# HSarham/automatic-ar

Measured on AMD Instinct MI355X. Metric: LM iterations/sec, higher is better.
Workload: dtype f64

## Files before the change

### automatic-ar_amd/aar/__init__.py

```python
import ctypes as C
import os

import numpy as np

_HERE = os.path.dirname(os.path.abspath(__file__))
LIB_PATH = os.environ.get("AAR_LIB") or os.path.join(os.path.dirname(_HERE), "libaar.so")

AAR_OK = 0
AAR_ERR_INVALID, AAR_ERR_NO_DEVICE, AAR_ERR_HIP, AAR_ERR_UNSUPPORTED = -1, -2, -3, -4
AAR_ERR_NUMERIC, AAR_ERR_IO, AAR_ERR_COMM = -5, -6, -7
RES_F32, RES_F64 = 0, 1
COMM_ID_BYTES = 128

SYMBOLS = [
    "aar_last_error", "aar_dataset_free", "aar_dataset_full_len", "aar_synth_default", "aar_synth_generate",
    "aar_solution_read", "aar_solution_write", "aar_solution_write_yaml", "aar_detections_write",
    "aar_rodrigues_vec2mat", "aar_rodrigues_mat2vec", "aar_plan_shards", "aar_comm_make_id", "aar_comm_create",
    "aar_comm_destroy", "aar_problem_desc_from_dataset", "aar_problem_create", "aar_problem_destroy",
    "aar_problem_full_len", "aar_problem_num_vars", "aar_problem_local_obs", "aar_eval_residuals",
    "aar_eval_normal_equations", "aar_eval_damped_step", "aar_lm_default_params", "aar_lm_init", "aar_lm_step",
    "aar_lm_get_solution", "aar_lm_solve", "aar_get_stage_times", "aar_reproj_stats", "aar_device_count",
    "aar_device_synchronize", "aar_set_kernel_profiling", "aar_get_kernel_times", "aar_kernel_name",
    "aar_problem_set_huber_delta", "aar_problem_get_huber_delta", "aar_track", "aar_cam_config_read",
    "aar_undistort_points", "aar_local_group_create", "aar_local_group_destroy", "aar_comm_create_local",
    "aar_cam_configs_read", "aar_detections_read", "aar_detections_free", "aar_subseqs_read", "aar_ippe_square",
    "aar_vote_transforms", "aar_init_default_params", "aar_initializer_run", "aar_initializer_object_poses",
    "aar_comm_get_stats", "aar_lm_set_step_callback", "aar_lm_set_stop_function", "aar_problem_extract_z", "aar_problem_merge_z",
    "aar_solution_read_ex", "aar_cam_configs_read_ex", "aar_set_stage_timers", "aar_problem_pcg_iterations",
    "aar_solver_default_options", "aar_problem_create_ex", "aar_problem_get_solver_stats", "aar_problem_set_test_hook",
    "aar_problem_covariance", "aar_covariance_write_yaml",
    "aar_problem_residual_report", "aar_dataset_select_observations", "aar_residual_report_write_yaml",
    "aar_problem_constraints_validate", "aar_problem_create_constrained", "aar_problem_num_priors", "aar_problem_eval_priors",
    "aar_smooth_params_validate", "aar_track_smooth", "aar_track_smooth_system",
]
NUM_KERNELS = 18
PRIOR_CAMERA, PRIOR_MARKER = 0, 1
PRIOR_KINDS = {"camera": PRIOR_CAMERA, "marker": PRIOR_MARKER}
SOLVER_DIRECT, SOLVER_PCG, SOLVER_SPCG, SOLVER_AUTO = 0, 1, 2, 3
TEST_HOOK_SPCG_DROP = 1
ENV_SOLVER, ENV_DETERMINISTIC, ENV_PCG_ETA, ENV_PCG_MAX_IT = 1, 2, 4, 8
SOLVERS = {"direct": SOLVER_DIRECT, "pcg": SOLVER_PCG, "spcg": SOLVER_SPCG, "auto": SOLVER_AUTO}
SOLVER_NAMES = {v: k for k, v in SOLVERS.items()}


class AarError(RuntimeError):
    def __init__(self, code, msg):
        super().__init__("aar error %d: %s" % (code, msg))
        self.code = code


class CDataset(C.Structure):
    _fields_ = [
        ("num_cams", C.c_int32), ("num_markers", C.c_int32), ("num_frames", C.c_int32),
        ("root_cam", C.c_int32), ("root_marker", C.c_int32),
        ("cam_ids", C.POINTER(C.c_int32)), ("marker_ids", C.POINTER(C.c_int32)), ("frame_ids", C.POINTER(C.c_int32)),
        ("image_sizes", C.POINTER(C.c_int32)), ("cam_mats", C.POINTER(C.c_double)), ("dist_coeffs", C.POINTER(C.c_double)),
        ("marker_size", C.c_double), ("num_obs", C.c_int64),
        ("obs_frame", C.POINTER(C.c_int32)), ("obs_cam", C.POINTER(C.c_int32)), ("obs_marker", C.POINTER(C.c_int32)),
        ("obs_uv", C.POINTER(C.c_float)), ("x_full", C.POINTER(C.c_double)), ("x_truth", C.POINTER(C.c_double)),
        ("optimize_cam_poses", C.c_int32), ("optimize_marker_poses", C.c_int32),
        ("optimize_object_poses", C.c_int32), ("optimize_cam_intrinsics", C.c_int32),
    ]


class CSynthDesc(C.Structure):
    _fields_ = [
        ("num_cams", C.c_int32), ("num_markers", C.c_int32), ("num_frames", C.c_int32), ("seed", C.c_uint64),
        ("marker_size", C.c_double), ("noise_px", C.c_double), ("init_rot_sigma", C.c_double),
        ("init_trans_sigma", C.c_double), ("init_scale", C.c_double), ("cam_arc_deg", C.c_double),
        ("min_view_cos", C.c_double),
    ]


class CProblemDesc(C.Structure):
    _fields_ = [
        ("num_cams", C.c_int32), ("num_markers", C.c_int32), ("num_frames", C.c_int32),
        ("root_cam", C.c_int32), ("root_marker", C.c_int32),
        ("cam_mats", C.POINTER(C.c_double)), ("marker_size", C.c_double), ("num_obs", C.c_int64),
        ("obs_frame", C.POINTER(C.c_int32)), ("obs_cam", C.POINTER(C.c_int32)), ("obs_marker", C.POINTER(C.c_int32)),
        ("obs_uv", C.POINTER(C.c_float)),
        ("optimize_cam_poses", C.c_int32), ("optimize_marker_poses", C.c_int32), ("optimize_object_poses", C.c_int32),
        ("optimize_cam_intrinsics", C.c_int32),
        ("residual_mode", C.c_int32), ("with_huber", C.c_int32), ("device_id", C.c_int32), ("comm", C.c_void_p),
    ]


class CSolverOptions(C.Structure):
    _fields_ = [("struct_size", C.c_uint32), ("solver", C.c_int32), ("deterministic", C.c_int32), ("pcg_max_it", C.c_int32),
                ("pcg_eta", C.c_double), ("pcg_eta_loose", C.c_double), ("pcg_eta_switch", C.c_double), ("pcg_abs_tol", C.c_double)]


class CSolverStats(C.Structure):
    _fields_ = [("struct_size", C.c_uint32), ("solver", C.c_int32), ("deterministic", C.c_int32), ("last_iterations", C.c_int32),
                ("total_iterations", C.c_int64), ("solves", C.c_int64), ("fallbacks", C.c_int64), ("pcg_eta", C.c_double),
                ("pcg_max_it", C.c_int32), ("env_overrides", C.c_int32), ("same_xcd_solves", C.c_int64), ("pcg_eta_loose", C.c_double),
                ("pcg_eta_switch", C.c_double), ("pcg_abs_tol", C.c_double)]


class CCovarianceReport(C.Structure):
    _fields_ = [("struct_size", C.c_uint32), ("num_residuals", C.c_int64), ("num_vars", C.c_int64), ("sum_sq", C.c_double),
                ("sigma2", C.c_double), ("min_pivot", C.c_double), ("max_pivot", C.c_double), ("frames_written", C.c_int32)]


class COutlierRule(C.Structure):
    _fields_ = [("struct_size", C.c_uint32), ("k_median", C.c_double), ("min_px", C.c_double)]


class CResidualReport(C.Structure):
    _fields_ = [("struct_size", C.c_uint32), ("num_detections", C.c_int64), ("num_rejected", C.c_int64), ("num_nonfinite", C.c_int64),
                ("sum_sq", C.c_double), ("rmse", C.c_double), ("median", C.c_double), ("max", C.c_double), ("threshold", C.c_double),
                ("cams_emptied", C.c_int32), ("markers_emptied", C.c_int32), ("frames_emptied", C.c_int32)]


class CPosePrior(C.Structure):
    _fields_ = [("kind", C.c_int32), ("index", C.c_int32), ("x6", C.c_double * 6), ("info", C.c_double * 36)]


class CConstraints(C.Structure):
    _fields_ = [("struct_size", C.c_uint32), ("n_fixed_cams", C.c_int32), ("fixed_cams", C.POINTER(C.c_int32)),
                ("n_fixed_markers", C.c_int32), ("fixed_markers", C.POINTER(C.c_int32)),
                ("n_priors", C.c_int32), ("priors", C.POINTER(CPosePrior))]


class Constraints:

    def __init__(self, fixed_cams=None, fixed_markers=None, priors=None):
        self._fc = np.ascontiguousarray(list(fixed_cams or []), dtype=np.int32)
        self._fm = np.ascontiguousarray(list(fixed_markers or []), dtype=np.int32)
        pr = list(priors or [])
        self._pr = (CPosePrior * max(len(pr), 1))()
        for i, (kind, index, x6, info) in enumerate(pr):
            q = self._pr[i]
            q.kind = PRIOR_KINDS[kind] if isinstance(kind, str) else int(kind)
            q.index = int(index)
            x6 = np.asarray(x6, dtype=np.float64).reshape(6)
            info = np.asarray(info, dtype=np.float64).reshape(36)
            for k in range(6):
                q.x6[k] = float(x6[k])
            for k in range(36):
                q.info[k] = float(info[k])
        c = CConstraints()
        c.struct_size = C.sizeof(CConstraints)
        c.n_fixed_cams = len(self._fc)
        c.fixed_cams = self._fc.ctypes.data_as(C.POINTER(C.c_int32)) if len(self._fc) else None
        c.n_fixed_markers = len(self._fm)
        c.fixed_markers = self._fm.ctypes.data_as(C.POINTER(C.c_int32)) if len(self._fm) else None
        c.n_priors = len(pr)
        c.priors = C.cast(self._pr, C.POINTER(CPosePrior)) if pr else None
        self.c = c
        self.n_priors = len(pr)

    def empty(self):
        return self.c.n_fixed_cams == 0 and self.c.n_fixed_markers == 0 and self.c.n_priors == 0


def constraints_validate(ds, fixed_cams=None, fixed_markers=None, priors=None, optimize=None, struct_size=None):
    cds = ds.as_c()
    d = CProblemDesc()
    lib().aar_problem_desc_from_dataset(C.byref(cds), C.byref(d))
    if optimize is not None:
        d.optimize_cam_poses, d.optimize_marker_poses, d.optimize_object_poses = [int(b) for b in optimize]
    k = Constraints(fixed_cams, fixed_markers, priors)
    if struct_size is not None:
        k.c.struct_size = int(struct_size)
    _check(lib().aar_problem_constraints_validate(C.byref(d), C.byref(k.c)))


class CLmParams(C.Structure):
    _fields_ = [
        ("max_iters", C.c_int32), ("min_error", C.c_double), ("min_step_error_diff", C.c_double),
        ("min_average_step_error_diff", C.c_double), ("tau", C.c_double), ("verbose", C.c_int32),
    ]


class CSmoothParams(C.Structure):
    _fields_ = [("struct_size", C.c_uint32), ("sigma_rot", C.c_double), ("sigma_trans", C.c_double),
                ("frame_time", C.POINTER(C.c_double)), ("rel_motion", C.POINTER(C.c_double))]


# ... 765 lines not shown
        x = np.array(self._x(x_full), dtype=np.float64)
        it = np.zeros(self.ds.num_frames, dtype=np.int32)
        err = np.zeros(self.ds.num_frames)
        _check(lib().aar_track(self.handle, _dptr(x), C.byref(params) if params is not None else None,
                               it.ctypes.data_as(C.POINTER(C.c_int32)), _dptr(err)))
        return x, it, err

    def track_smooth(self, x_full, sigma_rot, sigma_trans, frame_time=None, rel_motion=None, params=None):
        x = np.array(self._x(x_full), dtype=np.float64)
        F = self.ds.num_frames
        sp = SmoothParams(sigma_rot, sigma_trans, frame_time, rel_motion)
        sp.check_lengths(F)
        fe, pe = np.zeros(max(F, 1)), np.zeros(max(F - 1, 1))
        rep = CSmoothReport()
        rep.struct_size = C.sizeof(CSmoothReport)
        _check(lib().aar_track_smooth(self.handle, _dptr(x), C.byref(params) if params is not None else None, C.byref(sp.c),
                                      _dptr(fe), _dptr(pe), C.byref(rep)))
        report = {k: getattr(rep, k) for k, _ in CSmoothReport._fields_ if k != "struct_size"}
        return x, report, fe[:F], pe[:max(F - 1, 0)]

    def track_smooth_system(self, x_full, sigma_rot, sigma_trans, mu, frame_time=None, rel_motion=None):
        x = self._x(x_full)
        F = self.ds.num_frames
        sp = SmoothParams(sigma_rot, sigma_trans, frame_time, rel_motion)
        sp.check_lengths(F)
        diag, off = np.zeros((max(F, 1), 6, 6)), np.zeros((max(F - 1, 1), 6, 6))
        rhs, delta, cost = np.zeros(6 * max(F, 1)), np.zeros(6 * max(F, 1)), np.zeros(2)
        _check(lib().aar_track_smooth_system(self.handle, _dptr(x), C.byref(sp.c), float(mu), _dptr(diag), _dptr(off), _dptr(rhs),
                                             _dptr(delta), _dptr(cost)))
        return diag[:F], off[:max(F - 1, 0)], rhs[:6 * F], delta[:6 * F], (cost[0], cost[1])

    def set_step_callback(self, fn, want_z=True):
        if fn is None:
            self._step_cb = None
            _check(lib().aar_lm_set_step_callback(self.handle, C.cast(None, STEP_CB), None, 0))
            return
        def tramp(ctx, zp, n):
            fn(np.ctypeslib.as_array(zp, shape=(n,)).copy() if zp else None)
        self._step_cb = STEP_CB(tramp)
        _check(lib().aar_lm_set_step_callback(self.handle, self._step_cb, None, int(want_z)))

    def set_stop_function(self, fn):
        if fn is None:
            self._stop_fn = None
            _check(lib().aar_lm_set_stop_function(self.handle, C.cast(None, STOP_FN), None))
            return
        def tramp(ctx, zp, n):
            return 1 if fn(np.ctypeslib.as_array(zp, shape=(n,)).copy()) else 0
        self._stop_fn = STOP_FN(tramp)
        _check(lib().aar_lm_set_stop_function(self.handle, self._stop_fn, None))

    def extract_z(self, x_full):
        x = self._x(x_full)
        z = np.zeros(self.num_vars)
        _check(lib().aar_problem_extract_z(self.handle, _dptr(x), _dptr(z)))
        return z

    def set_huber_delta(self, delta):
        _check(lib().aar_problem_set_huber_delta(self.handle, float(delta)))

    def get_huber_delta(self):
        return float(lib().aar_problem_get_huber_delta(self.handle))

    def set_kernel_profiling(self, on):
        _check(lib().aar_set_kernel_profiling(self.handle, int(on)))

    def kernel_times(self):
        sec = np.zeros(NUM_KERNELS)
        cnt = np.zeros(NUM_KERNELS, dtype=np.int64)
        _check(lib().aar_get_kernel_times(self.handle, _dptr(sec), cnt.ctypes.data_as(C.POINTER(C.c_int64))))
        return {lib().aar_kernel_name(i).decode(): (float(sec[i]), int(cnt[i])) for i in range(NUM_KERNELS)}

    def pcg_iterations(self):
        out = (C.c_int32 * 2)()
        _check(lib().aar_problem_pcg_iterations(self.handle, out))
        return int(out[0]), int(out[1])

    def solver_stats(self):
        st = CSolverStats()
        st.struct_size = C.sizeof(CSolverStats)
        _check(lib().aar_problem_get_solver_stats(self.handle, C.byref(st)))
        return dict(solver=SOLVER_NAMES[st.solver], deterministic=bool(st.deterministic), last_iterations=st.last_iterations,
                    total_iterations=st.total_iterations, solves=st.solves, fallbacks=st.fallbacks, pcg_eta=st.pcg_eta, pcg_max_it=st.pcg_max_it,
                    same_xcd_solves=st.same_xcd_solves, pcg_eta_loose=st.pcg_eta_loose, pcg_eta_switch=st.pcg_eta_switch, pcg_abs_tol=st.pcg_abs_tol, env_overrides=st.env_overrides)

    def set_test_hook(self, hook, value):
        _check(lib().aar_problem_set_test_hook(self.handle, int(hook), int(value)))

    def set_stage_timers(self, on):
        _check(lib().aar_set_stage_timers(self.handle, int(on)))

    def stage_times(self):
        t = CStageTimes()
        _check(lib().aar_get_stage_times(self.handle, C.byref(t)))
        return {n: getattr(t, n) for n, _ in CStageTimes._fields_}
```

### automatic-ar_amd/csrc/ba_capi.hip

```cpp
#include <hip/hip_runtime.h>
#include <dlfcn.h>
#include <execinfo.h>
#include <fcntl.h>
#include <unistd.h>
#include <signal.h>

#include <algorithm>
#include <array>
#include <atomic>
#include <chrono>
#include <cmath>
#include <cstring>
#include <map>
#include <numeric>
#include <condition_variable>
#include <mutex>
#include <vector>

#include "../host/internal.h"
#include "geom.hpp"
#include "hostcopy.h"
#include "kernels.h"

using namespace aar;
// ... 112 lines not shown
    if (i < n_pad) {
        if (j > i) return;
        double *a = S + (size_t)i * n_pad + j, *b = packed + (size_t)i * (i + 1) / 2 + j;
        if (dir == 0) *b = *a; else *a = *b;
    } else if (j < extra) {
        double *a = S + (size_t)n_pad * n_pad + j, *b = packed + tri + j;
        if (dir == 0) *b = *a; else *a = *b;
    }
}
}

#define NCCL_TRY(expr)                                                                                          \
    do {                                                                                                        \
        int _r = (expr);                                                                                        \
        if (_r != 0)                                                                                            \
            return set_error(AAR_ERR_COMM, "%s failed: %s", #expr, g_nccl.GetErrorString ? g_nccl.GetErrorString(_r) : "?"); \
    } while (0)

struct aar_problem {
    DeviceProblem P;
    PoseLayout L;
    int f_begin = 0, f_end = 0;
    int64_t o_begin = 0, N_global = 0;
    aar_comm *comm = nullptr;
    int device = 0;
    hipStream_t stream = nullptr;
    std::vector<void *> allocs;
    double *h_scal = nullptr;
    int32_t h_flags[4] = {0, 0, 0, 0};
    unsigned long long seq = 0;
    double *d_frames_all = nullptr;
    double *d_diag = nullptr;
    double *d_pack = nullptr;
    double *d_status = nullptr;
    PinnedBuf h_z;
    double *h_gather = nullptr; size_t h_gather_n = 0;
    hipEvent_t up_ev = nullptr;
    bool mu_seed_valid = false;
    double mu_seed = 0;
    std::vector<int32_t> h_fslot_start, h_fslot_ent;
    std::vector<int32_t> h_ent_fixed;
    std::vector<aar_pose_prior> priors;
    aar_lm_params prm;
    int cur = 0;
    double mu = -1, v = 2, currErr = 0, prevErr = 0;
    double rel_drop = -1;
    bool lm_ready = false;
    bool with_huber = false;
    float hubber_delta = 2.5f;
    aar_lm_step_callback step_cb = nullptr;
    void *step_ctx = nullptr;
    bool step_want_z = false;
    aar_lm_stop_function stop_fn = nullptr;
    void *stop_ctx = nullptr;
    std::vector<double> cb_x, cb_z;
    float huber_of_blocks = -1.f;
    bool blocks_valid = false;
    double vinv_mu = -1;
    double schur_mu = -1;
    int panels_blk = -1;
    double panels_mu = -1;
    bool s_reduced = false;
    bool trial_reduced = false;
    bool fused_comm = true;
    bool spec_chol = true;
    int solver = AAR_SOLVER_DIRECT;
    int env_overrides = 0;
    bool force_direct = false;
    int spcg_skip = 0, spcg_backoff = 0;
    int last_cg_its = -1;
    int near_cap_tries = 0;
    int64_t spcg_fallbacks = 0;
    double *h_pcg = nullptr;
    unsigned long long pcg_seq = 0;
    int spec_chol_blk = -1;
    double spec_chol_mu = -1;
    bool spec_chol_by_cg = false;
    double spec_chol_eta = 0;
    hipStream_t stream2 = nullptr;
    hipEvent_t ev_fork = nullptr, ev_join = nullptr;
    bool overlap = false;
    bool merge_passes = true;
    int64_t trial_points = 0, launches = 0;
    aar_stage_times times;
    bool stage_timers = false;
    hipEvent_t ev[2] = {nullptr, nullptr};
    bool profiling = false;
    std::vector<hipEvent_t> ev_pool;
    std::vector<int> ev_kid;
    size_t ev_used = 0;
    double k_seconds[KID_COUNT] = {0};
    int64_t k_launches[KID_COUNT] = {0};
    double *cov_ws = nullptr;
    int32_t *cov_iws = nullptr;
    RRWork rr;
    bool rr_ready = false;
};

namespace {

template <class T>
int dev_alloc(aar_problem *pb, T **ptr, size_t count) {
    void *p = nullptr;
    size_t bytes = std::max<size_t>(count, 1) * sizeof(T);
    HIP_TRY(hipMalloc(&p, bytes));
    HIP_TRY(hipMemsetAsync(p, 0, bytes, pb->stream));
    pb->allocs.push_back(p);
    *ptr = static_cast<T *>(p);
    return AAR_OK;
}

int copy_h2d(aar_problem *pb, void *dst, const void *src, size_t bytes) {
    const char *what = "";
    const int e = h2d(dst, src, bytes, pb->stream, &what);
    return e ? set_error(AAR_ERR_HIP, "%s failed: %s", what, hipGetErrorString((hipError_t)e)) : AAR_OK;
}
int copy_d2h(aar_problem *pb, void *dst, const void *src, size_t bytes) {
    const char *what = "";
    const int e = d2h(dst, src, bytes, pb->stream, &what);
    return e ? set_error(AAR_ERR_HIP, "%s failed: %s", what, hipGetErrorString((hipError_t)e)) : AAR_OK;
}

template <class T>
int dev_upload(aar_problem *pb, T **ptr, const std::vector<T> &h) {
    int rc = dev_alloc(pb, ptr, h.size());
    if (rc) return rc;
    return h.empty() ? AAR_OK : copy_h2d(pb, *ptr, h.data(), h.size() * sizeof(T));
}

int ensure_device(int device_id) {
    int n = 0;
    hipError_t e = hipGetDeviceCount(&n);
    if (e != hipSuccess || n <= 0)
        return set_error(AAR_ERR_NO_DEVICE, "no HIP device available (%s); this library has no CPU path",
                         e == hipSuccess ? "device count 0" : hipGetErrorString(e));
    if (device_id < 0 || device_id >= n) return set_error(AAR_ERR_INVALID, "device_id %d out of range (%d devices)", device_id, n);
    HIP_TRY(hipSetDevice(device_id));
    return AAR_OK;
}

void pack_z(const aar_problem *pb, const double *x_full, double *z) {
    const PoseLayout &L = pb->L;
    const int A = pb->P.A, F = pb->P.F;
    memset(z, 0, (size_t)6 * (A + F) * sizeof(double));
    for (int c = 0; c < L.C; c++)
        if (c != L.rc) memcpy(&z[6 * (size_t)c], x_full + L.full_cam0() + 6LL * L.cam_slot(c), 6 * sizeof(double));
    for (int m = 0; m < L.M; m++)
        if (m != L.rm) memcpy(&z[6 * (size_t)(L.C + m)], x_full + L.full_mk0() + 6LL * L.mk_slot(m), 6 * sizeof(double));
    if (F) memcpy(&z[6 * (size_t)A], x_full + L.full_fr0() + 6LL * pb->f_begin, (size_t)6 * F * sizeof(double));
    if (L.oi)
        for (int c = 0; c < L.C; c++) memcpy(&z[6 * (size_t)(L.C + L.M + c)], x_full + L.full_intr0() + 9LL * c, 4 * sizeof(double));
}

int upload_z(aar_problem *pb, const double *x_full, int which) {
    if (pb->up_ev) HIP_TRY(hipEventSynchronize(pb->up_ev));
    const size_t cnt = (size_t)6 * (pb->P.A + pb->P.F);
    if (pb->h_z.reserve(cnt)) return set_error(AAR_ERR_HIP, "hipHostMalloc(pose staging) failed");
    pack_z(pb, x_full, pb->h_z.data());
    if (!pb->up_ev && hipEventCreateWithFlags(&pb->up_ev, hipEventDisableTiming) != hipSuccess) { pb->up_ev = nullptr; (void)hipGetLastError(); }
    if (cnt) HIP_TRY(hipMemcpyAsync(pb->P.z[which], pb->h_z.data(), cnt * sizeof(double), hipMemcpyHostToDevice, pb->stream));
    if (pb->up_ev) HIP_TRY(hipEventRecord(pb->up_ev, pb->stream));
    else HIP_TRY(hipStreamSynchronize(pb->stream));
    return AAR_OK;
}

int allreduce(aar_problem *pb, double *buf, size_t count, int op) {
// ... 292 lines not shown
        pb->spec_chol_blk = -1;
    }
    if (P.use_pcg) {
        if (pb->vinv_mu != mu) {
            launch_frame_inv(P, cur, mu, pb->stream);
            pb->vinv_mu = mu;
            pb->launches += 1;
        }
        if (!pb->comm) {
            StageTimer t(pb, &pb->times.chol);
            launch_pcg(P, cur, mu, pb->stream);
            pb->launches += 1;
        } else {
            { StageTimer t(pb, &pb->times.chol); launch_pcgd_setup(P, cur, mu, pb->stream); }
            { StageTimer t(pb, &pb->times.allreduce); int rc = allreduce(pb, P.pcgd_setup, (size_t)P.A * 28 + ((P.pcg_fused && !P.deterministic && P.pcg_coarse) ? 144 : 0), NCCL_SUM); if (rc) return rc; }
            pb->launches += 1;
            for (int k = 0;; k++) {
                const bool last = k >= P.pcg_max_it + 1;
                const bool poll = last || (k % 4) == 3;
                if (poll) pb->pcg_seq++;
                { StageTimer t(pb, &pb->times.chol); launch_pcgd_iter(P, cur, mu, k, last, poll ? pb->pcg_seq : 0ull, pb->stream); }
                pb->launches += 1;
                if (poll) {
                    int rc = check_async("pcg launch");
                    if (rc) return rc;
                    volatile unsigned long long *sq = reinterpret_cast<volatile unsigned long long *>(pb->h_pcg) + 3;
                    const auto t0 = std::chrono::steady_clock::now();
                    unsigned spins = 0;
                    int poll_rc = AAR_OK;
                    while (*sq != pb->pcg_seq) {
                        if ((++spins & 0x3fff) == 0) {
                            if (hipStreamQuery(pb->stream) == hipSuccess && *sq != pb->pcg_seq) {
                                poll_rc = set_error(AAR_ERR_HIP, "device did not publish the PCG progress record: %s", hipGetErrorString(hipGetLastError()));
                                break;
                            }
                            if (std::chrono::duration<double>(std::chrono::steady_clock::now() - t0).count() > 120.0) {
                                poll_rc = set_error(AAR_ERR_HIP, "timed out waiting for the PCG progress record");
                                break;
                            }
                        }
                        __builtin_ia32_pause();
                    }
                    std::atomic_thread_fence(std::memory_order_acquire);
                    if (poll_rc) return poll_rc;
                    if (pb->h_pcg[0] != 0.0 || last) break;
                }
                { StageTimer t(pb, &pb->times.allreduce); int rc = allreduce(pb, pcgd_y_of_launch(P, k), (size_t)6 * P.A, NCCL_SUM); if (rc) return rc; }
            }
        }
        chol_done = true;
    }
    if (!P.use_pcg && pb->schur_mu != mu) {
        StageTimer t(pb, &pb->times.schur);
        if (pb->s_reduced) {
            int rc = zero_block_set(pb, cur);
            if (rc) return rc;
            launch_passB(P, cur, pb->stream);
            launch_prior(P, cur, true, pb->stream);
            pb->launches += P.n_prior ? 2 : 1;
            pb->s_reduced = false;
        } else if (pb->schur_mu >= 0) {
            launch_schur(P, cur, -1.0, pb->stream, 0, 0, nullptr, panels_ok(pb, cur, pb->schur_mu));
            panels_now(pb, cur, pb->schur_mu);
            pb->launches += 1;
        }
        if (pb->vinv_mu != mu) {
            launch_frame_inv(P, cur, mu, pb->stream);
            pb->vinv_mu = mu;
            pb->launches += 1;
        }
        launch_schur(P, cur, 1.0, pb->stream, 0, 0, nullptr, panels_ok(pb, cur, mu));
        panels_now(pb, cur, mu);
        pb->launches += 1;
    }
    pb->schur_mu = -1;
    if (pb->comm && !pb->s_reduced && !P.use_pcg) {
        StageTimer t(pb, &pb->times.allreduce);
        int rc = allreduce_system(pb, cur, 0);
        if (rc) return rc;
    }
    pb->s_reduced = false;
    pb->trial_reduced = false;
    bool backsub_rode = false;
    if (P.use_spcg && !pb->force_direct && pb->spcg_skip > 0) pb->spcg_skip--;
    if (!chol_done) {
        StageTimer t(pb, &pb->times.chol);
        if (by_cg) backsub_rode = launch_spcg(P, cur, mu, pb->stream, pb->stage_timers ? -1 : tr);
        else backsub_rode = launch_chol(P, cur, mu, pb->stream, pb->stage_timers ? -1 : tr);
    }
    if (!backsub_rode) {
        StageTimer t(pb, &pb->times.backsub);
        launch_backsub(P, cur, tr, pb->stream);
    }
    pb->launches += 2 + 3 * P.nT;
    pb->blocks_valid = false;
    if (evaluate_trial) {
        int rc = eval_blocks(pb, tr, mu * 0.33, cur, false, true);
        if (rc) return rc;
        pb->trial_points++;
    } else {
        HIP_TRY(hipMemsetAsync(P.err_part, 0, sizeof(double) * (size_t)std::max(n_err_terms(P), 1), pb->stream));
    }
    int rc = AAR_OK;
    bool rode = false;
    if (P.use_pcg) {
        if ((rc = launch_scalars(pb, n_err_terms(P)))) return rc;
    } else if (evaluate_trial && !pb->comm) {
        StageTimer t(pb, &pb->times.schur);
        rode = launch_schur(P, tr, 1.0, pb->stream, pb->seq + 1, n_err_terms(P), nullptr, panels_ok(pb, tr, mu * 0.33));
        panels_now(pb, tr, mu * 0.33);
        pb->launches += 1;
        if (rode) pb->seq++;
        else if ((rc = launch_scalars(pb, n_err_terms(P)))) return rc;
    } else if (evaluate_trial && pb->fused_comm) {
        {
            StageTimer t(pb, &pb->times.schur);
            rode = launch_schur(P, tr, 1.0, pb->stream, 0, n_err_terms(P), P.blk[tr].tail, panels_ok(pb, tr, mu * 0.33));
            panels_now(pb, tr, mu * 0.33);
            pb->launches += 1;
            if (!rode) { launch_reduce_scalars(P, n_err_terms(P), false, 0ull, pb->stream, P.blk[tr].tail); pb->launches += 1; }
        }
        pb->seq++;
        {
            StageTimer t(pb, &pb->times.allreduce);
            if ((rc = allreduce_system(pb, tr, 4, pb->seq))) return rc;
        }
        pb->trial_reduced = true;
        if (pb->spec_chol && !pb->stage_timers && !pb->profiling) {
            StageTimer t(pb, &pb->times.chol);
            const bool spec_cg = P.use_spcg && pb->spcg_skip == 0 && !cg_near_cap;
            if (spec_cg) launch_spcg(P, tr, mu * 0.33, pb->stream);
            else (void)launch_chol(P, tr, mu * 0.33, pb->stream);
            pb->spec_chol_by_cg = spec_cg;
            pb->spec_chol_blk = tr;
            pb->spec_chol_mu = mu * 0.33;
            pb->spec_chol_eta = P.pcg_eta_now;
            pb->launches += 3 * P.nT;
        }
    } else {
        if ((rc = launch_scalars(pb, n_err_terms(P)))) return rc;
        if (evaluate_trial) {
            StageTimer t(pb, &pb->times.schur);
            launch_schur(P, tr, 1.0, pb->stream, 0, 0, nullptr, panels_ok(pb, tr, mu * 0.33));
            panels_now(pb, tr, mu * 0.33);
            pb->launches += 1;
        }
    }
    if ((rc = check_async("kernel launch"))) return rc;
    if ((rc = wait_result(pb))) return rc;
    if (by_cg && pb->h_scal[7] >= 0.0) pb->last_cg_its = (int)pb->h_scal[7];
    if (by_cg && (pb->h_flags[0] & (8 | 4))) pb->last_cg_its = std::min(P.spcg_max_it, SPCG_MAX_IT);
    if (cg_near_cap && P.use_spcg && !pb->force_direct && pb->spcg_skip == 0 && ++pb->near_cap_tries >= 8) { pb->last_cg_its = -1; pb->near_cap_tries = 0; }
    if (pb->h_flags[0]) {
        (void)hipMemsetAsync(P.flags, 0, 4 * sizeof(int32_t), pb->stream);
        if (by_cg && (pb->h_flags[0] & (8 | 4))) {
            if (pb->h_flags[0] & 4) spcg_ws_reset(P, pb->stream);
            pb->spcg_fallbacks++;
            pb->spcg_backoff = pb->spcg_backoff ? std::min(2 * pb->spcg_backoff, 1024) : 8;
            pb->spcg_skip = pb->spcg_backoff;
            return TRY_CG_FAILED;
        }
        set_error(AAR_ERR_NUMERIC, "device flags %d at mu=%g (1: a frame block is not positive definite, 2: non-positive pivot of the reduced system, 4: back-substitution chain timed out)", pb->h_flags[0], mu);
        return ((pb->h_flags[0] & 2) && !(pb->h_flags[0] & 4)) ? TRY_NOT_POSITIVE_DEFINITE : AAR_ERR_NUMERIC;
    }
    return AAR_OK;
}

int rebuild_current(aar_problem *pb) {
    pb->mu_seed_valid = false;
    int rc = zero_block_set(pb, pb->cur);
    if (rc) return rc;
    if ((rc = zero_block_set(pb, 1 - pb->cur))) return rc;
    const float huber_now = pb->P.huber;
    if (pb->with_huber && pb->huber_of_blocks > 0.f) pb->P.huber = pb->huber_of_blocks;
    rc = eval_blocks(pb, pb->cur, -1.0, -1);
    pb->P.huber = huber_now;
    if (rc) return rc;
    pb->blocks_valid = true;
    pb->vinv_mu = -1;
    pb->schur_mu = -1;
    pb->s_reduced = pb->trial_reduced = false;
    return AAR_OK;
}

int damped_try_fb(aar_problem *pb, double mu, bool evaluate_trial) {
    int rc = damped_try(pb, mu, evaluate_trial);
    if (rc != TRY_CG_FAILED) return rc;
    if (evaluate_trial) pb->trial_points--;
    pb->trial_reduced = false;
    if ((rc = rebuild_current(pb))) return rc;
    pb->force_direct = true;
    rc = damped_try(pb, mu, evaluate_trial);
// ... 274 lines not shown
    return problem_create(d, opts, &k, out);
}

int32_t aar_problem_num_priors(const aar_problem *pb) { return pb ? pb->P.n_prior : 0; }

static int abort_bt_fd = 2;
static void abort_backtrace(int sig) {
    void *bt[64];
    { char msg[64]; const int k = aar::g_last_kernel_id; int n = 0; const char *t = "last kernel id "; while (t[n]) { msg[n] = t[n]; n++; } if (k < 0) msg[n++] = '-'; else { if (k >= 10) msg[n++] = '0' + k / 10; msg[n++] = '0' + k % 10; } msg[n++] = '\n'; (void)!write(abort_bt_fd, msg, n); }
    const int n = backtrace(bt, 64);
    backtrace_symbols_fd(bt, n, abort_bt_fd);
    signal(sig, SIG_DFL);
    raise(sig);
}

int aar_problem_create_ex(const aar_problem_desc *d, const aar_solver_options *opts, aar_problem **out) { return problem_create(d, opts, nullptr, out); }

static int problem_create(const aar_problem_desc *d, const aar_solver_options *opts, const aar_problem_constraints *cons, aar_problem **out) {
    { static bool once = false; if (!once && getenv("AAR_ABORT_BACKTRACE")) { once = true; const int fd = open(getenv("AAR_ABORT_BACKTRACE"), O_WRONLY | O_CREAT | O_APPEND, 0644); if (fd >= 0) abort_bt_fd = fd; signal(SIGABRT, abort_backtrace); } }
    if (!d || !out) return set_error(AAR_ERR_INVALID, "aar_problem_create: null argument");
    aar_solver_options so;
    aar_solver_default_options(&so);
    if (opts) {
        if (opts->struct_size < 2 * sizeof(uint32_t)) return set_error(AAR_ERR_INVALID, "aar_solver_options.struct_size is not set (use aar_solver_default_options)");
        memcpy(&so, opts, std::min<size_t>(opts->struct_size, sizeof so));
        so.struct_size = (uint32_t)sizeof so;
    }
    int env_over = 0;
    if (const char *e = getenv("AAR_SOLVER")) {
        if (so.solver == AAR_SOLVER_AUTO) {
            int v = -1;
            if (!strcmp(e, "direct")) v = AAR_SOLVER_DIRECT;
            else if (!strcmp(e, "pcg")) v = AAR_SOLVER_PCG;
            else if (!strcmp(e, "spcg")) v = AAR_SOLVER_SPCG;
            if (v >= 0) { so.solver = v; env_over |= AAR_ENV_SOLVER; }
        }
    }
    if (const char *e = getenv("AAR_DETERMINISTIC")) if (!so.deterministic && atoi(e) != 0) { so.deterministic = 1; env_over |= AAR_ENV_DETERMINISTIC; }
    if (const char *e = getenv("AAR_PCG_ETA")) if (so.pcg_eta == 0 && atof(e) > 0) { so.pcg_eta = atof(e); env_over |= AAR_ENV_PCG_ETA; }
    if (const char *e = getenv("AAR_PCG_MAX_IT")) if (so.pcg_max_it == 0 && atoi(e) > 0) { so.pcg_max_it = atoi(e); env_over |= AAR_ENV_PCG_MAX_IT; }
    if (so.solver < AAR_SOLVER_DIRECT || so.solver > AAR_SOLVER_AUTO) return set_error(AAR_ERR_INVALID, "aar_solver_options.solver %d is not one of AAR_SOLVER_*", so.solver);
    if (so.pcg_eta < 0 || so.pcg_max_it < 0 || so.pcg_eta_loose < 0 || so.pcg_eta_switch < 0 || so.pcg_abs_tol < 0) return set_error(AAR_ERR_INVALID, "aar_solver_options: negative pcg_eta / pcg_eta_loose / pcg_eta_switch / pcg_abs_tol / pcg_max_it");
    const int C = d->num_cams, M = d->num_markers, Fg = d->num_frames;
    const int64_t Ng = d->num_obs;
    if (C < 1 || M < 1 || Fg < 0 || Ng < 0) return set_error(AAR_ERR_INVALID, "aar_problem_create: bad sizes");
    if (d->root_cam < 0 || d->root_cam >= C || d->root_marker < 0 || d->root_marker >= M)
        return set_error(AAR_ERR_INVALID, "aar_problem_create: root index out of range");
    if (!d->cam_mats || (Ng > 0 && (!d->obs_frame || !d->obs_cam || !d->obs_marker || !d->obs_uv)))
        return set_error(AAR_ERR_INVALID, "aar_problem_create: null array");
    if (Ng >= (1LL << 31) || (int64_t)C + M >= 32768) return set_error(AAR_ERR_UNSUPPORTED, "problem too large for 32-bit indexing");
    std::vector<int64_t> per_frame(Fg, 0);
    int64_t global_slots = 0;
    {
        std::vector<int32_t> seen_c(C, -1), seen_m(M, -1);
        for (int64_t o = 0; o < Ng; o++) {
            const int f = d->obs_frame[o], c = d->obs_cam[o], m = d->obs_marker[o];
            if (f < 0 || f >= Fg || c < 0 || c >= C || m < 0 || m >= M) return set_error(AAR_ERR_INVALID, "observation %lld has an index out of range", (long long)o);
            if (o > 0 && f < d->obs_frame[o - 1]) return set_error(AAR_ERR_INVALID, "observations must be ordered by frame (reference residual order)");
            per_frame[f]++;
            if (seen_c[c] != f) { seen_c[c] = f; global_slots += d->optimize_cam_intrinsics ? 2 : 1; }
            if (seen_m[m] != f) { seen_m[m] = f; global_slots += 1; }
        }
    }
    int rc = ensure_device(d->device_id);
    if (rc) return rc;

    aar_problem *pb = new aar_problem();
    pb->device = d->device_id;
    pb->comm = d->comm;
    aar_lm_default_params(&pb->prm);
    memset(&pb->times, 0, sizeof pb->times);
    const char *tenv = getenv("AAR_STAGE_TIMERS");
    pb->stage_timers = tenv && tenv[0] == '1';
    auto fail = [&](int code) { aar_problem_destroy(pb); return code; };
    if (hipStreamCreateWithFlags(&pb->stream, hipStreamNonBlocking) != hipSuccess) return fail(set_error(AAR_ERR_HIP, "hipStreamCreate failed"));
    (void)hipEventCreate(&pb->ev[0]);
    (void)hipEventCreate(&pb->ev[1]);
    if (hipStreamCreateWithFlags(&pb->stream2, hipStreamNonBlocking) != hipSuccess ||
        hipEventCreateWithFlags(&pb->ev_fork, hipEventDisableTiming) != hipSuccess ||
        hipEventCreateWithFlags(&pb->ev_join, hipEventDisableTiming) != hipSuccess)
        return fail(set_error(AAR_ERR_HIP, "second stream / events could not be created"));
    { const char *e = getenv("AAR_OVERLAP"); pb->overlap = (e && e[0] == '1'); }
    { const char *e = getenv("AAR_MERGE_PASSES"); if (e) pb->merge_passes = (e[0] != '0'); }
    { const char *e = getenv("AAR_FUSED_COMM"); if (e) pb->fused_comm = (e[0] != '0'); }
    { const char *e = getenv("AAR_SPEC_CHOL"); if (e) pb->spec_chol = (e[0] != '0'); }

    PoseLayout &L = pb->L;
    L.C = C; L.M = M; L.F = Fg; L.rc = d->root_cam; L.rm = d->root_marker;
    L.oc = d->optimize_cam_poses != 0; L.om = d->optimize_marker_poses != 0; L.of = d->optimize_object_poses != 0;
    L.oi = d->optimize_cam_intrinsics != 0;
    pb->N_global = Ng;

    const int world = pb->comm ? pb->comm->world : 1, rank = pb->comm ? pb->comm->rank : 0;
    pb->P.pcg_rank0 = rank == 0 ? 1 : 0;
    std::vector<int32_t> begin(world + 1, 0);
    if ((rc = aar_plan_shards(Fg, per_frame.data(), world, begin.data()))) return fail(rc);
    pb->f_begin = begin[rank];
    pb->f_end = begin[rank + 1];
    int64_t ob = 0;
    for (int f = 0; f < pb->f_begin; f++) ob += per_frame[f];
    int64_t N = 0;
    for (int f = pb->f_begin; f < pb->f_end; f++) N += per_frame[f];
    pb->o_begin = ob;

    DeviceProblem &P = pb->P;
    P.intr = L.oi ? 1 : 0;
    P.C = C; P.M = M; P.A = C + M + (L.oi ? C : 0); P.F = pb->f_end - pb->f_begin; P.N = N;
    P.n = 6 * P.A;
    P.nT = (P.n + CHOL_NB - 1) / CHOL_NB;
    P.n_pad = P.nT * CHOL_NB;
    P.spcg_root_c = (L.oc && C > 1) ? L.rc : -1;
    P.spcg_root_m = (L.om && M > 1) ? C + L.rm : -1;
    P.spcg_n_free = (L.oc ? C - 1 : 0) + (L.om ? M - 1 : 0) + (L.oi ? C : 0);
    P.res_f32 = d->residual_mode == AAR_RES_F64 ? 0 : 1;
    pb->with_huber = d->with_huber != 0;
    P.huber = pb->with_huber ? pb->hubber_delta : -1.f;
    P.half_size = (double)((float)d->marker_size / 2.f);
    P.frames_fixed = L.of ? 0 : 1;
    const int A = P.A, F = P.F;
    std::vector<int32_t> held(C + M, 0);
    bool held_extra = false;
    if (cons) {
        for (int i = 0; i < cons->n_fixed_cams; i++) { const int c = cons->fixed_cams[i]; if (c != L.rc && L.oc) { held[c] = 1; held_extra = true; } }
        for (int i = 0; i < cons->n_fixed_markers; i++) { const int m = cons->fixed_markers[i]; if (m != L.rm && L.om) { held[C + m] = 1; held_extra = true; } }
    }

    int local_rc = AAR_OK;
    std::vector<int32_t> frame_obs_start(F + 1, 0), fslot_start(F + 1, 0), fslot_ent;
    std::vector<ObsIdx> a_idx(N);
    std::vector<float> a_uv((size_t)8 * N);
    if (N) memcpy(a_uv.data(), d->obs_uv + 8 * ob, sizeof(float) * 8 * N);
    {
        int64_t o = 0;
        std::vector<int32_t> slot_of(A, -1);
        for (int f = 0; f < F; f++) {
            frame_obs_start[f] = (int32_t)o;
            const int64_t cnt = per_frame[pb->f_begin + f];
            std::vector<int32_t> ents;
            for (int64_t k = 0; k < cnt; k++) {
                const int64_t g = ob + o + k;
                ents.push_back(d->obs_cam[g]);
                ents.push_back(C + d->obs_marker[g]);
                if (L.oi) ents.push_back(C + M + d->obs_cam[g]);
            }
            std::sort(ents.begin(), ents.end());
            ents.erase(std::unique(ents.begin(), ents.end()), ents.end());
            if (ents.size() >= (1u << SLOT_C_BITS) && !local_rc) local_rc = set_error(AAR_ERR_UNSUPPORTED, "frame %d touches %zu entities (limit %d)", f, ents.size(), (1 << SLOT_C_BITS) - 1);
            for (size_t s = 0; s < ents.size(); s++) slot_of[ents[s]] = (int32_t)s;
            for (int64_t k = 0; k < cnt; k++) {
                const int64_t g = ob + o + k;
                ObsIdx id;
                id.frame = f; id.cam = d->obs_cam[g]; id.marker = C + d->obs_marker[g];
                id.slots = pack_slots(slot_of[id.cam], slot_of[id.marker], L.oi ? slot_of[C + M + id.cam] : 0);
                a_idx[o + k] = id;
            }
            fslot_start[f] = (int32_t)fslot_ent.size();
            fslot_ent.insert(fslot_ent.end(), ents.begin(), ents.end());
            P.max_kf = std::max<int>(P.max_kf, (int)ents.size());
            o += cnt;
        }
        frame_obs_start[F] = (int32_t)o;
        fslot_start[F] = (int32_t)fslot_ent.size();
    }
    P.total_slots = (int)fslot_ent.size();
    std::vector<int32_t> frame_stride(F, 1);
    for (int f = 0; f < F; f++) {
// ... 1330 lines not shown
    if (frame_err && F && (rc = copy_d2h(pb, frame_err, w.Ef[cur], (size_t)F * sizeof(double)))) return rc;
    if (pair_err && F > 1 && (rc = copy_d2h(pb, pair_err, w.Pe[cur], (size_t)(F - 1) * sizeof(double)))) return rc;
    if ((rc = check_async("smoothing kernels"))) return rc;
    PoseLayout keep = pb->L;
    pb->L.oc = false; pb->L.om = false; pb->L.of = true;
    rc = download_z(pb, pb->cur, x_full);
    pb->L = keep;
    if (rc) return rc;
    if (report) {
        aar_smooth_report r;
        memset(&r, 0, sizeof r);
        r.struct_size = report->struct_size;
        r.iterations = iters; r.stop_code = mustExit; r.rejected_tries = rejected;
        r.initial_cost = initial; r.final_cost = currErr; r.final_data_cost = currData; r.final_prior_cost = currPrior;
        r.final_mu = mu;
        r.seconds = std::chrono::duration<double>(std::chrono::steady_clock::now() - t0).count();
        memcpy(report, &r, std::min<size_t>(report->struct_size, sizeof r));
    }
    return AAR_OK;
}

int aar_set_kernel_profiling(aar_problem *pb, int on) {
    if (!pb) return set_error(AAR_ERR_INVALID, "aar_set_kernel_profiling: null argument");
    HIP_TRY(hipSetDevice(pb->device));
    HIP_TRY(hipStreamSynchronize(pb->stream));
    pb->ev_kid.clear();
    pb->ev_used = 0;
    pb->profiling = on != 0;
    if (on) {
        memset(pb->k_seconds, 0, sizeof pb->k_seconds);
        memset(pb->k_launches, 0, sizeof pb->k_launches);
        pb->P.hook.pre = prof_pre;
        pb->P.hook.post = prof_post;
        pb->P.hook.ctx = pb;
    } else {
        pb->P.hook = LaunchHook();
    }
    return AAR_OK;
}

int aar_get_kernel_times(aar_problem *pb, double seconds[AAR_NUM_KERNELS], int64_t launches[AAR_NUM_KERNELS]) {
    if (!pb || !seconds || !launches) return set_error(AAR_ERR_INVALID, "aar_get_kernel_times: null argument");
    static_assert(AAR_NUM_KERNELS == KID_COUNT, "kernel id table out of sync with include/aar.h");
    static_assert(ENT_STRIDE == ENT_STRIDE_H, "entity row stride");
    HIP_TRY(hipSetDevice(pb->device));
    HIP_TRY(hipStreamSynchronize(pb->stream));
    prof_harvest(pb);
    for (int i = 0; i < KID_COUNT; i++) { seconds[i] = pb->k_seconds[i]; launches[i] = pb->k_launches[i]; }
    return AAR_OK;
}

const char *aar_kernel_name(int kid) {
    static const char *names[KID_COUNT] = {"k_unpack", "k_residual", "k_passA", "k_passB", "k_maxdiag", "k_frame_inv", "k_schur",
                                           "k_ldl_diag", "k_ldl_trsm", "k_ldl_update", "k_ldl_backsolve", "k_backsub",
                                           "k_reduce_scalars", "k_ldl_panel", "k_pcg", "k_spcg", "k_spcg_pre", "k_prior"};
    return (kid >= 0 && kid < KID_COUNT) ? names[kid] : "?";
}

int aar_problem_pcg_iterations(aar_problem *pb, int32_t out[2]) {
    if (!pb || !out) return set_error(AAR_ERR_INVALID, "aar_problem_pcg_iterations: null argument");
    out[0] = out[1] = 0;
    if (!pb->P.use_pcg && !pb->P.use_spcg) return AAR_OK;
    HIP_TRY(hipSetDevice(pb->device));
    { int rc = copy_d2h(pb, out, pb->P.use_pcg ? pb->P.pcg_counter + 2 : pb->P.spcg_iters, 2 * sizeof(int32_t)); if (rc) return rc; }
    if (out[0] > SPCG_MAX_IT && pb->P.use_spcg) out[0] = SPCG_MAX_IT;
    return AAR_OK;
}

int aar_problem_get_solver_stats(aar_problem *pb, aar_solver_stats *out) {
    if (!pb || !out) return set_error(AAR_ERR_INVALID, "aar_problem_get_solver_stats: null argument");
    const size_t cap = out->struct_size;
    if (cap < 4 * sizeof(int32_t) || cap > 4096) return set_error(AAR_ERR_INVALID, "aar_solver_stats.struct_size is not set (sizeof(aar_solver_stats) of the caller)");
    aar_solver_stats st;
    memset(&st, 0, sizeof st);
    st.solver = pb->solver;
    st.deterministic = pb->P.deterministic;
    st.pcg_eta = pb->P.pcg_eta;
    st.pcg_max_it = pb->P.use_spcg ? pb->P.spcg_max_it : pb->P.pcg_max_it;
    st.pcg_eta_loose = pb->P.pcg_eta_loose;
    st.pcg_eta_switch = pb->P.pcg_eta_switch;
    st.pcg_abs_tol = pb->P.pcg_abs_tol;
    st.env_overrides = pb->env_overrides;
    st.fallbacks = pb->spcg_fallbacks;
    if (pb->P.use_pcg || pb->P.use_spcg) {
        int32_t c[8] = {0, 0, 0, 0, 0, 0, 0, 0};
        HIP_TRY(hipSetDevice(pb->device));
        int rc = copy_d2h(pb, c, pb->P.use_spcg ? pb->P.spcg_iters : pb->P.pcg_counter + 2, (pb->P.use_spcg ? 8 : 3) * sizeof(int32_t));
        if (rc) return rc;
        st.last_iterations = std::min(c[0], pb->P.use_spcg ? SPCG_MAX_IT : c[0]);
        st.total_iterations = c[1];
        st.solves = c[2];
        st.same_xcd_solves = c[4];
    }
    st.struct_size = (uint32_t)std::min(cap, sizeof st);
    memcpy(out, &st, std::min(cap, sizeof st));
    return AAR_OK;
}

int aar_problem_set_test_hook(aar_problem *pb, int32_t hook, int32_t value) {
    if (!pb) return set_error(AAR_ERR_INVALID, "aar_problem_set_test_hook: null argument");
    if (hook == AAR_TEST_HOOK_SPCG_DROP) { pb->P.spcg_test_drop = value; return AAR_OK; }
    return set_error(AAR_ERR_INVALID, "aar_problem_set_test_hook: unknown hook %d", hook);
}

int aar_set_stage_timers(aar_problem *pb, int on) {
    if (!pb) return set_error(AAR_ERR_INVALID, "aar_set_stage_timers: null argument");
    HIP_TRY(hipSetDevice(pb->device));
    HIP_TRY(hipStreamSynchronize(pb->stream));
    pb->stage_timers = on != 0;
    memset(&pb->times, 0, sizeof pb->times);
    return AAR_OK;
}

int aar_get_stage_times(aar_problem *pb, aar_stage_times *t) {
    if (!pb || !t) return set_error(AAR_ERR_INVALID, "aar_get_stage_times: null argument");
    *t = pb->times;
    return AAR_OK;
}

}
```

### automatic-ar_amd/csrc/backsub.hpp

```cpp
#pragma once
#include "geom.hpp"
#include "kernels.h"

namespace aar {

__device__ __forceinline__ void hop_publish(int32_t *flag, int value, bool leader) {
    asm volatile("s_waitcnt vmcnt(0)" ::: "memory");
    if (leader) __hip_atomic_store(flag, value, __ATOMIC_RELAXED, __HIP_MEMORY_SCOPE_AGENT);
}
__device__ __forceinline__ bool hop_wait(const int32_t *flag, int value) {
    long spins = 0;
    while (__hip_atomic_load(flag, __ATOMIC_RELAXED, __HIP_MEMORY_SCOPE_AGENT) != value) {
        __builtin_amdgcn_s_sleep(1);
        if (++spins > (1L << 24)) return false;
    }
    asm volatile("" ::: "memory");
    return true;
}

struct BacksubArgs {
    const int32_t *fslot_start, *fslot_ent;
    const double *W, *Vinv, *gf, *g0, *delta_s, *zc;
    const float *Wf;
    double *zt;
    int A, F, n_frame_blocks;
    double *lin_part, *ent_out;
    int k_ent0;
};

__device__ __forceinline__ void backsub_body(const BacksubArgs &b, int blk, double *red, const int32_t *flag, int epoch, int32_t *err_flags) {
    const int tid = threadIdx.x, lane = tid & 63, wave = __builtin_amdgcn_readfirstlane(tid >> 6), nwaves = blockDim.x >> 6;
    auto dl = [&](int i) -> double {
        return flag ? __hip_atomic_load(b.delta_s + i, __ATOMIC_RELAXED, __HIP_MEMORY_SCOPE_AGENT) : b.delta_s[i];
    };
    auto wait = [&]() {
        if (!flag) return;
        if (tid == 0 && !hop_wait(flag, epoch)) atomicOr(err_flags, 4);
        __syncthreads();
    };
    if (blk == b.n_frame_blocks) {
        wait();
        double d2 = 0.0, dg = 0.0;
        for (int i = tid; i < 6 * b.A; i += blockDim.x) {
            const double d = dl(i);
            b.zt[i] = b.zc[i] + d;
            d2 += d * d;
            dg += d * b.g0[i];
        }
#pragma unroll
        for (int off = 32; off > 0; off >>= 1) { d2 += __shfl_xor(d2, off); dg += __shfl_xor(dg, off); }
        if (lane == 0) { red[wave] = d2; red[16 + wave] = dg; }
        __syncthreads();
        if (tid == 0) {
            double s2 = 0.0, sg = 0.0;
            for (int w = 0; w < nwaves; w++) { s2 += red[w]; sg += red[16 + w]; }
            b.lin_part[2 * (size_t)b.F] = s2;
            b.lin_part[2 * (size_t)b.F + 1] = sg;
        }
        __threadfence_block();
        __syncthreads();
        for (int e = tid; e < b.A; e += blockDim.x) {
            if (e >= b.k_ent0) make_k_row(b.zt + 6 * (size_t)e, b.ent_out + (size_t)e * ENT_STRIDE);
            else make_ent_row(b.zt + 6 * (size_t)e, b.ent_out + (size_t)e * ENT_STRIDE);
        }
        return;
    }
    const int f = blk * nwaves + wave;
    const bool live = f < b.F;
    const int s0 = live ? b.fslot_start[f] : 0, s1 = live ? b.fslot_start[f + 1] : 0;
    const int sl = s0 + lane;
    const bool has = sl < s1;
    int a0 = 0;
    double2 w0[18];
    if (has) {
        a0 = b.fslot_ent[sl];
        if (b.Wf) {
            const float4 *wf = reinterpret_cast<const float4 *>(b.Wf + (size_t)s0 * 36) + lane;
            const int kf = s1 - s0;
#pragma unroll
            for (int q = 0; q < 9; q++) {
                const float4 v = wf[(size_t)q * kf];
                w0[2 * q] = make_double2(v.x, v.y); w0[2 * q + 1] = make_double2(v.z, v.w);
            }
        } else {
            const double2 *wb = reinterpret_cast<const double2 *>(b.W + (size_t)sl * 36);
#pragma unroll
            for (int q = 0; q < 18; q++) w0[q] = wb[q];
        }
    }
    double g[6], vrow[6], zc6 = 0.0;
#pragma unroll
    for (int i = 0; i < 6; i++) { g[i] = live ? b.gf[(size_t)f * 6 + i] : 0.0; vrow[i] = (live && lane < 6) ? b.Vinv[(size_t)f * 36 + lane * 6 + i] : 0.0; }
    if (live && lane < 6) zc6 = b.zc[(size_t)6 * (b.A + f) + lane];
    wait();
    if (!live) return;
    double c[6] = {0, 0, 0, 0, 0, 0};
    if (has) {
        double da[6];
#pragma unroll
        for (int i = 0; i < 6; i++) da[i] = dl(6 * a0 + i);
#pragma unroll
        for (int i = 0; i < 6; i++) {
            c[0] += w0[3 * i].x * da[i]; c[1] += w0[3 * i].y * da[i]; c[2] += w0[3 * i + 1].x * da[i];
            c[3] += w0[3 * i + 1].y * da[i]; c[4] += w0[3 * i + 2].x * da[i]; c[5] += w0[3 * i + 2].y * da[i];
        }
    }
    for (int s = s0 + lane + 64; s < s1; s += 64) {
        const int a = b.fslot_ent[s];
        double2 wt[18];
        if (b.Wf) {
            const float4 *wf = reinterpret_cast<const float4 *>(b.Wf + (size_t)s0 * 36) + (s - s0);
            const int kf = s1 - s0;
#pragma unroll
            for (int q = 0; q < 9; q++) {
                const float4 v = wf[(size_t)q * kf];
                wt[2 * q] = make_double2(v.x, v.y); wt[2 * q + 1] = make_double2(v.z, v.w);
            }
        } else {
            const double2 *wb = reinterpret_cast<const double2 *>(b.W + (size_t)s * 36);
#pragma unroll
            for (int q = 0; q < 18; q++) wt[q] = wb[q];
        }
        double da[6];
#pragma unroll
        for (int i = 0; i < 6; i++) da[i] = dl(6 * a + i);
#pragma unroll
        for (int i = 0; i < 6; i++) {
            const double2 x0 = wt[3 * i], x1 = wt[3 * i + 1], x2 = wt[3 * i + 2];
            c[0] += x0.x * da[i]; c[1] += x0.y * da[i]; c[2] += x1.x * da[i];
            c[3] += x1.y * da[i]; c[4] += x2.x * da[i]; c[5] += x2.y * da[i];
        }
    }
#pragma unroll
    for (int off = 32; off > 0; off >>= 1)
#pragma unroll
        for (int i = 0; i < 6; i++) c[i] += __shfl_xor(c[i], off);
    double d = 0.0;
    if (lane < 6) {
#pragma unroll
        for (int k = 0; k < 6; k++) d += vrow[k] * (g[k] - c[k]);
        b.zt[(size_t)6 * (b.A + f) + lane] = zc6 + d;
    }
    {
        const double zn = (lane < 6) ? zc6 + d : 0.0;
        double zv[6];
#pragma unroll
        for (int i = 0; i < 6; i++) zv[i] = __shfl(zn, i);
        if (lane == 0) make_ent_row(zv, b.ent_out + (size_t)(b.A + f) * ENT_STRIDE);
    }
    double d2 = (lane < 6) ? d * d : 0.0;
    double dgv = 0.0;
#pragma unroll
    for (int i = 0; i < 6; i++) dgv += (lane == i) ? d * g[i] : 0.0;
#pragma unroll
    for (int off = 4; off > 0; off >>= 1) { d2 += __shfl_xor(d2, off); dgv += __shfl_xor(dgv, off); }
    if (lane == 0) { b.lin_part[2 * (size_t)f] = d2; b.lin_part[2 * (size_t)f + 1] = dgv; }
}

BacksubArgs backsub_args(const DeviceProblem &P, int cur, int trial, int waves_per_block);

}
```

### automatic-ar_amd/csrc/eval_kernels.hip

```cpp
#include <algorithm>
#include <vector>
#include "geom.hpp"
#include "kernels.h"
#include "hostcopy.h"
#include "wave.hpp"
#include "track_eval.hpp"

namespace aar {

volatile int g_last_kernel_id = -1;

template <int NV, int CH = 32, class Sink>
__device__ __forceinline__ void wave_sum_lds(const double (&vals)[NV], double *__restrict__ sc, int lane, Sink sink) {
    constexpr int L = 64 / CH;
    constexpr int SPREAD = 32 / CH > 0 ? 32 / CH : 1;
#pragma unroll
    for (int base = 0; base < NV; base += CH) {
        const int cnt = (NV - base) < CH ? (NV - base) : CH;
#pragma unroll
        for (int i = 0; i < CH; i++)
            if (i < cnt) sc[i * 64 + lane] = vals[base + i];
        __builtin_amdgcn_fence(__ATOMIC_RELEASE, "wavefront");
        __builtin_amdgcn_wave_barrier();
        const int vi = lane / L, part = lane % L;
        double s = 0;
        if (vi < cnt) {
            const double *row = sc + lane * CH;
#pragma unroll 8
            for (int k = 0; k < CH; k++) s += row[(k + lane / SPREAD) & (CH - 1)];
        }
#pragma unroll
        for (int off = 1; off < L; off <<= 1) s += __shfl_xor(s, off);
        if (part == 0 && vi < cnt) sink(base + vi, s);
        __builtin_amdgcn_wave_barrier();
        __builtin_amdgcn_fence(__ATOMIC_ACQUIRE, "wavefront");
    }
}

__global__ void k_unpack(const double *__restrict__ z, double *__restrict__ ent, int n_ent, int k0, int k1, double *__restrict__ zero_p, int64_t zero_n,
                         double *__restrict__ zero_q, int64_t zero_qn) {
    const int64_t gid = (int64_t)blockIdx.x * blockDim.x + threadIdx.x;
    for (int64_t i = gid; i < zero_n; i += (int64_t)gridDim.x * blockDim.x) zero_p[i] = 0.0;
    for (int64_t i = gid; i < zero_qn; i += (int64_t)gridDim.x * blockDim.x) zero_q[i] = 0.0;
    if (gid >= n_ent) return;
    if (gid >= k0 && gid < k1) make_k_row(z + 6 * gid, ent + gid * ENT_STRIDE);
    else make_ent_row(z + 6 * gid, ent + gid * ENT_STRIDE);
}

__global__ void __launch_bounds__(256) k_residual(const ObsIdx *__restrict__ idx, const float *__restrict__ uv,
                                                  const double *__restrict__ ent, const double *__restrict__ Kmat, int kstride,
                                                  int64_t N, int A, double h, int res_f32, float huber, double *__restrict__ r_out,
                                                  double *__restrict__ err_part) {
    const int64_t o = (int64_t)blockIdx.x * blockDim.x + threadIdx.x;
    double ss = 0;
    if (o < N) {
        const ObsIdx id = idx[o];
        const float4 uv0 = reinterpret_cast<const float4 *>(uv)[2 * o];
        const float4 uv1 = reinterpret_cast<const float4 *>(uv)[2 * o + 1];
        const float ou[8] = {uv0.x, uv0.y, uv0.z, uv0.w, uv1.x, uv1.y, uv1.z, uv1.w};
        EntRT ec, em, ef;
        load_ent_rt(ent, id.cam, ec);
        load_ent_rt(ent, id.marker, em);
        load_ent_rt(ent, A + id.frame, ef);
        double K[9];
#pragma unroll
        for (int i = 0; i < 9; i++) K[i] = Kmat[kstride * id.cam + i];
#pragma unroll
        for (int k = 0; k < 4; k++) {
            CornerGeom g;
            project_corner(ec, em, ef, K, h, k, g);
            double rx, ry;
            corner_residual(ou[2 * k], ou[2 * k + 1], g.u, g.v, res_f32, huber, rx, ry);
            ss += rx * rx + ry * ry;
            if (r_out) {
                r_out[8 * o + 2 * k] = rx;
                r_out[8 * o + 2 * k + 1] = ry;
            }
        }
    }
    __shared__ double wsum[4];
#pragma unroll
    for (int off = 32; off > 0; off >>= 1) ss += __shfl_xor(ss, off);
    if ((threadIdx.x & 63) == 0) wsum[threadIdx.x >> 6] = ss;
    __syncthreads();
    if (threadIdx.x == 0) err_part[blockIdx.x] = wsum[0] + wsum[1] + wsum[2] + wsum[3];
}

__device__ __forceinline__ void load_ent_lds(const double *row, Ent &e) {
#pragma unroll
    for (int i = 0; i < 9; i++) e.R[i] = row[i];
#pragma unroll
    for (int i = 0; i < 3; i++) e.t[i] = row[9 + i];
#pragma unroll
    for (int i = 0; i < 9; i++) e.Jl[i] = row[12 + i];
}

struct PassAArgs {
    const ObsIdx *idx; const float *uv; const double *ent; const double *Kmat;
    int kstride;
    const int32_t *frame_obs_start, *fslot_start, *fslot_ent, *frame_stride;
    unsigned long long *stamps;
    int k_ent0;
    int A, F, C, res_f32, max_kf, frames_fixed;
    float huber;
    double h, mu_pred;
    double *V, *gf, *W, *Vinv, *hf, *err_part;
    float *Wf;
    double *zero0; int64_t zero0_n; double *zero1; int64_t zero1_n; double *zero2; int64_t zero2_n;
    int32_t *flags;
    double *Wd, *Yd; const int32_t *slot_dense; int Ad;
};

constexpr int ENT_LDS = 25;
constexpr int WLS = 37;
__host__ __device__ constexpr size_t passA_w_doubles(int max_kf) { return ((size_t)max_kf * WLS + 1) & ~(size_t)1; }
__host__ __device__ constexpr int passA_sum_chunk(int block) { return block >= 128 ? 8 : 32; }

template <int BLOCK>
__device__ __forceinline__ void passA_epilogue(const PassAArgs &a, const double *Wl, const double *acc, double *scratch, const int f, const int s0, const int kf) {
    const int tid = threadIdx.x;
// ... 119 lines not shown
    }
    constexpr int LPO = 4 / CPL;
    for (int t = tid; t < nobs * LPO; t += BLOCK) {
        const int it = t / LPO, part = t - it * LPO;
        const int o = o0 + (int)(((int64_t)it * stride) % nobs);
        const ObsIdx id = a.idx[o];
        const int sc = id.slots & ((1 << SLOT_C_BITS) - 1), sm = (id.slots >> SLOT_C_BITS) & ((1 << SLOT_M_BITS) - 1);
        const int sk = (id.slots >> (SLOT_C_BITS + SLOT_M_BITS)) & ((1 << SLOT_M_BITS) - 1);
        Ent ec, em;
        load_ent_lds(entl + (size_t)sc * ENT_LDS, ec);
        load_ent_lds(entl + (size_t)sm * ENT_LDS, em);
        double K[9];
#pragma unroll
        for (int i = 0; i < 9; i++) K[i] = a.Kmat[a.kstride * id.cam + i];
        double Wc[36], Wm[36], Wk[INTR ? 24 : 1];
#pragma unroll
        for (int i = 0; i < 36; i++) { Wc[i] = 0.0; Wm[i] = 0.0; }
        if (INTR) {
#pragma unroll
            for (int i = 0; i < 24; i++) Wk[i] = 0.0;
        }
#pragma unroll
        for (int kk = 0; kk < CPL; kk++) {
            const int k = part * CPL + kk;
            const float2 ouv = reinterpret_cast<const float2 *>(a.uv)[4 * (int64_t)o + k];
            CornerGeom g;
            project_corner(ec, em, ef, K, a.h, k, g);
            double r[2];
            corner_residual(ouv.x, ouv.y, g.u, g.v, a.res_f32, a.huber, r[0], r[1]);
            double Gc[2][6], Gm[2][6], Gf[2][6];
            corner_jacobian<true, true, true>(ec, em, ef, K, g, Gc, Gm, Gf);
            if (INTR) {
                double Gk[2][4];
                corner_jacobian_intr(g, Gk);
#pragma unroll
                for (int rr = 0; rr < 2; rr++)
#pragma unroll
                    for (int i = 0; i < 4; i++)
#pragma unroll
                        for (int j = 0; j < 6; j++) Wk[i * 6 + j] += Gk[rr][i] * Gf[rr][j];
            }
#pragma unroll
            for (int rr = 0; rr < 2; rr++) {
                vals[27] += r[rr] * r[rr];
#pragma unroll
                for (int i = 0; i < 6; i++) {
                    vals[21 + i] += Gf[rr][i] * r[rr];
#pragma unroll
                    for (int j = 0; j <= i; j++) vals[i * (i + 1) / 2 + j] += Gf[rr][i] * Gf[rr][j];
#pragma unroll
                    for (int j = 0; j < 6; j++) {
                        Wc[i * 6 + j] += Gc[rr][i] * Gf[rr][j];
                        Wm[i * 6 + j] += Gm[rr][i] * Gf[rr][j];
                    }
                }
            }
        }
        double *wc = Wl + sc * WLS;
        double *wm = Wl + sm * WLS;
#pragma unroll
        for (int i = 0; i < 36; i++) atomicAdd(wc + i, Wc[i]);
#pragma unroll
        for (int i = 0; i < 36; i++) atomicAdd(wm + i, Wm[i]);
        if (INTR) {
            double *wk = Wl + sk * WLS;
#pragma unroll
            for (int i = 0; i < 24; i++) atomicAdd(wk + i, Wk[i]);
        }
    }
    wave_sum_lds<28, CH>(vals, scratch + wave * (CH * 64), lane, [&](int i, double s) { atomicAdd(acc + i, s); });
    __syncthreads();
    passA_epilogue<BLOCK>(a, Wl, acc, scratch, f, s0, kf);
}

constexpr int HLS = 21, HLS_INTR = 25;
__host__ __device__ constexpr size_t passA_h_doubles(int max_kf, int hls = HLS) { return ((size_t)max_kf * hls + 1) & ~(size_t)1; }

#ifdef AAR_PASSA_STAMPS
#define PA_STAMP(n) do { if (a.stamps && f < 512 && tid == 0) a.stamps[f * 16 + (n)] = __builtin_readcyclecounter(); } while (0)
#else
#define PA_STAMP(n) do { } while (0)
#endif

template <int BLOCK, int CPL, bool INTR = false>
__device__ __forceinline__ void passA_wrench_body(const PassAArgs &a, double *lds, const int f, const int n_blocks_a) {
    constexpr int SL = INTR ? HLS_INTR : HLS;
    double *Hl = lds;
    double *acc = lds + passA_h_doubles(a.max_kf, SL);
    double *hacc = acc + 32;
    double *frow = acc + 64;
    double *Yl = frow + 24;
    double *vil = Yl + 36;
    const int tid = threadIdx.x, lane = tid & 63, wave = tid >> 6;
    const int o0 = a.frame_obs_start[f], nobs = a.frame_obs_start[f + 1] - o0;
    const int s0 = a.fslot_start[f], kf = a.fslot_start[f + 1] - s0;
    PA_STAMP(0);
    Ent ef;
    load_ent(a.ent, a.A + __builtin_amdgcn_readfirstlane(f), ef);
    constexpr int LPO = 4 / CPL;
    const int stride = a.frame_stride[f];
    const int part = tid % LPO;
    int pos = 0, step = 0;
    if (nobs > 0) {
        pos = (int)(((unsigned long long)(tid / LPO) * (unsigned)stride) % (unsigned)nobs);
        step = (int)(((unsigned long long)(BLOCK / LPO) * (unsigned)stride) % (unsigned)nobs);
    }
    int t = tid;
    bool have = t < nobs * LPO;
    ObsIdx id = {0, 0, 0, 0};
    float2 ouv[CPL];
    EntRT ec, em;
    double K[9];
    auto fetch_obs = [&]() {
        const int o = o0 + pos;
        id = a.idx[o];
#pragma unroll
        for (int kk = 0; kk < CPL; kk++) ouv[kk] = reinterpret_cast<const float2 *>(a.uv)[4 * (int64_t)o + part * CPL + kk];
    };
    auto fetch_rows = [&]() {
        load_ent_rt(a.ent, id.cam, ec);
        load_ent_rt(a.ent, id.marker, em);
#pragma unroll
        for (int i = 0; i < 9; i++) K[i] = a.Kmat[a.kstride * id.cam + i];
    };
    if (have) fetch_obs();
    const int e_slot = tid < kf ? a.fslot_ent[s0 + tid] : -1;
    double2 frv = make_double2(0.0, 0.0);
    if (tid < ENT_STRIDE / 2) frv = reinterpret_cast<const double2 *>(a.ent + (size_t)(a.A + f) * ENT_STRIDE)[tid];
    for (int i = tid; i < kf * SL; i += BLOCK) Hl[i] = 0.0;
    for (int i = tid; i < 64; i += BLOCK) acc[i] = 0.0;
    if (have) fetch_rows();
    {
        const int64_t gid = (int64_t)f * BLOCK + tid, gstride = (int64_t)n_blocks_a * BLOCK;
        for (int64_t i = gid; i < a.zero0_n; i += gstride) a.zero0[i] = 0.0;
        for (int64_t i = gid; i < a.zero1_n; i += gstride) a.zero1[i] = 0.0;
        for (int64_t i = gid; i < a.zero2_n; i += gstride) a.zero2[i] = 0.0;
    }
    __syncthreads();
    PA_STAMP(1);

    double vals[7];
#pragma unroll
    for (int i = 0; i < 7; i++) vals[i] = 0.0;
    while (have) {
        const int sc = id.slots & ((1 << SLOT_C_BITS) - 1), sm = (id.slots >> SLOT_C_BITS) & ((1 << SLOT_M_BITS) - 1);
        const int sk = (id.slots >> (SLOT_C_BITS + SLOT_M_BITS)) & ((1 << SLOT_M_BITS) - 1);
        double H[21], Mk[INTR ? 24 : 1];
#pragma unroll
        for (int i = 0; i < 21; i++) H[i] = 0.0;
        if (INTR) {
#pragma unroll
            for (int i = 0; i < 24; i++) Mk[i] = 0.0;
        }
#pragma unroll (INTR && CPL == 4 ? 2 : CPL)
        for (int kk = 0; kk < CPL; kk++) {
            CornerGeom g;
            project_corner(ec, em, ef, K, a.h, part * CPL + kk, g);
            double r[2], w[2][6];
            corner_residual(ouv[kk].x, ouv[kk].y, g.u, g.v, a.res_f32, a.huber, r[0], r[1]);
            corner_wrench(ec, K, g, w);
            if (INTR) {
                double Gk[2][4];
                corner_jacobian_intr(g, Gk);
#pragma unroll
                for (int rr = 0; rr < 2; rr++)
#pragma unroll
                    for (int i = 0; i < 4; i++)
#pragma unroll
                        for (int j = 0; j < 6; j++) Mk[i * 6 + j] += Gk[rr][i] * w[rr][j];
            }
#pragma unroll
            for (int rr = 0; rr < 2; rr++) {
                vals[6] += r[rr] * r[rr];
#pragma unroll
                for (int i = 0; i < 6; i++) {
                    vals[i] += w[rr][i] * r[rr];
#pragma unroll
                    for (int j = 0; j <= i; j++) H[i * (i + 1) / 2 + j] += w[rr][i] * w[rr][j];
                }
            }
        }
        t += BLOCK;
        have = t < nobs * LPO;
        if (have) {
            pos += step;
            if (pos >= nobs) pos -= nobs;
            fetch_obs();
        }
        double *hc = Hl + sc * SL, *hm = Hl + sm * SL;
#pragma unroll
        for (int i = 0; i < 21; i++) atomicAdd(hc + i, H[i]);
#pragma unroll
        for (int i = 0; i < 21; i++) atomicAdd(hm + i, H[i]);
        if (INTR) {
            double *hk = Hl + sk * SL;
#pragma unroll
            for (int i = 0; i < 24; i++) atomicAdd(hk + i, Mk[i]);
        }
        if (have) fetch_rows();
    }
    PA_STAMP(2);
    double2 rv[7];
    if (e_slot >= 0) {
        const double2 *rowp = reinterpret_cast<const double2 *>(a.ent + (size_t)e_slot * ENT_STRIDE);
#pragma unroll
        for (int i = 0; i < 7; i++) rv[i] = rowp[4 + i];
        if (e_slot < a.C) atomicAdd(hacc + 30, 1.0);
    }
    for (int ts = tid + BLOCK; ts < kf; ts += BLOCK)
        if (a.fslot_ent[s0 + ts] < a.C) atomicAdd(hacc + 30, 1.0);
    if (tid < ENT_STRIDE / 2) { frow[2 * tid] = frv.x; frow[2 * tid + 1] = frv.y; }
#pragma unroll
    for (int i = 0; i < 7; i++) {
        const double sv = wave_sum_dpp(vals[i]);
        if (lane == 0) atomicAdd(hacc + 21 + i, sv);
    }
    PA_STAMP(3);
    __syncthreads();
    PA_STAMP(4);
    if (tid < 21) {
        const int nc = (int)hacc[30];
        double sv = 0.0;
        for (int ts = 0; ts < nc; ts++) sv += Hl[ts * SL + tid];
        hacc[tid] = sv;
    }
    __syncthreads();
    PA_STAMP(5);
    if (wave == BLOCK / 64 - 1) {
        const double *jl = frow + 12;
        if (lane < 36) {
            const int k = lane / 6, j = lane - 6 * k;
            Yl[lane] = j < 3 ? hacc[sym6(k, 0)] * jl[j] + hacc[sym6(k, 1)] * jl[3 + j] + hacc[sym6(k, 2)] * jl[6 + j] : hacc[sym6(k, j)];
        }
        __builtin_amdgcn_fence(__ATOMIC_RELEASE, "wavefront");
        __builtin_amdgcn_wave_barrier();
        __builtin_amdgcn_fence(__ATOMIC_ACQUIRE, "wavefront");
        if (lane < 28) {
            double out;
            if (lane < 21) {
                int i = 0;
                while ((i + 1) * (i + 2) / 2 <= lane) i++;
                const int j = lane - i * (i + 1) / 2;
                out = i < 3 ? jl[i] * Yl[j] + jl[3 + i] * Yl[6 + j] + jl[6 + i] * Yl[12 + j] : Yl[i * 6 + j];
            } else if (lane < 27) {
                const int i = lane - 21;
                out = i < 3 ? jl[i] * hacc[21] + jl[3 + i] * hacc[22] + jl[6 + i] * hacc[23] : hacc[21 + i];
            } else out = hacc[27];
            acc[lane] = out;
        }
        __builtin_amdgcn_fence(__ATOMIC_RELEASE, "wavefront");
        __builtin_amdgcn_wave_barrier();
        __builtin_amdgcn_fence(__ATOMIC_ACQUIRE, "wavefront");
        if (a.mu_pred >= 0.0 && lane == 63) {
            double out[36];
            if (a.frames_fixed) {
#pragma unroll
                for (int i = 0; i < 36; i++) out[i] = 0.0;
            } else {
                double m[6][6];
#pragma unroll
                for (int i = 0; i < 6; i++)
#pragma unroll
                    for (int j = 0; j < 6; j++) m[i][j] = acc[sym6(i, j)] + (i == j ? a.mu_pred : 0.0);
                if (!spd6_inverse(m, out)) atomicOr(a.flags, 1);
            }
            const bool dense_ = a.Yd != nullptr;
#pragma unroll
            for (int i = 0; i < 6; i++) {
                double hv = 0.0;
#pragma unroll
                for (int j = 0; j < 6; j++) {
                    a.Vinv[(size_t)f * 36 + i * 6 + j] = out[i * 6 + j];
                    hv += out[i * 6 + j] * acc[21 + j];
                    if (dense_) vil[i * 6 + j] = out[i * 6 + j];
                }
                a.hf[(size_t)f * 6 + i] = hv;
            }
        }
    }
    PA_STAMP(6);
    for (int ts = tid; ts < kf; ts += BLOCK) {
        int e = e_slot;
        if (ts != tid) {
            e = a.fslot_ent[s0 + ts];
            const double2 *rowp = reinterpret_cast<const double2 *>(a.ent + (size_t)e * ENT_STRIDE);
#pragma unroll
            for (int i = 0; i < 7; i++) rv[i] = rowp[4 + i];
        }
        if (INTR && e >= a.k_ent0) {
            const double *mk = Hl + ts * SL;
            double wv[36];
#pragma unroll
            for (int i = 0; i < 4; i++) {
                double m6[6];
#pragma unroll
                for (int j = 0; j < 6; j++) m6[j] = mk[i * 6 + j];
#pragma unroll
                for (int j = 0; j < 3; j++) wv[6 * i + j] = m6[0] * ef.Jl[j] + m6[1] * ef.Jl[3 + j] + m6[2] * ef.Jl[6 + j];
                wv[6 * i + 3] = m6[3]; wv[6 * i + 4] = m6[4]; wv[6 * i + 5] = m6[5];
            }
#pragma unroll
            for (int q = 24; q < 36; q++) wv[q] = 0.0;
            if (a.W) {
                double2 *wp = reinterpret_cast<double2 *>(a.W + (size_t)(s0 + ts) * 36);
#pragma unroll
                for (int q = 0; q < 18; q++) wp[q] = make_double2(wv[2 * q], wv[2 * q + 1]);
            }
            if (a.Wf) {
                float4 *wf = reinterpret_cast<float4 *>(a.Wf + (size_t)s0 * 36) + ts;
#pragma unroll
                for (int q = 0; q < 9; q++) wf[(size_t)q * kf] = make_float4((float)wv[4 * q], (float)wv[4 * q + 1], (float)wv[4 * q + 2], (float)wv[4 * q + 3]);
            }
            continue;
        }
        const bool cam = e < a.C;
        const double tt[3] = {cam ? rv[0].y - ef.t[0] : rv[0].y, cam ? rv[1].x - ef.t[1] : rv[1].x, cam ? rv[1].y - ef.t[2] : rv[1].y};
        const double Jl[9] = {rv[2].x, rv[2].y, rv[3].x, rv[3].y, rv[4].x, rv[4].y, rv[5].x, rv[5].y, rv[6].x};
        double H[21], X[6][6];
        const double *slot = Hl + ts * SL;
#pragma unroll
        for (int i = 0; i < 21; i++) H[i] = slot[i];
#pragma unroll
        for (int l = 0; l < 6; l++) {
            double zt[3], zb[3], x[3];
#pragma unroll
            for (int i = 0; i < 3; i++) {
                zt[i] = cam ? H[sym6(i, l)] : ef.R[i] * H[sym6(0, l)] + ef.R[3 + i] * H[sym6(1, l)] + ef.R[6 + i] * H[sym6(2, l)];
                zb[i] = cam ? H[sym6(3 + i, l)] : ef.R[i] * H[sym6(3, l)] + ef.R[3 + i] * H[sym6(4, l)] + ef.R[6 + i] * H[sym6(5, l)];
            }
            cross3(tt, zb, x);
            const double v[3] = {zt[0] - x[0], zt[1] - x[1], zt[2] - x[2]};
#pragma unroll
            for (int i = 0; i < 3; i++) {
                const double wt = Jl[i] * v[0] + Jl[3 + i] * v[1] + Jl[6 + i] * v[2];
                X[i][l] = cam ? -wt : wt;
                X[3 + i][l] = cam ? -zb[i] : zb[i];
            }
        }
        double2 *wp = reinterpret_cast<double2 *>(a.W + (size_t)(s0 + ts) * 36);
        float4 *wf = a.Wf ? reinterpret_cast<float4 *>(a.Wf + (size_t)s0 * 36) + ts : nullptr;
#pragma unroll
        for (int i2 = 0; i2 < 3; i2++) {
            float w12[12];
#pragma unroll
            for (int ii = 0; ii < 2; ii++) {
                const int i = 2 * i2 + ii;
                double wr[3];
#pragma unroll
                for (int j = 0; j < 3; j++) wr[j] = X[i][0] * ef.Jl[j] + X[i][1] * ef.Jl[3 + j] + X[i][2] * ef.Jl[6 + j];
                if (a.W) {
                    wp[3 * i] = make_double2(wr[0], wr[1]);
                    wp[3 * i + 1] = make_double2(wr[2], X[i][3]);
                    wp[3 * i + 2] = make_double2(X[i][4], X[i][5]);
                }
                w12[6 * ii] = (float)wr[0]; w12[6 * ii + 1] = (float)wr[1]; w12[6 * ii + 2] = (float)wr[2];
                w12[6 * ii + 3] = (float)X[i][3]; w12[6 * ii + 4] = (float)X[i][4]; w12[6 * ii + 5] = (float)X[i][5];
            }
            if (wf) {
#pragma unroll
                for (int q = 0; q < 3; q++) wf[(size_t)(3 * i2 + q) * kf] = make_float4(w12[4 * q], w12[4 * q + 1], w12[4 * q + 2], w12[4 * q + 3]);
            }
        }
    }
    PA_STAMP(7);
    __syncthreads();
    PA_STAMP(8);
    for (int q = tid; q < 36; q += BLOCK) a.V[(size_t)f * 36 + q] = acc[sym6(q / 6, q % 6)];
    for (int q = tid; q < 6; q += BLOCK) a.gf[(size_t)f * 6 + q] = acc[21 + q];
    if (tid == 0) a.err_part[f] = acc[27];
    const bool dense = a.Yd != nullptr && a.mu_pred >= 0.0;
    PA_STAMP(9);
    if (dense) {
        __syncthreads();
        double vi[36];
#pragma unroll
        for (int q = 0; q < 36; q++) vi[q] = vil[q];
        const size_t fbase = (size_t)f * a.Ad * 36;
        for (int ts = tid; ts < kf; ts += BLOCK) {
            const double2 *wp = reinterpret_cast<const double2 *>(a.W + (size_t)(s0 + ts) * 36);
            const size_t o = fbase + (size_t)a.slot_dense[s0 + ts] * 36;
#pragma unroll
            for (int i = 0; i < 6; i++) {
                const double2 w0 = wp[3 * i], w1 = wp[3 * i + 1], w2 = wp[3 * i + 2];
                const double w[6] = {w0.x, w0.y, w1.x, w1.y, w2.x, w2.y};
                double y[6] = {0, 0, 0, 0, 0, 0};
#pragma unroll
                for (int k = 0; k < 6; k++)
#pragma unroll
                    for (int j = 0; j < 6; j++) y[j] = fma(w[k], vi[k * 6 + j], y[j]);
                double2 *yp = reinterpret_cast<double2 *>(a.Yd + o + i * 6), *wd = reinterpret_cast<double2 *>(a.Wd + o + i * 6);
                yp[0] = make_double2(y[0], y[1]); yp[1] = make_double2(y[2], y[3]); yp[2] = make_double2(y[4], y[5]);
                wd[0] = w0; wd[1] = w1; wd[2] = w2;
            }
        }
        if (tid < 6) a.Wd[fbase + tid] = acc[21 + tid];
    }
}

struct PassBArgs {
    const ObsIdx *idx; const float *uv; const double *ent; const double *Kmat; const int32_t *chunk_start;
    int kstride, k_ent0;
    int n_chunks, A, res_f32, n_pad;
    float huber;
    double h;
    double *U0, *g0;
    double *part; int part_stride;
};

template <bool DET = false, bool LEAN = false>
__device__ __forceinline__ void passB_body(const PassBArgs &b, double *scratch, const int first_chunk) {
    const ObsIdx *__restrict__ idx = b.idx;
    const float *__restrict__ uv = b.uv;
    const double *__restrict__ ent = b.ent, *__restrict__ Kmat = b.Kmat;
    const int32_t *__restrict__ chunk_start = b.chunk_start;
    const int n_chunks = b.n_chunks, A = b.A, res_f32 = b.res_f32, n_pad = b.n_pad;
    const float huber = b.huber;
    const double h = b.h;
    double *__restrict__ U0 = b.U0, *__restrict__ g0 = b.g0;
    const int lane = threadIdx.x & 63, wave = __builtin_amdgcn_readfirstlane(threadIdx.x >> 6);
    const int chunk = first_chunk + wave;
    if (chunk >= n_chunks) return;
    const int o0 = chunk_start[chunk], o1 = chunk_start[chunk + 1];
    double vals[90];
#pragma unroll
    for (int i = 0; i < 90; i++) vals[i] = 0.0;
    const ObsIdx head = idx[o0];
    Ent ec, em;
    load_ent(ent, head.cam, ec);
    load_ent(ent, head.marker, em);
    double K[9];
#pragma unroll
    for (int i = 0; i < 9; i++) K[i] = Kmat[b.kstride * head.cam + i];
    for (int o = o0 + lane; o < o1; o += 64) {
        const ObsIdx id = idx[o];
        const float4 uv0 = reinterpret_cast<const float4 *>(uv)[2 * (int64_t)o];
        const float4 uv1 = reinterpret_cast<const float4 *>(uv)[2 * (int64_t)o + 1];
        const float ou[8] = {uv0.x, uv0.y, uv0.z, uv0.w, uv1.x, uv1.y, uv1.z, uv1.w};
        Ent ef;
        load_ent(ent, A + id.frame, ef);
#pragma unroll LEAN ? 1 : 4
        for (int k = 0; k < 4; k++) {
            CornerGeom g;
            project_corner(ec, em, ef, K, h, k, g);
            double r[2];
            float ox, oy;
            if (LEAN) { const float2 t = reinterpret_cast<const float2 *>(uv)[4 * (int64_t)o + k]; ox = t.x; oy = t.y; }
            else { ox = ou[2 * k]; oy = ou[2 * k + 1]; }
            corner_residual(ox, oy, g.u, g.v, res_f32, huber, r[0], r[1]);
            double Gc[2][6], Gm[2][6], Gf[2][6];
            corner_jacobian<true, true, false>(ec, em, ef, K, g, Gc, Gm, Gf);
#pragma unroll
            for (int rr = 0; rr < 2; rr++) {
#pragma unroll
                for (int i = 0; i < 6; i++) {
                    vals[78 + i] += Gc[rr][i] * r[rr];
                    vals[84 + i] += Gm[rr][i] * r[rr];
#pragma unroll
                    for (int j = 0; j <= i; j++) {
                        vals[i * (i + 1) / 2 + j] += Gc[rr][i] * Gc[rr][j];
                        vals[21 + i * (i + 1) / 2 + j] += Gm[rr][i] * Gm[rr][j];
                    }
#pragma unroll
                    for (int j = 0; j < 6; j++) vals[42 + i * 6 + j] += Gc[rr][i] * Gm[rr][j];
                }
            }
        }
    }
    const int rc = 6 * head.cam, rm = 6 * head.marker;
    wave_sum_lds<90>(vals, scratch + wave * 2048, lane, [&](int v, double s) {
        if (DET) { b.part[(size_t)chunk * b.part_stride + v] = s; return; }
        if (v < 42) {
            const int base = v < 21 ? rc : rm, p = v < 21 ? v : v - 21;
            int i = 0;
            while ((i + 1) * (i + 2) / 2 <= p) i++;
            const int j = p - i * (i + 1) / 2;
            atomicAdd(U0 + (size_t)(base + i) * n_pad + base + j, s);
        } else if (v < 78) {
            const int i = (v - 42) / 6, j = (v - 42) % 6;
            atomicAdd(U0 + (size_t)(rm + j) * n_pad + rc + i, s);
        } else if (v < 84) {
            atomicAdd(g0 + rc + (v - 78), s);
        } else {
            atomicAdd(g0 + rm + (v - 84), s);
        }
    });
}

template <bool DET = false>
__device__ __forceinline__ void passB_wrench_body(const PassBArgs &b, double *scratch, const int first_chunk) {
    __shared__ double pb_red[4][128];
    const ObsIdx *__restrict__ idx = b.idx;
    const float *__restrict__ uv = b.uv;
    const double *__restrict__ ent = b.ent, *__restrict__ Kmat = b.Kmat;
    const int32_t *__restrict__ chunk_start = b.chunk_start;
    const int n_chunks = b.n_chunks, A = b.A, res_f32 = b.res_f32, n_pad = b.n_pad;
    const float huber = b.huber;
    const double h = b.h;
    double *__restrict__ U0 = b.U0, *__restrict__ g0 = b.g0;
    const int lane = threadIdx.x & 63, wave = __builtin_amdgcn_readfirstlane(threadIdx.x >> 6);
    const int chunk = first_chunk + wave;
    if (chunk >= n_chunks) return;
    const int o0 = chunk_start[chunk], o1 = chunk_start[chunk + 1];
    double vals[90];
#pragma unroll
    for (int i = 0; i < 90; i++) vals[i] = 0.0;
    const ObsIdx head = idx[o0];
    Ent ec, em;
    load_ent(ent, head.cam, ec);
    load_ent(ent, head.marker, em);
    double K[9];
#pragma unroll
    for (int i = 0; i < 9; i++) K[i] = Kmat[b.kstride * head.cam + i];
    for (int o = o0 + lane; o < o1; o += 64) {
        const ObsIdx id = idx[o];
        const float4 uv0 = reinterpret_cast<const float4 *>(uv)[2 * (int64_t)o];
        const float4 uv1 = reinterpret_cast<const float4 *>(uv)[2 * (int64_t)o + 1];
        const float ou[8] = {uv0.x, uv0.y, uv0.z, uv0.w, uv1.x, uv1.y, uv1.z, uv1.w};
        EntRT ef;
        load_ent_rt(ent, A + id.frame, ef);
        double H[21], bw[6];
#pragma unroll
        for (int i = 0; i < 21; i++) H[i] = 0.0;
#pragma unroll
        for (int i = 0; i < 6; i++) bw[i] = 0.0;
#pragma unroll
        for (int k = 0; k < 4; k++) {
            CornerGeom g;
            project_corner(ec, em, ef, K, h, k, g);
            double r[2];
            corner_residual(ou[2 * k], ou[2 * k + 1], g.u, g.v, res_f32, huber, r[0], r[1]);
#pragma unroll
            for (int rr = 0; rr < 2; rr++) {
                double w[6];
#pragma unroll
                for (int j = 0; j < 3; j++) w[3 + j] = (K[3 * rr + j] - (rr ? g.v : g.u) * K[6 + j]) * g.iw;
                cross3(g.pc, &w[3], &w[0]);
#pragma unroll
                for (int i = 0; i < 6; i++) {
                    bw[i] += w[i] * r[rr];
#pragma unroll
                    for (int j = 0; j <= i; j++) H[i * (i + 1) / 2 + j] += w[i] * w[j];
                }
            }
        }
        double Q[3][3], E[3][3], e3[3];
        {
            const double d[3] = {ec.t[0] - ef.t[0], ec.t[1] - ef.t[1], ec.t[2] - ef.t[2]};
#pragma unroll
            for (int i = 0; i < 3; i++) {
#pragma unroll
                for (int j = 0; j < 3; j++) Q[i][j] = ef.R[i] * ec.R[j] + ef.R[3 + i] * ec.R[3 + j] + ef.R[6 + i] * ec.R[6 + j];
                e3[i] = ef.R[i] * d[0] + ef.R[3 + i] * d[1] + ef.R[6 + i] * d[2] - em.t[i];
            }
#pragma unroll
            for (int j = 0; j < 3; j++) {
                const double qc[3] = {Q[0][j], Q[1][j], Q[2][j]};
                double x[3];
                cross3(e3, qc, x);
                E[0][j] = x[0]; E[1][j] = x[1]; E[2][j] = x[2];
            }
        }
#pragma unroll
        for (int i = 0; i < 21; i++) vals[i] += H[i];
#pragma unroll
        for (int i = 0; i < 6; i++) vals[78 + i] += bw[i];
#pragma unroll
        for (int i = 0; i < 3; i++) {
            vals[84 + i] += Q[i][0] * bw[0] + Q[i][1] * bw[1] + Q[i][2] * bw[2] + E[i][0] * bw[3] + E[i][1] * bw[4] + E[i][2] * bw[5];
            vals[87 + i] += Q[i][0] * bw[3] + Q[i][1] * bw[4] + Q[i][2] * bw[5];
// ... 171 lines not shown
            atomicAdd(U0 + (size_t)(rk + i) * n_pad + rm + j, s);
        } else {
            atomicAdd(g0 + rk + (v - 58), s);
        }
    });
}

__global__ void __launch_bounds__(256) k_passB_intr(const PassBArgs b) {
    __shared__ double scratch[4 * 2048];
    passB_intr_body(b, scratch, (int)blockIdx.x * 4);
}
__global__ void __launch_bounds__(256) k_passB_intr_det(const PassBArgs b) {
    __shared__ double scratch[4 * 2048];
    passB_intr_body<true>(b, scratch, (int)blockIdx.x * 4);
}

struct PassBReduceArgs {
    const int32_t *start, *chunk, *kind, *ea, *eb;
    const double *part;
    int stride, n_items, n_pad, intr, k_ent0;
    double *U0, *g0;
};
__device__ __forceinline__ void unpack_lower(int p, int &i, int &j) {
    i = 0;
    while ((i + 1) * (i + 2) / 2 <= p) i++;
    j = p - i * (i + 1) / 2;
}
__global__ void __launch_bounds__(256) k_passB_reduce(const PassBReduceArgs r) {
    const int item = (int)blockIdx.x * 4 + (int)(threadIdx.x >> 6), lane = threadIdx.x & 63;
    if (item >= r.n_items) return;
    const int c0 = r.start[item], c1 = r.start[item + 1], kind = r.kind[item];
    const int ea = r.ea[item], eb = r.eb[item];
    const int nv = kind == 0 ? (r.intr ? 65 : 27) : (kind == 1 ? 27 : (r.intr ? 60 : 36));
    for (int v = lane; v < nv; v += 64) {
        int src, i, j;
        double *dst;
        if (kind == 0) {
            const int rc = 6 * ea, rk = 6 * (r.k_ent0 + ea);
            if (v < 21) { src = v; unpack_lower(v, i, j); dst = r.U0 + (size_t)(rc + i) * r.n_pad + rc + j; }
            else if (v < 27) { src = 78 + (v - 21); dst = r.g0 + rc + (v - 21); }
            else if (v < 37) { src = 90 + (v - 27); unpack_lower(v - 27, i, j); dst = r.U0 + (size_t)(rk + i) * r.n_pad + rk + j; }
            else if (v < 61) { src = 90 + 10 + (v - 37); i = (v - 37) / 6; j = (v - 37) % 6; dst = r.U0 + (size_t)(rk + i) * r.n_pad + rc + j; }
            else { src = 90 + 58 + (v - 61); dst = r.g0 + rk + (v - 61); }
        } else if (kind == 1) {
            const int rm = 6 * ea;
            if (v < 21) { src = 21 + v; unpack_lower(v, i, j); dst = r.U0 + (size_t)(rm + i) * r.n_pad + rm + j; }
            else { src = 84 + (v - 21); dst = r.g0 + rm + (v - 21); }
        } else {
            const int rc = 6 * ea, rm = 6 * eb, rk = 6 * (r.k_ent0 + ea);
            if (v < 36) { src = 42 + v; i = v / 6; j = v % 6; dst = r.U0 + (size_t)(rm + j) * r.n_pad + rc + i; }
            else { src = 90 + 34 + (v - 36); i = (v - 36) / 6; j = (v - 36) % 6; dst = r.U0 + (size_t)(rk + i) * r.n_pad + rm + j; }
        }
        double s = 0.0;
        int k = c0;
        for (; k + 8 <= c1; k += 8) {
            double t[8];
#pragma unroll
            for (int u = 0; u < 8; u++) t[u] = r.part[(size_t)r.chunk[k + u] * r.stride + src];
#pragma unroll
            for (int u = 0; u < 8; u++) s += t[u];
        }
        for (; k < c1; k++) s += r.part[(size_t)r.chunk[k] * r.stride + src];
        *dst = s;
    }
}

template <int BLOCK, int CPL, bool WR>
__global__ void __launch_bounds__(BLOCK) k_passA_intr(const PassAArgs a) {
    extern __shared__ double lds[];
    if (WR) passA_wrench_body<BLOCK, CPL, true>(a, lds, (int)blockIdx.x, (int)gridDim.x);
    else passA_body<BLOCK, CPL, true>(a, lds, (int)blockIdx.x, (int)gridDim.x);
}

template <int BLOCK, int CPL, bool WR, bool WRB = WR>
__global__ void __launch_bounds__(BLOCK) k_passAB(const PassAArgs a, const PassBArgs b) {
    extern __shared__ double lds[];
    if ((int)blockIdx.x < a.F) {
        if (WR) passA_wrench_body<BLOCK, CPL>(a, lds, (int)blockIdx.x, a.F);
        else passA_body<BLOCK, CPL>(a, lds, (int)blockIdx.x, a.F);
    } else if (WRB) passB_wrench_body(b, lds, ((int)blockIdx.x - a.F) * (BLOCK / 64));
    else passB_body(b, lds, ((int)blockIdx.x - a.F) * (BLOCK / 64));
}
template <int BLOCK, int CPL>
__global__ void __launch_bounds__(BLOCK, 2) k_passAB_o2(const PassAArgs a, const PassBArgs b) {
    extern __shared__ double lds[];
    if ((int)blockIdx.x < a.F) passA_wrench_body<BLOCK, CPL>(a, lds, (int)blockIdx.x, a.F);
    else passB_body<false, true>(b, lds, ((int)blockIdx.x - a.F) * (BLOCK / 64));
}
template <int BLOCK, int CPL, bool WR>
__global__ void __launch_bounds__(BLOCK) k_passAB_intr(const PassAArgs a, const PassBArgs b, int nb) {
    extern __shared__ double lds[];
    const int blk = (int)blockIdx.x;
    if (blk < a.F) {
        if (WR) passA_wrench_body<BLOCK, CPL, true>(a, lds, blk, a.F);
        else passA_body<BLOCK, CPL, true>(a, lds, blk, a.F);
    }
    else if (blk < a.F + nb) passB_body(b, lds, (blk - a.F) * (BLOCK / 64));
    else passB_intr_body(b, lds, (blk - a.F - nb) * (BLOCK / 64));
}

__global__ void __launch_bounds__(256) k_maxdiag(const double *__restrict__ U0, int n_pad, int A,
                                                 const int32_t *__restrict__ ent_fixed, const double *__restrict__ V,
                                                 int F, int frames_fixed, double *__restrict__ out) {
    double m = -1.7976931348623157e308;
    for (int i = threadIdx.x; i < 6 * A; i += blockDim.x)
        if (!ent_fixed[i / 6]) m = fmax(m, U0[(size_t)i * n_pad + i]);
    if (!frames_fixed)
        for (int i0 = threadIdx.x; i0 < 6 * F; i0 += 8 * (int)blockDim.x) {
            double v[8];
#pragma unroll
            for (int u = 0; u < 8; u++) {
                const int i = i0 + u * (int)blockDim.x;
                v[u] = i < 6 * F ? V[(size_t)(i / 6) * 36 + (i % 6) * 7] : m;
            }
#pragma unroll
            for (int u = 0; u < 8; u++) m = fmax(m, v[u]);
        }
    __shared__ double wm[4];
#pragma unroll
    for (int off = 32; off > 0; off >>= 1) m = fmax(m, __shfl_xor(m, off));
    if ((threadIdx.x & 63) == 0) wm[threadIdx.x >> 6] = m;
    __syncthreads();
    if (threadIdx.x == 0) out[0] = fmax(fmax(wm[0], wm[1]), fmax(wm[2], wm[3]));
}

void launch_unpack(const DeviceProblem &P, int which, hipStream_t st, int zero_blk) {
    const int n_ent = P.A + P.F;
    double *zp = nullptr, *zq = nullptr;
    int64_t zn = 0, zqn = 0;
    int blocks = (n_ent + 255) / 256;
    if (zero_blk >= 0) {
        zp = P.blk[zero_blk].S; zn = (int64_t)P.n_pad * P.n_pad + 2 * (int64_t)P.n_pad;
        zq = P.lin_part; zqn = 2 * (int64_t)(P.F + 1);
        blocks = (int)std::max<int64_t>(blocks, std::min<int64_t>(512, (zn + 2047) / 2048));
    }
    { HookScope _h(P, KID_UNPACK); hipLaunchKernelGGL(k_unpack, dim3(blocks), dim3(256), 0, st, P.z[which], P.ent[which], n_ent,
                                                      P.C + P.M, P.intr ? P.C + P.M + P.C : P.C + P.M, zp, zn, zq, zqn); }
}

void launch_residual(const DeviceProblem &P, int which, double *r_out, hipStream_t st) {
    const int blocks = (int)((P.N + 255) / 256);
    if (blocks == 0) return;
    const KTable kt = k_table(P, which);
    { HookScope _h(P, KID_RESIDUAL); hipLaunchKernelGGL(k_residual, dim3(blocks), dim3(256), 0, st, P.a_idx, P.a_uv, P.ent[which], kt.base, kt.stride, P.N, P.A,
                       P.half_size, P.res_f32, P.huber, r_out, P.err_part); }
}

int residual_blocks(const DeviceProblem &P) { return (int)((P.N + 255) / 256); }

size_t passA_wrench_lds_bytes(int max_kf, bool intr) { return (passA_h_doubles(max_kf, intr ? HLS_INTR : HLS) + 64 + 24 + 72) * sizeof(double); }

size_t passA_lds_bytes(int max_kf, int block) {
    return (passA_w_doubles(max_kf) + 64 + (size_t)(max_kf + 1) * ENT_LDS + (block / 64) * passA_sum_chunk(block) * 64) * sizeof(double);
}

static PassAArgs passA_args(const DeviceProblem &P, int which, double mu_pred, int zero_blk) {
    PassAArgs a;
    a.idx = P.a_idx; a.uv = P.a_uv; a.ent = P.ent[which];
    { const KTable kt = k_table(P, which); a.Kmat = kt.base; a.kstride = kt.stride; }
    a.frame_obs_start = P.frame_obs_start; a.fslot_start = P.fslot_start; a.fslot_ent = P.fslot_ent; a.frame_stride = P.frame_stride;
    a.stamps = nullptr; a.k_ent0 = P.intr ? P.C + P.M : P.A;
#ifdef AAR_PASSA_STAMPS
    {
        static unsigned long long *st = nullptr;
        if (!st && getenv("AAR_STAMPS_A")) {
            (void)hipMalloc(&st, 512 * 16 * 8); (void)hipMemset(st, 0, 512 * 16 * 8);
            static unsigned long long *keep = st;
            atexit([] { std::vector<unsigned long long> h(512 * 16); (void)d2h(h.data(), keep, 512 * 16 * 8, nullptr);
                        FILE *fp = fopen(getenv("AAR_STAMPS_A"), "w"); for (int i = 0; i < 512; i++) { for (int j = 0; j < 16; j++) fprintf(fp, "%llu ", h[i * 16 + j]); fprintf(fp, "\n"); } fclose(fp); });
        }
        a.stamps = st;
    }
#endif
    a.A = P.A; a.F = P.F; a.C = P.C; a.res_f32 = P.res_f32; a.max_kf = P.max_kf; a.frames_fixed = P.frames_fixed;
    a.huber = P.huber;
    a.h = P.half_size; a.mu_pred = mu_pred;
    const DeviceProblem::Blocks &b = P.blk[which];
    a.V = b.V; a.gf = b.gf; a.W = b.W; a.Wf = b.Wf; a.Vinv = b.Vinv; a.hf = b.hf; a.err_part = P.err_part;
    if (b.Wf && !P.want_w64) a.W = nullptr;
    a.zero0 = a.zero1 = a.zero2 = nullptr; a.zero0_n = a.zero1_n = a.zero2_n = 0;
    if (zero_blk >= 0) {
        const DeviceProblem::Blocks &zb = P.blk[zero_blk];
        a.zero0 = zb.S; a.zero0_n = (int64_t)P.n_pad * P.n_pad;
        a.zero1 = zb.rhs; a.zero1_n = P.n_pad;
        a.zero2 = zb.g0; a.zero2_n = P.n_pad;
    }
    a.flags = P.flags;
    a.Wd = a.Yd = nullptr; a.slot_dense = nullptr; a.Ad = 0;
    if (P.n_smwork > 0 && P.dense_from_passA) { a.Wd = P.Wd; a.Yd = P.Yd; a.slot_dense = P.slot_dense; a.Ad = P.Ad; }
    return a;
}

static PassBArgs passB_args(const DeviceProblem &P, int which) {
    PassBArgs b;
    b.idx = P.b_idx; b.uv = P.b_uv; b.ent = P.ent[which]; b.chunk_start = P.chunk_start;
    { const KTable kt = k_table(P, which); b.Kmat = kt.base; b.kstride = kt.stride; }
    b.k_ent0 = P.C + P.M;
    b.n_chunks = P.n_chunks; b.A = P.A; b.res_f32 = P.res_f32; b.n_pad = P.n_pad; b.huber = P.huber; b.h = P.half_size;
    b.U0 = P.blk[which].S; b.g0 = P.blk[which].g0;
    b.part = P.pb_part; b.part_stride = P.pb_stride;
    return b;
}

template <int B, int CPL>
static void launch_passA_t(const DeviceProblem &P, const PassAArgs &a, const PassBArgs *pbargs, hipStream_t st) {
    size_t lds = P.tune.passA_wrench ? passA_wrench_lds_bytes(P.max_kf, P.intr != 0) : passA_lds_bytes(P.max_kf, B);
    if (pbargs) lds = std::max(lds, (size_t)(B / 64) * 2048 * sizeof(double));
    HookScope _h(P, KID_PASSA);
    const int nb = (P.n_chunks + B / 64 - 1) / (B / 64);
    if (P.intr && pbargs) {
        if (P.tune.passA_wrench) launch_lds(k_passAB_intr<B, CPL, true>, dim3(P.F + 2 * nb), dim3(B), lds, st, a, *pbargs, nb);
        else launch_lds(k_passAB_intr<B, CPL, false>, dim3(P.F + 2 * nb), dim3(B), lds, st, a, *pbargs, nb);
    } else if (P.intr) {
        if (P.tune.passA_wrench) launch_lds(k_passA_intr<B, CPL, true>, dim3(P.F), dim3(B), lds, st, a);
        else launch_lds(k_passA_intr<B, CPL, false>, dim3(P.F), dim3(B), lds, st, a);
    } else if (pbargs && P.tune.passA_wrench && !P.tune.passB_wrench_merged &&
               (P.tune.passAB_occ2 >= 0 ? P.tune.passAB_occ2 != 0 : P.F + nb > P.n_cus * 4 / (B / 64))) {
        launch_lds(k_passAB_o2<B, CPL>, dim3(P.F + nb), dim3(B), lds, st, a, *pbargs);
    } else if (pbargs && P.tune.passA_wrench && !P.tune.passB_wrench_merged) {
        launch_lds(k_passAB<B, CPL, true, false>, dim3(P.F + nb), dim3(B), lds, st, a, *pbargs);
    } else if (pbargs && P.tune.passA_wrench) {
        launch_lds(k_passAB<B, CPL, true>, dim3(P.F + nb), dim3(B), lds, st, a, *pbargs);
    } else if (pbargs) {
        launch_lds(k_passAB<B, CPL, false>, dim3(P.F + nb), dim3(B), lds, st, a, *pbargs);
    } else if (P.tune.passA_wrench) {
        launch_lds(k_passA<B, CPL, true>, dim3(P.F), dim3(B), lds, st, a);
    } else {
        launch_lds(k_passA<B, CPL, false>, dim3(P.F), dim3(B), lds, st, a);
    }
}

static void launch_passA_any(const DeviceProblem &P, const PassAArgs &a, const PassBArgs *pbargs, hipStream_t st) {
    const double avg = (double)P.N / (double)P.F;
    if (P.deterministic && avg > 96) return launch_passA_t<64, 4>(P, a, pbargs, st);
    const int var = P.tune.passA_variant;
    if (var == 641) return launch_passA_t<64, 1>(P, a, pbargs, st);
    if (var == 642) return launch_passA_t<64, 2>(P, a, pbargs, st);
    if (var == 644) return launch_passA_t<64, 4>(P, a, pbargs, st);
    if (var == 1281) return launch_passA_t<128, 1>(P, a, pbargs, st);
    if (var == 1282) return launch_passA_t<128, 2>(P, a, pbargs, st);
    if (var == 1284) return launch_passA_t<128, 4>(P, a, pbargs, st);
    if (var == 2564) return launch_passA_t<256, 4>(P, a, pbargs, st);
    if (avg <= 14) launch_passA_t<64, 1>(P, a, pbargs, st);
    else if (avg <= 30) launch_passA_t<64, 2>(P, a, pbargs, st);
    else if (avg <= 96) launch_passA_t<64, 4>(P, a, pbargs, st);
    else launch_passA_t<128, 4>(P, a, pbargs, st);
}

void launch_passA(const DeviceProblem &P, int which, double mu_pred, int zero_blk, hipStream_t st) {
    if (P.F == 0) return;
    launch_passA_any(P, passA_args(P, which, mu_pred, zero_blk), nullptr, st);
}

void launch_passB(const DeviceProblem &P, int which, hipStream_t st) {
    if (P.n_chunks == 0) return;
    if (P.deterministic) {
        HookScope _h(P, KID_PASSB);
        const PassBArgs b = passB_args(P, which);
        if (P.tune.passA_wrench) hipLaunchKernelGGL(k_passB_det<true>, dim3((P.n_chunks + 3) / 4), dim3(256), 0, st, b);
        else hipLaunchKernelGGL(k_passB_det<false>, dim3((P.n_chunks + 3) / 4), dim3(256), 0, st, b);
        if (P.intr) hipLaunchKernelGGL(k_passB_intr_det, dim3((P.n_chunks + 3) / 4), dim3(256), 0, st, b);
        PassBReduceArgs r;
        r.start = P.pbr_start; r.chunk = P.pbr_chunk; r.kind = P.pbr_kind; r.ea = P.pbr_a; r.eb = P.pbr_b; r.part = P.pb_part;
        r.stride = P.pb_stride; r.n_items = P.n_pbr; r.n_pad = P.n_pad; r.intr = P.intr; r.k_ent0 = P.C + P.M; r.U0 = b.U0; r.g0 = b.g0;
        hipLaunchKernelGGL(k_passB_reduce, dim3((P.n_pbr + 3) / 4), dim3(256), 0, st, r);
        return;
    }
    {
        HookScope _h(P, KID_PASSB);
        if (P.tune.passB_lean == 1) hipLaunchKernelGGL(k_passB_lean2, dim3((P.n_chunks + 3) / 4), dim3(256), 0, st, passB_args(P, which));
        else if (P.tune.passB_lean == 2) hipLaunchKernelGGL(k_passB_lean1, dim3((P.n_chunks + 3) / 4), dim3(256), 0, st, passB_args(P, which));
        else if (P.tune.passA_wrench) hipLaunchKernelGGL(k_passB<true>, dim3((P.n_chunks + 3) / 4), dim3(256), 0, st, passB_args(P, which));
        else hipLaunchKernelGGL(k_passB<false>, dim3((P.n_chunks + 3) / 4), dim3(256), 0, st, passB_args(P, which));
    }
    if (P.intr) { HookScope _h(P, KID_PASSB); hipLaunchKernelGGL(k_passB_intr, dim3((P.n_chunks + 3) / 4), dim3(256), 0, st, passB_args(P, which)); }
}

bool launch_passAB(const DeviceProblem &P, int which, double mu_pred, int zero_blk, hipStream_t st) {
    if (P.F == 0 || P.n_chunks == 0 || P.deterministic) return false;
    const int64_t waves = (int64_t)P.F * ((double)P.N / (double)P.F <= 96 ? 1 : 4) + (P.intr ? 2 : 1) * (int64_t)P.n_chunks;
    if (waves > 4096) return false;
    const PassBArgs b = passB_args(P, which);
    launch_passA_any(P, passA_args(P, which, mu_pred, zero_blk), &b, st);
    return true;
}

void launch_maxdiag(const DeviceProblem &P, int which, hipStream_t st) {
    { HookScope _h(P, KID_MAXDIAG); hipLaunchKernelGGL(k_maxdiag, dim3(1), dim3(256), 0, st, P.blk[which].S, P.n_pad, P.A, P.ent_fixed, P.blk[which].V, P.F,
                       P.frames_fixed, P.scal + 4); }
}

}

namespace aar {


__global__ void __launch_bounds__(256) k_track(const TrackArgs a) {
    const int lane = threadIdx.x & 63, f = blockIdx.x * 4 + __builtin_amdgcn_readfirstlane(threadIdx.x >> 6);
    if (f >= a.F) return;
    double z[6];
#pragma unroll
    for (int i = 0; i < 6; i++) z[i] = a.z[6 * (size_t)(a.A + f) + i];
    const double rows = 8.0 * (double)(a.frame_obs_start[f + 1] - a.frame_obs_start[f]);
    double V[21], g[6];
    double currErr = track_eval<true>(a, f, z, lane, V, g), prevErr = currErr;
    double mu = -1.0, v = 2.0;
    int mustExit = 0, iters = 0;
    for (int it = 0; it < a.max_iters && !mustExit && rows > 0; it++) {
        if (it > 0) (void)track_eval<true>(a, f, z, lane, V, g);
        if (mu < 0) {
            double mx = V[0];
#pragma unroll
            for (int i = 1; i < 6; i++) mx = fmax(mx, V[i * (i + 1) / 2 + i]);
            mu = mx * a.tau;
        }
        double gain = 0.0;
        int ntries = 0;
        bool accepted = false;
        do {
            double m[6][6], inv[36], d[6], zt[6];
#pragma unroll
            for (int i = 0; i < 6; i++)
#pragma unroll
                for (int j = 0; j < 6; j++) m[i][j] = V[sym6(i, j)] + (i == j ? mu : 0.0);
            (void)spd6_inverse(m, inv);
            double d2 = 0.0, dg = 0.0;
#pragma unroll
            for (int i = 0; i < 6; i++) {
                double s = 0.0;
#pragma unroll
                for (int j = 0; j < 6; j++) s += inv[i * 6 + j] * g[j];
// ... 47 lines not shown
```

### automatic-ar_amd/csrc/kernels.h

```cpp
#pragma once
#include <hip/hip_runtime.h>
#include <stdint.h>
#include <utility>

namespace aar {

constexpr int CHOL_NB = 96;
constexpr int PASSB_CHUNK = 1024;
constexpr int SPCG_MAX_IT = 128, SPCG_BUFS = SPCG_MAX_IT + 2, SPCG_MAX_NT = 14;
inline int spcg_default_cap(int nT) { return nT <= 4 ? 64 : SPCG_MAX_IT; }
constexpr int PCG_NY = 16;
constexpr int PCG_NYV = 2;
constexpr int PCG_HOP_WORDS = (2 * PCG_NY + 1) * 16;
constexpr double PCG_W32_MIN_ETA = 1e-4;
constexpr double SPCG_ABS_TOL_DEFAULT = 2e-5, PCG_ABS_TOL_DEFAULT = 5e-5;
constexpr double SPCG_ETA_DEFAULT = 3e-4, SPCG_ETA_LOOSE_DEFAULT = 0.0, PCG_ETA_DEFAULT = 5e-3, PCG_ETA_LOOSE_DEFAULT = 0.0;
inline int spcg_stride(int n_pad) { return 8 * (n_pad / 6); }


#ifndef SPCG_PRE
#define SPCG_PRE 0
#endif

enum KernelId { KID_UNPACK = 0, KID_RESIDUAL, KID_PASSA, KID_PASSB, KID_MAXDIAG, KID_FRAME_INV, KID_SCHUR, KID_LDL_DIAG,
// ... 16 lines not shown
    int64_t N = 0;
    int n = 0, n_pad = 0, nT = 0;
    int total_slots = 0, max_kf = 0;
    int n_chunks = 0, n_swork = 0;
    int res_f32 = 1;
    float huber = -1.f;
    double half_size = 0;
    double *K = nullptr;
    ObsIdx *a_idx = nullptr;
    float *a_uv = nullptr;
    int32_t *frame_obs_start = nullptr;
    int32_t *frame_stride = nullptr;
    int32_t *fslot_start = nullptr;
    int32_t *fslot_ent = nullptr;
    ObsIdx *b_idx = nullptr;
    float *b_uv = nullptr;
    int32_t *chunk_start = nullptr;
    int32_t *ent_fixed = nullptr;
    int frames_fixed = 0;
    int32_t *sw_ent = nullptr, *sw_begin = nullptr, *sw_end = nullptr;
    int4 *pair_rec = nullptr;
    int n_smwork = 0;
    int32_t *sm_ga = nullptr, *sm_gb = nullptr, *sm_fb = nullptr, *sm_fe = nullptr, *sm_frames = nullptr;
    int Ad = 0;
    int32_t *slot_dense = nullptr;
    int32_t *slot_frame = nullptr;
    int32_t *dense_ent = nullptr;
    double *Wd = nullptr, *Yd = nullptr;
    int dense_from_passA = 1;
    int deterministic = 0;
    double *pb_part = nullptr;
    int pb_stride = 0, n_pbr = 0;
    int32_t *pbr_start = nullptr, *pbr_chunk = nullptr, *pbr_kind = nullptr, *pbr_a = nullptr, *pbr_b = nullptr;
    double *sp_part = nullptr;
    int64_t *sp_off = nullptr;
    int32_t *se_start = nullptr, *se_items = nullptr;
    int use_pcg = 0, pcg_grid = 0, pcg_max_it = 200;
    double pcg_eta = 0.1;
    double pcg_eta_loose = 0.0, pcg_eta_switch = 0.01, pcg_eta_now = 0.1;
    double pcg_abs_tol = SPCG_ABS_TOL_DEFAULT;
    int pcg_n_items = 0;
    int32_t *pcg_it_ent = nullptr, *pcg_it_begin = nullptr, *pcg_it_end = nullptr, *pcg_ent_item_start = nullptr;
    double *pcg_ws = nullptr;
    int32_t *pcg_counter = nullptr;
    mutable int pcg_parity = 0;
    int n_cus = 256;
    mutable int want_w64 = 0;
    int pcg_fused = 1;
    int pcg_rank0 = 1;
    int pcg_resident = 1;
    int pcg_e_every = 1;
    mutable int pcg_e_age = 0;
    int pcg_coarse = 1, pcg_coarse_from = 8;
    int32_t *up_start = nullptr, *up_ent = nullptr;
    double *pcg_yg = nullptr;
    int32_t *pcg_hop = nullptr;
    int use_spcg = 0, spcg_max_it = 64;
    int spcg_spread = 8;
    int spcg_coarse = 1;
    int spcg_coarse_from = 12;
    mutable int spcg_coarse_on = 0;
    double *spcg_pre = nullptr;
    mutable int spcg_pre_epoch = 0;
    int spcg_root_c = -1, spcg_root_m = -1, spcg_n_free = 0;
    int spcg_test_drop = -1;
    double *spcg_ws = nullptr;
    int32_t *spcg_iters = nullptr;
    mutable int spcg_parity = 0;
    int32_t *spcg_done = nullptr;
    mutable int spcg_epoch = 0;
    double *pcgd_setup = nullptr, *pcgd_minv = nullptr, *pcgd_state = nullptr, *pcgd_y = nullptr, *pcgd_host = nullptr;
    struct Tuning {
        int fused_panel = 3;
        int bs_rides = 1;
        int backsub_rides = 0;
        int lookahead = 1;
        int passA_variant = 0;
        int passAB_occ2 = -1;
        int spcg_backsub_rides = 0;
        int passA_wrench = 1;
        int passB_wrench_merged = 0;
        int passB_lean = 0;
        int pack_system = -1;
        int init_headstart = 1;
    } tune;
    double *z[2] = {nullptr, nullptr};
    double *ent[2] = {nullptr, nullptr};
    struct Blocks {
        double *V = nullptr, *gf = nullptr;
        double *W = nullptr;
        float *Wf = nullptr;
        double *Vinv = nullptr, *hf = nullptr;
        double *S = nullptr;
        double *rhs = nullptr;
        double *g0 = nullptr;
        double *tail = nullptr;
    } blk[2];
    double *Dfac = nullptr;
    double *Linv16 = nullptr;
    double *Lp = nullptr;
    double *zf = nullptr;
    double *delta_s = nullptr;
    int32_t *bs_flags = nullptr;
    mutable int bs_epoch = 0;
    double *err_part = nullptr;
    double *lin_part = nullptr;
    double *scal = nullptr;
    double *host_result = nullptr;
    int32_t *flags = nullptr;
    double *r_out = nullptr;
    int n_prior = 0, prior_rank0 = 1;
    int32_t *prior_ent = nullptr;
    double *prior_dat = nullptr;
    double *prior_out = nullptr;
    LaunchHook hook;
};

void raise_dynamic_lds(const void *kernel, size_t bytes);
template <typename... Params, typename... Args>
inline void launch_lds(void (*kernel)(Params...), dim3 grid, dim3 block, size_t lds, hipStream_t st, Args &&...args) {
    raise_dynamic_lds(reinterpret_cast<const void *>(kernel), lds);
    hipLaunchKernelGGL(kernel, grid, block, lds, st, std::forward<Args>(args)...);
}

struct KTable { const double *base; int stride; };
constexpr int ENT_STRIDE_H = 24;
inline KTable k_table(const DeviceProblem &P, int which) {
    if (P.intr) return KTable{P.ent[which] + (size_t)(P.C + P.M) * ENT_STRIDE_H, ENT_STRIDE_H};
    return KTable{P.K, 9};
}
constexpr int SLOT_C_BITS = 10, SLOT_M_BITS = 11;
inline int pack_slots(int sc, int sm, int sk) { return sc | (sm << SLOT_C_BITS) | (sk << (SLOT_C_BITS + SLOT_M_BITS)); }

extern volatile int g_last_kernel_id;
struct HookScope {
    const DeviceProblem &P;
    int kid;
    HookScope(const DeviceProblem &p, int k) : P(p), kid(k) { g_last_kernel_id = k; if (P.hook.pre) P.hook.pre(P.hook.ctx, kid); }
    ~HookScope() { if (P.hook.post) P.hook.post(P.hook.ctx, kid); }
};

void launch_unpack(const DeviceProblem &P, int which, hipStream_t st, int zero_blk = -1);
void launch_residual(const DeviceProblem &P, int which, double *r_out, hipStream_t st);
void launch_passA(const DeviceProblem &P, int which, double mu_pred, int zero_blk, hipStream_t st);
void launch_passB(const DeviceProblem &P, int which, hipStream_t st);
bool launch_passAB(const DeviceProblem &P, int which, double mu_pred, int zero_blk, hipStream_t st);
size_t passA_lds_bytes(int max_kf, int block);
size_t passA_wrench_lds_bytes(int max_kf, bool intr);
void launch_maxdiag(const DeviceProblem &P, int which, hipStream_t st);
void launch_frame_inv(const DeviceProblem &P, int which, double mu, hipStream_t st, const double *mu_dev = nullptr, double mu_scale = 0.0);
bool launch_schur(const DeviceProblem &P, int which, double sign, hipStream_t st, unsigned long long ride_seq = 0, int ride_n_err = 0,
                  double *ride_scal = nullptr, bool panels_ready = false);
bool launch_chol(const DeviceProblem &P, int which, double mu, hipStream_t st, int trial = -1);
void launch_backsub(const DeviceProblem &P, int cur, int trial, hipStream_t st);
void launch_pcg(const DeviceProblem &P, int which, double mu, hipStream_t st);
size_t pcg_lds_bytes(int A, bool coarse = false);
int pcg_max_grid(int A, bool coarse, int cus);
bool launch_spcg(const DeviceProblem &P, int which, double mu, hipStream_t st, int trial = -1);
int spcg_resident_per_cu(int nT, bool coarse);
inline bool spcg_coarse_now(const DeviceProblem &P) { return P.spcg_coarse && (P.spcg_root_c >= 0 || P.spcg_root_m >= 0); }
bool spcg_fits(int nT);
size_t spcg_ws_doubles(int n_pad);
size_t spcg_pre_doubles(int n_pad);
void spcg_ws_reset(const DeviceProblem &P, hipStream_t st);
void launch_pcgd_setup(const DeviceProblem &P, int which, double mu, hipStream_t st);
void launch_pcgd_iter(const DeviceProblem &P, int which, double mu, int k, bool last, unsigned long long publish_seq, hipStream_t st);
double *pcgd_y_of_launch(const DeviceProblem &P, int k);
void launch_reduce_scalars(const DeviceProblem &P, int n_err, bool fold_shared, unsigned long long publish_seq, hipStream_t st,
                           double *scal_out = nullptr, int maxdiag_blk = -1);
void launch_publish(const DeviceProblem &P, unsigned long long publish_seq, hipStream_t st, const double *src = nullptr, bool flags_reduced = false);
int residual_blocks(const DeviceProblem &P);
constexpr int PRIOR_DAT = 42;
void launch_prior(const DeviceProblem &P, int which, bool add, hipStream_t st);
inline int n_err_terms(const DeviceProblem &P) { return P.F + ((P.n_prior > 0 && P.prior_rank0) ? 1 : 0); }
void launch_track(const DeviceProblem &P, int which, int max_iters, double min_error, double min_step, double min_avg, double tau,
                  int32_t *iters_out, double *err_out, hipStream_t st);

constexpr int SMOOTH_TAIL = 256;
struct SmoothWork {
    double *z[2] = {nullptr, nullptr};
    double *delta = nullptr;
    double *Dg = nullptr, *Of = nullptr;
    double *rhs = nullptr;
    double *Dw = nullptr, *Uw = nullptr, *bw = nullptr, *Dinv = nullptr, *Ls = nullptr;
    double *Ef[2] = {nullptr, nullptr}, *Pe[2] = {nullptr, nullptr};
    double *lin = nullptr;
    double *lam = nullptr;
    double *rel_buf = nullptr;
    const double *rel = nullptr;
    double *res = nullptr;
    int32_t *flag = nullptr;
};
size_t smooth_work_doubles(int F);
void smooth_work_carve(SmoothWork &w, double *base, int F);
void launch_smooth_eval(const DeviceProblem &P, int which, const SmoothWork &w, int cur, bool with_j, hipStream_t st);
int launch_smooth_solve(const SmoothWork &w, int F, double mu, hipStream_t st);

void launch_cov_stage(const double *S, int n_pad, double *S2, int n2, const int32_t *rowmask, hipStream_t st);
void launch_cov_inverse(const double *S2, const double *Dfac, const double *Lp, int n_pad, int n2, int nT2, int fused_m, double *Lc, double *Dinv,
                        double *X, double *Sinv, hipStream_t st);
void launch_cov_diag_blocks(const double *Sinv, int n_pad, int A, double *out, hipStream_t st);
void launch_cov_frames(const DeviceProblem &P, int which, const double *Sinv, const int32_t *rowmask, double *out, hipStream_t st);

constexpr int RR_DIGIT_BITS = 11, RR_BINS = 1 << RR_DIGIT_BITS, RR_PASSES = 6;
struct RRSel {
    unsigned long long prefix, rank;
    double t;
    int pshift, done, single, pad;
};
struct RRWork {
    double *err = nullptr, *ss = nullptr, *fstat = nullptr, *rstat = nullptr, *esum = nullptr, *emax = nullptr, *hd = nullptr;
    uint8_t *keep = nullptr;
    int32_t *perm = nullptr, *run_start = nullptr, *cam_run_start = nullptr, *mk_run_start = nullptr, *mk_runs = nullptr;
    unsigned long long *rmax = nullptr;
    uint32_t *hist = nullptr;
    RRSel *sel = nullptr;
    int R = 0;
};
constexpr int RR_HIST_WORDS = RR_BINS + 3;
void launch_rr_errors(const DeviceProblem &P, int which, const RRWork &w, unsigned long long rank, hipStream_t st);
void launch_rr_select_pass(const DeviceProblem &P, const RRWork &w, hipStream_t st);
void launch_rr_to_double(const RRWork &w, hipStream_t st);
void launch_rr_pick(const RRWork &w, bool reduced, hipStream_t st);
void launch_rr_stats(const DeviceProblem &P, const RRWork &w, int has_rule, double k_median, double min_px, hipStream_t st);

__device__ __forceinline__ double encode_flags(int f) {
    return (double)(f & 1) + 4096.0 * (double)((f >> 1) & 1) + 16777216.0 * (double)((f >> 2) & 1) + 68719476736.0 * (double)((f >> 3) & 1);
}
__device__ __forceinline__ int decode_flags(double v) {
    const long long q = (long long)v;
    return ((q % 4096) ? 1 : 0) | (((q / 4096) % 4096) ? 2 : 0) | (((q / 16777216) % 4096) ? 4 : 0) | ((q / 68719476736LL) ? 8 : 0);
}

__device__ __forceinline__ void publish_host(const double *__restrict__ scal, const int32_t *__restrict__ flags,
                                             double *__restrict__ host, unsigned long long seq, int flags_reduced = 0) {
// ... 10 lines not shown
```

### automatic-ar_amd/csrc/solve_kernels.hip

```cpp
#include <type_traits>
#include "geom.hpp"
#include "kernels.h"
#include "backsub.hpp"

namespace aar {

typedef double dg_acc_t __attribute__((ext_vector_type(4)));

__global__ void __launch_bounds__(256) k_frame_inv(const double *__restrict__ V, const double *__restrict__ gf, int F,
                                                   double mu, int frames_fixed, double *__restrict__ Vinv,
                                                   double *__restrict__ hf, int32_t *__restrict__ flags,
                                                   const double *__restrict__ mu_dev = nullptr, double mu_scale = 0.0) {
    const int f = blockIdx.x * blockDim.x + threadIdx.x;
    if (f >= F) return;
    if (mu_dev) mu = mu_scale * mu_dev[0];
    double out[36];
    if (frames_fixed) {
#pragma unroll
        for (int i = 0; i < 36; i++) out[i] = 0.0;
    } else {
        double a[6][6];
#pragma unroll
        for (int i = 0; i < 6; i++)
#pragma unroll
            for (int j = 0; j < 6; j++) a[i][j] = V[(size_t)f * 36 + i * 6 + j] + (i == j ? mu : 0.0);
        if (!spd6_inverse(a, out)) atomicOr(flags, 1);
    }
#pragma unroll
    for (int i = 0; i < 6; i++) {
        double hv = 0.0;
#pragma unroll
        for (int j = 0; j < 6; j++) {
            Vinv[(size_t)f * 36 + i * 6 + j] = out[i * 6 + j];
            hv += out[i * 6 + j] * gf[(size_t)f * 6 + j];
        }
        hf[(size_t)f * 6 + i] = hv;
    }
}

__global__ void k_publish(const double *__restrict__ scal, const int32_t *__restrict__ flags, double *__restrict__ host,
                          unsigned long long seq, int flags_reduced) {
    if (threadIdx.x == 0) publish_host(scal, flags, host, seq, flags_reduced);
}


struct ReduceArgs {
    const double *err_part; int n_err; const double *lin_part; int F; int fold_shared;
    double *scal; const int32_t *flags; double *host; unsigned long long publish_seq;
    const double *md_U, *md_V; const int32_t *md_fixed; int md_n_pad, md_A, md_frames_fixed;
    const int32_t *cg_iters;
};

__device__ __forceinline__ void reduce_scalars_body(const ReduceArgs &r) {
    __shared__ double red[3][256];
    const int tid = threadIdx.x < 256 ? threadIdx.x : 255;
    const bool act = threadIdx.x < 256;
    double e = 0.0, d2 = 0.0, dg = 0.0;
    if (act) {
    for (int i0 = tid; i0 < r.n_err; i0 += 8 * 256) {
        double v[8];
#pragma unroll
        for (int u = 0; u < 8; u++) v[u] = (i0 + 256 * u < r.n_err) ? r.err_part[i0 + 256 * u] : 0.0;
#pragma unroll
        for (int u = 0; u < 8; u++) e += v[u];
    }
    for (int i0 = tid; i0 < r.F; i0 += 8 * 256) {
        double2 v[8];
#pragma unroll
        for (int u = 0; u < 8; u++) v[u] = (i0 + 256 * u < r.F) ? reinterpret_cast<const double2 *>(r.lin_part)[i0 + 256 * u] : make_double2(0.0, 0.0);
#pragma unroll
        for (int u = 0; u < 8; u++) { d2 += v[u].x; dg += v[u].y; }
    }
    red[0][tid] = e; red[1][tid] = d2; red[2][tid] = dg;
    }
    __syncthreads();
    for (int off = 128; off > 0; off >>= 1) {
        if (act && tid < off) {
            red[0][tid] += red[0][tid + off];
            red[1][tid] += red[1][tid + off];
            red[2][tid] += red[2][tid + off];
        }
        __syncthreads();
    }
    const double sum_e = red[0][0], sum_d2 = red[1][0], sum_dg = red[2][0];
    if (r.md_U) {
        double m = -1.7976931348623157e308;
        if (act) {
            for (int i = tid; i < 6 * r.md_A; i += 256)
                if (!r.md_fixed[i / 6]) m = fmax(m, r.md_U[(size_t)i * r.md_n_pad + i]);
            if (!r.md_frames_fixed)
                for (int i0 = tid; i0 < 6 * r.F; i0 += 8 * 256) {
                    double v[8];
#pragma unroll
                    for (int u = 0; u < 8; u++) { const int i = i0 + u * 256; v[u] = i < 6 * r.F ? r.md_V[(size_t)(i / 6) * 36 + (i % 6) * 7] : m; }
#pragma unroll
                    for (int u = 0; u < 8; u++) m = fmax(m, v[u]);
                }
        }
        __syncthreads();
        if (act) red[1][tid] = m;
        __syncthreads();
        for (int off = 128; off > 0; off >>= 1) {
            if (act && tid < off) red[1][tid] = fmax(red[1][tid], red[1][tid + off]);
            __syncthreads();
        }
    }
    if (act && tid == 0) {
        if (r.md_U) r.scal[4] = red[1][0];
        r.scal[0] = sum_e; r.scal[1] = sum_d2;
        r.scal[2] = sum_dg + (r.fold_shared ? r.lin_part[2 * (size_t)r.F + 1] : 0.0);
        r.scal[3] = encode_flags(r.flags[0] | r.flags[1] | r.flags[2] | r.flags[3]);
        r.scal[5] = r.lin_part[2 * (size_t)r.F]; r.scal[6] = r.lin_part[2 * (size_t)r.F + 1];
        r.scal[7] = r.cg_iters ? (double)r.cg_iters[0] : -1.0;
        if (r.publish_seq) publish_host(r.scal, r.flags, r.host, r.publish_seq);
    }
}

__global__ void __launch_bounds__(256) k_reduce_scalars(const ReduceArgs r) { reduce_scalars_body(r); }

template <int PRE, int NW = 4>
__global__ void __launch_bounds__(64 * NW) k_schur(const int32_t *__restrict__ sw_ent, const int32_t *__restrict__ sw_begin,
                                               const int32_t *__restrict__ sw_end, const int4 *__restrict__ pair_rec,
                                               const int32_t *__restrict__ fslot_ent, const double *__restrict__ W,
                                               const double *__restrict__ Vinv, const double *__restrict__ hf, int A,
                                               int n_pad, double sign, double *__restrict__ S, double *__restrict__ rhs,
                                               int rider, const ReduceArgs red, double *__restrict__ part = nullptr,
                                               const int64_t *__restrict__ part_off = nullptr) {
    if (rider && blockIdx.x == 0) {
        reduce_scalars_body(red);
        return;
    }
    extern __shared__ __align__(16) double lds[];
    double *panel = lds;
    double *pg = lds + (size_t)A * 36;
    double *ysc = pg + 8;
    const int w = (int)blockIdx.x - rider, tid = threadIdx.x, lane = tid & 63, wave = __builtin_amdgcn_readfirstlane(tid >> 6);
    const int a = sw_ent[w], pb = sw_begin[w], pe = sw_end[w];
    for (int i = tid; i < (a + 1) * 36; i += 64 * NW) panel[i] = 0.0;
    if (tid < 8) pg[tid] = 0.0;
    __syncthreads();
    double *ys = ysc + wave * 48;
    if constexpr (PRE == 0) {
        for (int p = pb + wave; p < pe; p += NW) {
            const int4 rec = pair_rec[p];
            const int f = rec.x, sg = rec.y, s0 = rec.z, sa = sg - s0;
            const double *Wa = W + (size_t)sg * 36;
            if (lane < 36) {
                const int i = lane / 6, j = lane % 6;
                double y = 0.0;
    #pragma unroll
                for (int k = 0; k < 6; k++) y += Wa[i * 6 + k] * Vinv[(size_t)f * 36 + k * 6 + j];
                ys[lane] = y;
            } else if (lane < 42) {
                const int i = lane - 36;
                double y = 0.0;
    #pragma unroll
                for (int k = 0; k < 6; k++) y += Wa[i * 6 + k] * hf[(size_t)f * 6 + k];
                atomicAdd(pg + i, y);
            }
            __builtin_amdgcn_fence(__ATOMIC_RELEASE, "wavefront");
            __builtin_amdgcn_wave_barrier();
            double Y[36];
    #pragma unroll
            for (int i = 0; i < 18; i++) { const double2 v2 = reinterpret_cast<const double2 *>(ys)[i]; Y[2 * i] = v2.x; Y[2 * i + 1] = v2.y; }
            __builtin_amdgcn_wave_barrier();
            const int sl = lane / 6, j = lane % 6;
            if (lane < 60) {
                for (int sb = sl; sb <= sa; sb += 10) {
                    const int b = fslot_ent[s0 + sb];
                    const double2 *wr = reinterpret_cast<const double2 *>(W + (size_t)(s0 + sb) * 36 + j * 6);
                    const double2 w0 = wr[0], w1 = wr[1], w2 = wr[2];
                    double *dst = panel + b * 36 + j;
    #pragma unroll
                    for (int i = 0; i < 6; i++) {
                        const double v = Y[i * 6] * w0.x + Y[i * 6 + 1] * w0.y + Y[i * 6 + 2] * w1.x + Y[i * 6 + 3] * w1.y +
                                         Y[i * 6 + 4] * w2.x + Y[i * 6 + 5] * w2.y;
                        atomicAdd(dst + i * 6, v);
                    }
                }
            }
        }
    } else {
        const int sl = lane / 6, j = lane % 6;
        int4 rec = make_int4(0, 0, 0, 0);
        if (pb + wave < pe) rec = pair_rec[pb + wave];
        for (int p = pb + wave; p < pe; p += NW) {
            const int f = rec.x, sg = rec.y, s0 = rec.z, sa = sg - s0;
            if (p + NW < pe) rec = pair_rec[p + NW];
            const double *Wa = W + (size_t)sg * 36;
            double wa[6], vv[6];
            if (lane < 36) {
                const int i = lane / 6, jj = lane % 6;
    #pragma unroll
                for (int k = 0; k < 6; k++) { wa[k] = Wa[i * 6 + k]; vv[k] = Vinv[(size_t)f * 36 + k * 6 + jj]; }
            } else if (lane < 42) {
                const int i = lane - 36;
    #pragma unroll
                for (int k = 0; k < 6; k++) { wa[k] = Wa[i * 6 + k]; vv[k] = hf[(size_t)f * 6 + k]; }
            }
            int bm[PRE > 0 ? PRE : 1];
            double2 wr[PRE > 0 ? PRE : 1][3];
    #pragma unroll
            for (int m = 0; m < PRE; m++) {
                const int sb = sl + 10 * m;
                bm[m] = -1;
                if (lane < 60 && sb <= sa) {
                    bm[m] = fslot_ent[s0 + sb];
                    const double2 *q = reinterpret_cast<const double2 *>(W + (size_t)(s0 + sb) * 36 + j * 6);
                    wr[m][0] = q[0]; wr[m][1] = q[1]; wr[m][2] = q[2];
                }
            }
            if (lane < 42) {
                double y = 0.0;
    #pragma unroll
                for (int k = 0; k < 6; k++) y += wa[k] * vv[k];
                if (lane < 36) ys[lane] = y;
                else atomicAdd(pg + (lane - 36), y);
            }
            __builtin_amdgcn_fence(__ATOMIC_RELEASE, "wavefront");
            __builtin_amdgcn_wave_barrier();
            double Y[36];
    #pragma unroll
            for (int i = 0; i < 18; i++) { const double2 v2 = reinterpret_cast<const double2 *>(ys)[i]; Y[2 * i] = v2.x; Y[2 * i + 1] = v2.y; }
            __builtin_amdgcn_wave_barrier();
            auto accumulate = [&](int b, const double2 &w0, const double2 &w1, const double2 &w2) {
                double *dst = panel + b * 36 + j;
    #pragma unroll
                for (int i = 0; i < 6; i++) {
                    const double v = Y[i * 6] * w0.x + Y[i * 6 + 1] * w0.y + Y[i * 6 + 2] * w1.x + Y[i * 6 + 3] * w1.y +
                                     Y[i * 6 + 4] * w2.x + Y[i * 6 + 5] * w2.y;
                    atomicAdd(dst + i * 6, v);
                }
            };
    #pragma unroll
            for (int m = 0; m < PRE; m++)
                if (bm[m] >= 0) accumulate(bm[m], wr[m][0], wr[m][1], wr[m][2]);
            if (lane < 60) {
                for (int sb = sl + 10 * PRE; sb <= sa; sb += 10) {
                    const int b = fslot_ent[s0 + sb];
                    const double2 *q = reinterpret_cast<const double2 *>(W + (size_t)(s0 + sb) * 36 + j * 6);
                    accumulate(b, q[0], q[1], q[2]);
                }
            }
        }
    }
    __syncthreads();
    if (part) {
        double *rec = part + part_off[w];
        for (int idx = tid; idx < (a + 1) * 36; idx += 64 * NW) rec[idx] = panel[idx];
        if (tid < 6) rec[(a + 1) * 36 + tid] = pg[tid];
        return;
    }
    for (int idx = tid; idx < (a + 1) * 36; idx += 64 * NW) {
        const double v = panel[idx];
        if (v != 0.0) {
            const int b = idx / 36, e = idx - b * 36, i = e / 6, j = e - i * 6;
            atomicAdd(S + (size_t)(6 * a + i) * n_pad + 6 * b + j, -sign * v);
        }
    }
    if (tid < 6) atomicAdd(rhs + 6 * a + tid, -sign * pg[tid]);
}

__global__ void __launch_bounds__(256) k_schur_reduce(const int32_t *__restrict__ se_start, const int32_t *__restrict__ se_items,
                                                      const int64_t *__restrict__ part_off, const double *__restrict__ part, int n_pad,
                                                      double sign, double *__restrict__ S, double *__restrict__ rhs) {
    const int a = blockIdx.x, i0 = se_start[a], i1 = se_start[a + 1], np = (a + 1) * 36;
    for (int idx = threadIdx.x; idx < np + 6; idx += 256) {
        double s = 0.0;
        int k = i0;
        for (; k + 8 <= i1; k += 8) {
            double t[8];
#pragma unroll
            for (int u = 0; u < 8; u++) t[u] = part[part_off[se_items[k + u]] + idx];
#pragma unroll
            for (int u = 0; u < 8; u++) s += t[u];
        }
        for (; k < i1; k++) s += part[part_off[se_items[k]] + idx];
        if (idx < np) {
            const int b = idx / 36, e = idx - b * 36, i = e / 6, j = e - i * 6;
            S[(size_t)(6 * a + i) * n_pad + 6 * b + j] -= sign * s;
        } else {
            rhs[6 * a + (idx - np)] -= sign * s;
        }
    }
}

__global__ void __launch_bounds__(256) k_schur_fill(const int32_t *__restrict__ slot_frame, const int32_t *__restrict__ slot_dense,
                                                    const double *__restrict__ W, const double *__restrict__ Vinv,
                                                    const double *__restrict__ gf, int total_slots, int F, int Ad,
                                                    double *__restrict__ Wd, double *__restrict__ Yd, int rider, const ReduceArgs red) {
    if (rider && blockIdx.x == 0) {
        reduce_scalars_body(red);
        return;
    }
    const int64_t gid = (int64_t)((int)blockIdx.x - rider) * 256 + threadIdx.x;
    if (gid >= (int64_t)total_slots * 6) {
        const int64_t q = gid - (int64_t)total_slots * 6;
        if (q < (int64_t)F * 6) Wd[(q / 6) * Ad * 36 + (q % 6)] = gf[q];
        return;
    }
    const int64_t sl = gid / 6;
    const int i = (int)(gid - sl * 6);
    const int f = slot_frame[sl];
    const double2 *wp = reinterpret_cast<const double2 *>(W + sl * 36 + i * 6);
    const double2 w0 = wp[0], w1 = wp[1], w2 = wp[2];
    const double w[6] = {w0.x, w0.y, w1.x, w1.y, w2.x, w2.y};
    double y[6] = {0, 0, 0, 0, 0, 0};
#pragma unroll
    for (int k = 0; k < 6; k++) {
        const double2 *vp = reinterpret_cast<const double2 *>(Vinv + (size_t)f * 36 + k * 6);
        const double2 v0 = vp[0], v1 = vp[1], v2 = vp[2];
        y[0] = fma(w[k], v0.x, y[0]); y[1] = fma(w[k], v0.y, y[1]); y[2] = fma(w[k], v1.x, y[2]);
        y[3] = fma(w[k], v1.y, y[3]); y[4] = fma(w[k], v2.x, y[4]); y[5] = fma(w[k], v2.y, y[5]);
    }
    const size_t o = ((size_t)f * Ad + slot_dense[sl]) * 36 + i * 6;
    double2 *yp = reinterpret_cast<double2 *>(Yd + o), *wd = reinterpret_cast<double2 *>(Wd + o);
    yp[0] = make_double2(y[0], y[1]); yp[1] = make_double2(y[2], y[3]); yp[2] = make_double2(y[4], y[5]);
    wd[0] = w0; wd[1] = w1; wd[2] = w2;
}

#ifndef AAR_SM_FPS
#define AAR_SM_FPS 4
#endif
constexpr int SM_GA = 16, SM_GB = 32, SM_AR = 6 * SM_GA, SM_BR = 6 * SM_GB, SM_ROWS = SM_AR + SM_BR, SM_FPS = AAR_SM_FPS, SM_PS = 6 * SM_FPS + 2,
              SM_DEPTH = 8 / SM_FPS, SM_KT = 6 * SM_FPS / 4;
static_assert((6 * SM_FPS) % 4 == 0 && SM_DEPTH >= 1, "whole MFMA k-steps per barrier");
__global__ void __launch_bounds__(512) k_schur_mfma(const int32_t *__restrict__ w_ga, const int32_t *__restrict__ w_gb,
                                                    const int32_t *__restrict__ w_fb, const int32_t *__restrict__ w_fe,
                                                    const int32_t *__restrict__ flist, const int32_t *__restrict__ dense_ent, const double *__restrict__ Wd,
                                                    const double *__restrict__ Yd, int Ad, int n_pad, double sign,
                                                    double *__restrict__ S, double *__restrict__ rhs, int rider, const ReduceArgs red) {
    extern __shared__ __align__(16) double stage[];
    if (rider && blockIdx.x == 0) {
        reduce_scalars_body(red);
        return;
    }
    const int w = (int)blockIdx.x - rider, tid = threadIdx.x, lane = tid & 63, wave = __builtin_amdgcn_readfirstlane(tid >> 6);
    const int ga = w_ga[w], gb = w_gb[w], fb = w_fb[w], fe = w_fe[w];
    const int lr = lane >> 4, lc = lane & 15;
    constexpr int SM_PIECES = SM_ROWS * 3 * SM_FPS, SM_PPT = (SM_PIECES + 511) / 512;
    int p_lds[SM_PPT], p_off[SM_PPT];
    unsigned sideA = 0;
    auto piece_ff = [&](int u) -> int { const int q = tid + 512 * u; return q >= SM_PIECES ? -1 : q / (SM_ROWS * 3); };
#pragma unroll
    for (int u = 0; u < SM_PPT; u++) {
// ... 963 lines not shown
    double a[RPT], vl[NL];
    auto fetch_block = [&](int t) {
#pragma unroll
        for (int k = 0; k < RPT; k++) {
            const int i = gq + G * k;
            a[k] = (gq < G && i < NB) ? lcol[(size_t)(t * NB + i) * lld + j] : 0.0;
        }
    };
    fetch_block(nT - 1);
#pragma unroll
    for (int u = 0; u < NL; u++) {
        const int e = tid + 1024 * u, i = e / NB, jj = e - i * NB;
        vl[u] = (jj < i) ? dd[e] : 0.0;
    }
    double acc = 0.0;
    for (int t = nT - 1; t > s; t--) {
        if (t < nT - 1) {
            if (tid == 0 && !hop_wait(flag + t, epoch)) atomicOr(err_flags, 4);
            __syncthreads();
        }
        if (tid < NB) xs[tid] = __hip_atomic_load(x + t * NB + tid, __ATOMIC_RELAXED, __HIP_MEMORY_SCOPE_AGENT);
        __syncthreads();
#pragma unroll
        for (int k = 0; k < RPT; k++) {
            const int i = gq + G * k;
            if (i < NB) acc = fma(a[k], xs[i], acc);
        }
        if (t - 1 > s) fetch_block(t - 1);
        if (t == nT - 1) {
#pragma unroll
            for (int u = 0; u < NL; u++) {
                const int e = tid + 1024 * u, i = e / NB, jj = e - i * NB;
                Ls[i * LD + jj] = vl[u];
            }
        }
        __syncthreads();
    }
    if (gq < G) part[gq * NB + j] = acc;
    __syncthreads();
    if (tid < NB) {
        double v = zsrc[r0 + tid];
#pragma unroll
        for (int g = 0; g < G; g++) v -= part[g * NB + tid];
        w[tid] = v;
    }
    __syncthreads();
    if (wave == 0) {
        const int i0 = lane, i1 = lane + 64;
        const bool h1 = i1 < NB;
        double b0 = w[i0], b1 = h1 ? w[i1] : 0.0;
        const int i1c = h1 ? i1 : 0;
#pragma unroll
        for (int jj = NB - 1; jj > 0; jj--) {
            const double v = jj < 64 ? b0 : b1;
            const int lo = __builtin_amdgcn_readlane(__double2loint(v), jj & 63), hi = __builtin_amdgcn_readlane(__double2hiint(v), jj & 63);
            const double xj = __hiloint2double(hi, lo);
            b0 = fma(-Ls[jj * LD + i0], xj, b0);
            if (jj > 64) b1 = fma(-Ls[jj * LD + i1c], xj, b1);
        }
        __hip_atomic_store(x + r0 + i0, b0, __ATOMIC_RELAXED, __HIP_MEMORY_SCOPE_AGENT);
        if (h1) __hip_atomic_store(x + r0 + i1, b1, __ATOMIC_RELAXED, __HIP_MEMORY_SCOPE_AGENT);
        hop_publish(flag + s, epoch, lane == 0);
    }
}


void launch_frame_inv(const DeviceProblem &P, int which, double mu, hipStream_t st, const double *mu_dev, double mu_scale) {
    if (P.F == 0) return;
    const DeviceProblem::Blocks &b = P.blk[which];
    { HookScope _h(P, KID_FRAME_INV); hipLaunchKernelGGL(k_frame_inv, dim3((P.F + 255) / 256), dim3(256), 0, st, b.V, b.gf, P.F, mu, P.frames_fixed, b.Vinv, b.hf, P.flags,
                                                         mu_dev, mu_scale); }
}

static ReduceArgs reduce_args(const DeviceProblem &P, int n_err, bool fold_shared, unsigned long long publish_seq, double *scal_out = nullptr) {
    ReduceArgs r;
    r.err_part = P.err_part; r.n_err = n_err; r.lin_part = P.lin_part; r.F = P.F; r.fold_shared = fold_shared ? 1 : 0;
    r.scal = scal_out ? scal_out : P.scal; r.flags = P.flags; r.host = P.host_result; r.publish_seq = publish_seq;
    r.md_U = r.md_V = nullptr; r.md_fixed = nullptr; r.md_n_pad = r.md_A = r.md_frames_fixed = 0;
    r.cg_iters = P.use_spcg ? P.spcg_iters : nullptr;
    return r;
}

bool launch_schur(const DeviceProblem &P, int which, double sign, hipStream_t st, unsigned long long ride_seq, int ride_n_err, double *ride_scal,
                  bool panels_ready) {
    const DeviceProblem::Blocks &b = P.blk[which];
    if (P.n_smwork > 0) {
        const size_t lds = (size_t)2 * SM_ROWS * SM_PS * sizeof(double);
        const ReduceArgs red = reduce_args(P, ride_n_err, false, ride_scal ? 0ull : ride_seq, ride_scal);
        const int extra = (ride_seq || ride_scal) ? 1 : 0;
        HookScope _h(P, KID_SCHUR);
        if (!panels_ready)
            hipLaunchKernelGGL(k_schur_fill, dim3((unsigned)(((int64_t)P.total_slots * 6 + (int64_t)P.F * 6 + 255) / 256) + extra), dim3(256), 0, st, P.slot_frame, P.slot_dense,
                               b.W, b.Vinv, b.gf, P.total_slots, P.F, P.Ad, P.Wd, P.Yd, extra, red);
        const int extra_m = panels_ready ? extra : 0;
        launch_lds(k_schur_mfma, dim3(P.n_smwork + extra_m), dim3(512), lds, st, P.sm_ga, P.sm_gb, P.sm_fb, P.sm_fe, P.sm_frames, P.dense_ent, P.Wd, P.Yd, P.Ad, P.n_pad, sign,
                   b.S, b.rhs, extra_m, red);
        return extra != 0;
    }
    if (P.n_swork == 0) return false;
    if (P.deterministic) {
        const size_t lds1 = ((size_t)P.A * 36 + 8 + 48) * sizeof(double);
        HookScope _h(P, KID_SCHUR);
        launch_lds(k_schur<0, 1>, dim3(P.n_swork), dim3(64), lds1, st, P.sw_ent, P.sw_begin, P.sw_end, P.pair_rec, P.fslot_ent, b.W, b.Vinv, b.hf, P.A, P.n_pad, sign,
                   b.S, b.rhs, 0, ReduceArgs(), P.sp_part, P.sp_off);
        hipLaunchKernelGGL(k_schur_reduce, dim3(P.A), dim3(256), 0, st, P.se_start, P.se_items, P.sp_off, P.sp_part, P.n_pad, sign, b.S, b.rhs);
        return false;
    }
    const size_t lds = ((size_t)P.A * 36 + 8 + 4 * 48) * sizeof(double);
    const ReduceArgs red = reduce_args(P, ride_n_err, false, ride_scal ? 0ull : ride_seq, ride_scal);
    const int extra = (ride_seq || ride_scal) ? 1 : 0;
    HookScope _h(P, KID_SCHUR);
    launch_lds(P.max_kf > 64 ? k_schur<3> : k_schur<0>, dim3(P.n_swork + extra), dim3(256), lds, st, P.sw_ent, P.sw_begin, P.sw_end, P.pair_rec, P.fslot_ent, b.W, b.Vinv, b.hf,
               P.A, P.n_pad, sign, b.S, b.rhs, extra, red, nullptr, nullptr);
    return extra != 0;
}

BacksubArgs backsub_args(const DeviceProblem &P, int cur, int trial, int waves_per_block) {
    const DeviceProblem::Blocks &b = P.blk[cur];
    BacksubArgs a;
    a.fslot_start = P.fslot_start; a.fslot_ent = P.fslot_ent; a.W = b.W; a.Vinv = b.Vinv; a.gf = b.gf; a.g0 = b.g0;
    a.Wf = P.use_pcg ? b.Wf : nullptr;
    a.delta_s = P.delta_s; a.zc = P.z[cur]; a.zt = P.z[trial]; a.A = P.A; a.F = P.F;
    a.n_frame_blocks = (P.F + waves_per_block - 1) / waves_per_block;
    a.lin_part = P.lin_part; a.ent_out = P.ent[trial]; a.k_ent0 = P.intr ? P.C + P.M : P.A;
    return a;
}

bool launch_chol(const DeviceProblem &P, int which, double mu, hipStream_t st, int trial) {
    const DeviceProblem::Blocks &b = P.blk[which];
    const size_t lds_diag = ((size_t)NB * (NB + 2) + 2 * NB * DG_YS + (size_t)NB * (NB / 2 + 2)) * sizeof(double);
    const int fused_m = P.tune.fused_panel;
    const bool bs_rides = P.tune.bs_rides != 0;
    const bool backsub_rides = P.tune.backsub_rides != 0;
    const bool lookahead = P.tune.lookahead != 0;
    bool rode_backsub = false;
    int upd_s = -1;
    for (int s = 0; s < P.nT; s++) {
        const int m = P.nT - s - 1;
        const bool last = s == P.nT - 1;
        const bool ride = bs_rides && last && (P.nT == 2 || P.nT == 3);
        const bool ride2 = backsub_rides && last && trial >= 0 && (P.nT == 1 || ride) && !P.hook.pre;
        BacksubArgs ba = backsub_args(P, which, trial >= 0 ? trial : which, DG_THREADS / 64);
        if (ride || ride2) P.bs_epoch++;
        const int grid = 1 + (ride ? 1 : 0) + (ride2 ? ba.n_frame_blocks + 1 : 0) + (upd_s >= 0 ? ldl_update_riders(P.nT - upd_s - 1) : 0);
        { HookScope _h(P, KID_LDL_DIAG); launch_lds(k_ldl_diag, dim3(grid), dim3(DG_THREADS), lds_diag, st, b.S, P.Dfac, P.Linv16, P.n_pad, P.n, s, mu, P.ent_fixed, P.flags,
                                                 P.nT, b.rhs, b.g0, P.delta_s, P.Lp, P.zf, fused_m, P.bs_flags, P.bs_epoch, ride ? 1 : 0, ride2 ? 1 : 0, ba,
                                                 upd_s, b.S, b.rhs); }
        upd_s = -1;
        rode_backsub = ride2;
        if (m > 0 && m <= fused_m) {
            const int ns = NSB * m;
            HookScope _h(P, KID_LDL_PANEL);
            hipLaunchKernelGGL(k_ldl_panel, dim3(ns * (ns + 1) / 2 + ns), dim3(128), 0, st, b.S, b.rhs, b.g0, P.Dfac, P.Linv16, P.n_pad, P.n, s, P.nT, mu, P.ent_fixed, P.Lp, P.zf);
        } else if (m > 0) {
            { HookScope _h(P, KID_LDL_TRSM); hipLaunchKernelGGL(k_ldl_trsm, dim3(NSB * m + 1), dim3(64), 0, st, b.S, b.rhs, b.g0, P.Dfac, P.Linv16, P.n_pad, P.n, s, P.nT, mu, P.ent_fixed); }
            if (lookahead && m >= 2) upd_s = s;
            else { HookScope _h(P, KID_LDL_UPDATE); hipLaunchKernelGGL(k_ldl_update, dim3(m * (m + 1) / 2 * 9 + m), dim3(256), 0, st, b.S, b.rhs, b.g0, P.Dfac, P.n_pad, P.n, s, P.nT, mu, P.ent_fixed); }
        }
    }
    if (P.nT > 1 && !(bs_rides && P.nT <= 3)) {
        const size_t lds = ((size_t)NB * (NB + 2) + 2 * NB + 10 * NB) * sizeof(double);
        P.bs_epoch++;
        HookScope _h(P, KID_LDL_BACKSOLVE);
        launch_lds(k_ldl_backsolve, dim3(P.nT - 1), dim3(1024), lds, st, b.S, b.rhs, P.Dfac, P.delta_s, P.n_pad, P.nT, P.bs_flags, P.bs_epoch, P.flags, P.Lp, P.zf, fused_m);
    }
    return rode_backsub;
}

void launch_backsub(const DeviceProblem &P, int cur, int trial, hipStream_t st) {
    const BacksubArgs ba = backsub_args(P, cur, trial, 4);
    { HookScope _h(P, KID_BACKSUB); hipLaunchKernelGGL(k_backsub, dim3(ba.n_frame_blocks + 1), dim3(256), 0, st, ba); }
}

void launch_reduce_scalars(const DeviceProblem &P, int n_err, bool fold_shared, unsigned long long publish_seq, hipStream_t st, double *scal_out, int maxdiag_blk) {
    ReduceArgs r = reduce_args(P, n_err, fold_shared, publish_seq, scal_out);
    if (maxdiag_blk >= 0) {
        r.md_U = P.blk[maxdiag_blk].S; r.md_V = P.blk[maxdiag_blk].V; r.md_fixed = P.ent_fixed; r.md_n_pad = P.n_pad; r.md_A = P.A; r.md_frames_fixed = P.frames_fixed;
    }
    { HookScope _h(P, KID_REDUCE); hipLaunchKernelGGL(k_reduce_scalars, dim3(1), dim3(256), 0, st, r); }
}

void launch_publish(const DeviceProblem &P, unsigned long long publish_seq, hipStream_t st, const double *src, bool flags_reduced) {
    hipLaunchKernelGGL(k_publish, dim3(1), dim3(64), 0, st, src ? src : P.scal, P.flags, P.host_result, publish_seq, flags_reduced ? 1 : 0);
}

}
```

### include/aar.h

```cpp
#ifndef AAR_H
#define AAR_H
#include <stdint.h>

#ifdef __cplusplus
extern "C" {
#endif

typedef enum aar_status {
    AAR_OK = 0,
    AAR_ERR_INVALID = -1,
    AAR_ERR_NO_DEVICE = -2,
    AAR_ERR_HIP = -3,
    AAR_ERR_UNSUPPORTED = -4,
    AAR_ERR_NUMERIC = -5,
    AAR_ERR_IO = -6,
    AAR_ERR_COMM = -7
} aar_status;

const char *aar_last_error(void);

typedef struct aar_dataset {
    int32_t num_cams, num_markers, num_frames;
    int32_t root_cam, root_marker;
    int32_t *cam_ids;
// ... 75 lines not shown
    int32_t n_excluded;
    const int32_t *excluded_cams;
    int32_t device_id;
} aar_init_params;
void aar_init_default_params(aar_init_params *);
int aar_initializer_run(const aar_detections *, const aar_cam_model *cams, int32_t n_cams, const aar_init_params *,
                        aar_dataset **out);
int aar_initializer_object_poses(const aar_dataset *solution, const aar_detections *, const aar_cam_model *cams, int32_t n_cams,
                                 const aar_init_params *, aar_dataset **out);

void aar_rodrigues_vec2mat(const double w[3], double R[9]);
void aar_rodrigues_mat2vec(const double R[9], double w[3]);

int aar_plan_shards(int32_t num_frames, const int64_t *obs_per_frame, int32_t world, int32_t *begin);

typedef struct aar_comm aar_comm;
#define AAR_COMM_ID_BYTES 128
int aar_comm_make_id(char id[AAR_COMM_ID_BYTES]);
int aar_comm_create(const char id[AAR_COMM_ID_BYTES], int32_t world_size, int32_t rank, int32_t device_id,
                    aar_comm **out);
void aar_comm_destroy(aar_comm *);
typedef struct aar_comm_stats {
    int32_t world_size, rank, ranks_seen;
    int64_t allreduce_calls, allreduce_bytes, system_allreduce_bytes;
} aar_comm_stats;
int aar_comm_get_stats(const aar_comm *, aar_comm_stats *out);
typedef struct aar_local_group aar_local_group;
int aar_local_group_create(int32_t world_size, aar_local_group **out);
void aar_local_group_destroy(aar_local_group *);
int aar_comm_create_local(aar_local_group *group, int32_t rank, int32_t device_id, aar_comm **out);

typedef struct aar_problem aar_problem;

enum { AAR_RES_F32 = 0,
       AAR_RES_F64 = 1 };

typedef struct aar_problem_desc {
    int32_t num_cams, num_markers, num_frames;
    int32_t root_cam, root_marker;
    const double *cam_mats;
    double marker_size;
    int64_t num_obs;
    const int32_t *obs_frame, *obs_cam, *obs_marker;
    const float *obs_uv;
    int32_t optimize_cam_poses, optimize_marker_poses, optimize_object_poses;
    int32_t optimize_cam_intrinsics;
    int32_t residual_mode;
    int32_t with_huber;
    int32_t device_id;
    aar_comm *comm;
} aar_problem_desc;

void aar_problem_desc_from_dataset(const aar_dataset *, aar_problem_desc *);
int aar_problem_create(const aar_problem_desc *, aar_problem **out);

enum { AAR_SOLVER_DIRECT = 0, AAR_SOLVER_PCG = 1, AAR_SOLVER_SPCG = 2, AAR_SOLVER_AUTO = 3 };
typedef struct aar_solver_options {
    uint32_t struct_size;
    int32_t solver;
    int32_t deterministic;
    int32_t pcg_max_it;
    double pcg_eta;
    double pcg_eta_loose;
    double pcg_eta_switch;
    double pcg_abs_tol;
} aar_solver_options;
void aar_solver_default_options(aar_solver_options *);
int aar_problem_create_ex(const aar_problem_desc *, const aar_solver_options *, aar_problem **out);
enum { AAR_ENV_SOLVER = 1, AAR_ENV_DETERMINISTIC = 2, AAR_ENV_PCG_ETA = 4, AAR_ENV_PCG_MAX_IT = 8 };
typedef struct aar_solver_stats {
    uint32_t struct_size;
    int32_t solver;
    int32_t deterministic;
    int32_t last_iterations;
    int64_t total_iterations, solves;
    int64_t fallbacks;
    double pcg_eta;
    int32_t pcg_max_it;
    int32_t env_overrides;
    int64_t same_xcd_solves;
    double pcg_eta_loose;
    double pcg_eta_switch;
    double pcg_abs_tol;
} aar_solver_stats;
int aar_problem_get_solver_stats(aar_problem *, aar_solver_stats *out);
enum { AAR_TEST_HOOK_SPCG_DROP = 1 };
int aar_problem_set_test_hook(aar_problem *, int32_t hook, int32_t value);
void aar_problem_destroy(aar_problem *);
int64_t aar_problem_full_len(const aar_problem *);
int64_t aar_problem_num_vars(const aar_problem *);
int64_t aar_problem_local_obs(const aar_problem *);
int aar_problem_set_huber_delta(aar_problem *, float delta);
float aar_problem_get_huber_delta(const aar_problem *);

int aar_eval_residuals(aar_problem *, const double *x_full, double *r, double *sum_sq);

int aar_eval_normal_equations(aar_problem *, const double *x_full, double *JtJ, double *B, double *sum_sq);

int aar_eval_damped_step(aar_problem *, const double *x_full, double mu, double *delta);

typedef struct aar_covariance_report {
    uint32_t struct_size;
    int64_t num_residuals;
    int64_t num_vars;
    double sum_sq;
    double sigma2;
    double min_pivot, max_pivot;
    int32_t frames_written;
} aar_covariance_report;
int aar_problem_covariance(aar_problem *, const double *x_full, double *entity_cov, double *entity_diag, double *frame_cov,
                           aar_covariance_report *report);
int aar_covariance_write_yaml(const char *path, const aar_dataset *d, const double *entity_diag, const double *frame_cov, double sigma2);

typedef struct aar_outlier_rule {
    uint32_t struct_size;
    double k_median;
    double min_px;
} aar_outlier_rule;
typedef struct aar_residual_report {
    uint32_t struct_size;
    int64_t num_detections, num_rejected, num_nonfinite;
    double sum_sq, rmse;
    double median, max, threshold;
    int32_t cams_emptied, markers_emptied, frames_emptied;
} aar_residual_report;
int aar_problem_residual_report(aar_problem *, const double *x_full, const aar_outlier_rule *rule, double *det_err, uint8_t *keep,
                                double *cam_stats, double *marker_stats, double *frame_stats, aar_residual_report *report);
int aar_dataset_select_observations(const aar_dataset *d, const uint8_t *keep, aar_dataset **out);
int aar_residual_report_write_yaml(const char *path, const aar_dataset *d, const double *cam_stats, const double *marker_stats,
                                   const double *det_err, const uint8_t *keep, const aar_residual_report *report);

enum { AAR_PRIOR_CAMERA = 0, AAR_PRIOR_MARKER = 1 };
typedef struct aar_pose_prior {
    int32_t kind;
    int32_t index;
    double x6[6];
    double info[36];
} aar_pose_prior;
typedef struct aar_problem_constraints {
    uint32_t struct_size;
    int32_t n_fixed_cams;
    const int32_t *fixed_cams;
    int32_t n_fixed_markers;
    const int32_t *fixed_markers;
    int32_t n_priors;
    const aar_pose_prior *priors;
} aar_problem_constraints;
int aar_problem_constraints_validate(const aar_problem_desc *, const aar_problem_constraints *);
int aar_problem_create_constrained(const aar_problem_desc *, const aar_solver_options *options, const aar_problem_constraints *constraints,
                                   aar_problem **out);
int32_t aar_problem_num_priors(const aar_problem *);
int aar_problem_eval_priors(aar_problem *, const double *x_full, double *e_out, double *cost);

typedef struct aar_lm_params {
    int32_t max_iters;
    double min_error;
    double min_step_error_diff;
    double min_average_step_error_diff;
    double tau;
    int32_t verbose;
} aar_lm_params;
void aar_lm_default_params(aar_lm_params *);

typedef struct aar_lm_iter {
    double err, mu, gain, delta_norm;
    int32_t accepted, tries;
} aar_lm_iter;

typedef struct aar_lm_report {
// ... 66 lines not shown
```

Measured before the change: 13380.

## Fuse back-substitution into pass-A and ride pass-B on the Schur kernel

```diff
diff --git a/automatic-ar_amd/aar/__init__.py b/automatic-ar_amd/aar/__init__.py
--- a/automatic-ar_amd/aar/__init__.py
+++ b/automatic-ar_amd/aar/__init__.py
@@ -38,6 +38,7 @@
 PRIOR_KINDS = {"camera": PRIOR_CAMERA, "marker": PRIOR_MARKER}
 SOLVER_DIRECT, SOLVER_PCG, SOLVER_SPCG, SOLVER_AUTO = 0, 1, 2, 3
 TEST_HOOK_SPCG_DROP = 1
+TEST_HOOK_FUSED_CHECK = 2
 ENV_SOLVER, ENV_DETERMINISTIC, ENV_PCG_ETA, ENV_PCG_MAX_IT = 1, 2, 4, 8
 SOLVERS = {"direct": SOLVER_DIRECT, "pcg": SOLVER_PCG, "spcg": SOLVER_SPCG, "auto": SOLVER_AUTO}
 SOLVER_NAMES = {v: k for k, v in SOLVERS.items()}
@@ -94,7 +95,8 @@
     _fields_ = [("struct_size", C.c_uint32), ("solver", C.c_int32), ("deterministic", C.c_int32), ("last_iterations", C.c_int32),
                 ("total_iterations", C.c_int64), ("solves", C.c_int64), ("fallbacks", C.c_int64), ("pcg_eta", C.c_double),
                 ("pcg_max_it", C.c_int32), ("env_overrides", C.c_int32), ("same_xcd_solves", C.c_int64), ("pcg_eta_loose", C.c_double),
-                ("pcg_eta_switch", C.c_double), ("pcg_abs_tol", C.c_double)]
+                ("pcg_eta_switch", C.c_double), ("pcg_abs_tol", C.c_double), ("fused_steps", C.c_int64),
+                ("fused_check_values", C.c_int64), ("fused_check_mismatches", C.c_int64)]
 
 
 class CCovarianceReport(C.Structure):
@@ -1026,7 +1028,8 @@
         _check(lib().aar_problem_get_solver_stats(self.handle, C.byref(st)))
         return dict(solver=SOLVER_NAMES[st.solver], deterministic=bool(st.deterministic), last_iterations=st.last_iterations,
                     total_iterations=st.total_iterations, solves=st.solves, fallbacks=st.fallbacks, pcg_eta=st.pcg_eta, pcg_max_it=st.pcg_max_it,
-                    same_xcd_solves=st.same_xcd_solves, pcg_eta_loose=st.pcg_eta_loose, pcg_eta_switch=st.pcg_eta_switch, pcg_abs_tol=st.pcg_abs_tol, env_overrides=st.env_overrides)
+                    same_xcd_solves=st.same_xcd_solves, pcg_eta_loose=st.pcg_eta_loose, pcg_eta_switch=st.pcg_eta_switch, pcg_abs_tol=st.pcg_abs_tol, env_overrides=st.env_overrides,
+                    fused_steps=st.fused_steps, fused_check_values=st.fused_check_values, fused_check_mismatches=st.fused_check_mismatches)
 
     def set_test_hook(self, hook, value):
         _check(lib().aar_problem_set_test_hook(self.handle, int(hook), int(value)))
diff --git a/automatic-ar_amd/csrc/ba_capi.hip b/automatic-ar_amd/csrc/ba_capi.hip
--- a/automatic-ar_amd/csrc/ba_capi.hip
+++ b/automatic-ar_amd/csrc/ba_capi.hip
@@ -218,6 +218,11 @@
     bool overlap = false;
     bool merge_passes = true;
     int64_t trial_points = 0, launches = 0;
+    int64_t fused_steps = 0;
+    bool fused_check = false;
+    int64_t fused_check_values = 0, fused_check_mismatches = 0;
+    std::vector<double> fused_check_ref, fused_check_got;
+    bool constrained = false;
     aar_stage_times times;
     bool stage_timers = false;
     hipEvent_t ev[2] = {nullptr, nullptr};
@@ -676,19 +681,51 @@
     pb->s_reduced = false;
     pb->trial_reduced = false;
     bool backsub_rode = false;
+    const bool fused = P.tune.fused_step != 0 && evaluate_trial && !pb->comm && !P.use_pcg && !chol_done && !P.deterministic && P.tune.passA_wrench && !P.tune.passB_wrench_merged &&
+                       pb->merge_passes && !P.intr && P.n_prior == 0 && !pb->constrained && P.n_smwork == 0 && P.n_swork > 0 && P.A < 96 && P.F > 0 && P.n_chunks > 0 &&
+                       !pb->stage_timers && (int64_t)P.F * ((double)P.N / (double)P.F <= 96 ? 1 : 4) + (int64_t)P.n_chunks <= 4096;
+    const int ride_b = !fused ? 0 : (P.tune.fused_step == 2 ? 2 : (P.tune.fused_step == 3 ? 1 : (P.n_swork + 1 + (P.n_chunks + 3) / 4 > P.n_cus ? 2 : 1)));
     if (P.use_spcg && !pb->force_direct && pb->spcg_skip > 0) pb->spcg_skip--;
     if (!chol_done) {
         StageTimer t(pb, &pb->times.chol);
-        if (by_cg) backsub_rode = launch_spcg(P, cur, mu, pb->stream, pb->stage_timers ? -1 : tr);
-        else backsub_rode = launch_chol(P, cur, mu, pb->stream, pb->stage_timers ? -1 : tr);
-    }
-    if (!backsub_rode) {
+        if (by_cg) backsub_rode = launch_spcg(P, cur, mu, pb->stream, (pb->stage_timers || fused) ? -1 : tr);
+        else backsub_rode = launch_chol(P, cur, mu, pb->stream, (pb->stage_timers || fused) ? -1 : tr);
+    }
+    if (!backsub_rode && !fused) {
         StageTimer t(pb, &pb->times.backsub);
         launch_backsub(P, cur, tr, pb->stream);
     }
-    pb->launches += 2 + 3 * P.nT;
+    pb->launches += (fused ? 1 : 2) + 3 * P.nT;
     pb->blocks_valid = false;
-    if (evaluate_trial) {
+    if (fused) {
+        if (pb->panels_blk == tr) pb->panels_blk = -1;
+        const size_t chk_n[3] = {(size_t)6 * (P.A + P.F), (size_t)(P.A + P.F) * ENT_STRIDE_H, (size_t)2 * (P.F + 1)};
+        double *const chk_p[3] = {P.z[tr], P.ent[tr], P.lin_part};
+        auto chk_fetch = [&](std::vector<double> &v) -> int {
+            v.resize(chk_n[0] + chk_n[1] + chk_n[2]);
+            size_t o = 0;
+            for (int k = 0; k < 3; k++) { int rc = copy_d2h(pb, v.data() + o, chk_p[k], chk_n[k] * sizeof(double)); if (rc) return rc; o += chk_n[k]; }
+            return AAR_OK;
+        };
+        if (pb->fused_check) {
+            launch_backsub(P, cur, tr, pb->stream);
+            int rc = chk_fetch(pb->fused_check_ref);
+            if (rc) return rc;
+            for (int k = 0; k < 3; k++) HIP_TRY(hipMemsetAsync(chk_p[k], 0xFF, chk_n[k] * sizeof(double), pb->stream));
+        }
+        launch_passA_fused(P, cur, tr, mu * 0.33, pb->stream);
+        pb->launches += 1;
+        pb->fused_steps++;
+        int rc = check_async("normal-equation kernels");
+        if (rc) return rc;
+        if (pb->fused_check) {
+            if ((rc = chk_fetch(pb->fused_check_got))) return rc;
+            pb->fused_check_values += (int64_t)pb->fused_check_ref.size();
+            for (size_t i = 0; i < pb->fused_check_ref.size(); i++)
+                if (memcmp(&pb->fused_check_ref[i], &pb->fused_check_got[i], sizeof(double)) != 0) pb->fused_check_mismatches++;
+        }
+        pb->trial_points++;
+    } else if (evaluate_trial) {
         int rc = eval_blocks(pb, tr, mu * 0.33, cur, false, true);
         if (rc) return rc;
         pb->trial_points++;
@@ -701,7 +738,7 @@
         if ((rc = launch_scalars(pb, n_err_terms(P)))) return rc;
     } else if (evaluate_trial && !pb->comm) {
         StageTimer t(pb, &pb->times.schur);
-        rode = launch_schur(P, tr, 1.0, pb->stream, pb->seq + 1, n_err_terms(P), nullptr, panels_ok(pb, tr, mu * 0.33));
+        rode = launch_schur(P, tr, 1.0, pb->stream, pb->seq + 1, n_err_terms(P), nullptr, panels_ok(pb, tr, mu * 0.33), ride_b);
         panels_now(pb, tr, mu * 0.33);
         pb->launches += 1;
         if (rode) pb->seq++;
@@ -1142,6 +1179,8 @@
         return fail(set_error(AAR_ERR_HIP, "second stream / events could not be created"));
     { const char *e = getenv("AAR_OVERLAP"); pb->overlap = (e && e[0] == '1'); }
     { const char *e = getenv("AAR_MERGE_PASSES"); if (e) pb->merge_passes = (e[0] != '0'); }
+    { const char *e = getenv("AAR_FUSED_STEP"); if (e) pb->P.tune.fused_step = atoi(e); }
+    pb->constrained = cons != nullptr;
     { const char *e = getenv("AAR_FUSED_COMM"); if (e) pb->fused_comm = (e[0] != '0'); }
     { const char *e = getenv("AAR_SPEC_CHOL"); if (e) pb->spec_chol = (e[0] != '0'); }
 
@@ -2638,6 +2677,9 @@
     st.pcg_abs_tol = pb->P.pcg_abs_tol;
     st.env_overrides = pb->env_overrides;
     st.fallbacks = pb->spcg_fallbacks;
+    st.fused_steps = pb->fused_steps;
+    st.fused_check_values = pb->fused_check_values;
+    st.fused_check_mismatches = pb->fused_check_mismatches;
     if (pb->P.use_pcg || pb->P.use_spcg) {
         int32_t c[8] = {0, 0, 0, 0, 0, 0, 0, 0};
         HIP_TRY(hipSetDevice(pb->device));
@@ -2656,6 +2698,7 @@
 int aar_problem_set_test_hook(aar_problem *pb, int32_t hook, int32_t value) {
     if (!pb) return set_error(AAR_ERR_INVALID, "aar_problem_set_test_hook: null argument");
     if (hook == AAR_TEST_HOOK_SPCG_DROP) { pb->P.spcg_test_drop = value; return AAR_OK; }
+    if (hook == AAR_TEST_HOOK_FUSED_CHECK) { pb->fused_check = value != 0; return AAR_OK; }
     return set_error(AAR_ERR_INVALID, "aar_problem_set_test_hook: unknown hook %d", hook);
 }
 
diff --git a/automatic-ar_amd/csrc/backsub.hpp b/automatic-ar_amd/csrc/backsub.hpp
--- a/automatic-ar_amd/csrc/backsub.hpp
+++ b/automatic-ar_amd/csrc/backsub.hpp
@@ -28,8 +28,50 @@
     int k_ent0;
 };
 
+template <class DL, class WAIT>
+__device__ __forceinline__ void backsub_shared(const BacksubArgs &b, double *red, DL dl, WAIT wait, int vthreads = 0) {
+    const int tid = threadIdx.x, lane = tid & 63, wave = __builtin_amdgcn_readfirstlane(tid >> 6), nwaves = blockDim.x >> 6;
+    const int vt = vthreads ? vthreads : (int)blockDim.x, nv = vt >> 6;
+    wait();
+    for (int vw = wave; vw < nv; vw += nwaves) {
+        double d2 = 0.0, dg = 0.0;
+        for (int i = vw * 64 + lane; i < 6 * b.A; i += vt) {
+            const double d = dl(i);
+            b.zt[i] = b.zc[i] + d;
+            d2 += d * d;
+            dg += d * b.g0[i];
+        }
+#pragma unroll
+        for (int off = 32; off > 0; off >>= 1) { d2 += __shfl_xor(d2, off); dg += __shfl_xor(dg, off); }
+        if (lane == 0) { red[vw] = d2; red[16 + vw] = dg; }
+    }
+    __syncthreads();
+    if (tid == 0) {
+        double s2 = 0.0, sg = 0.0;
+        for (int w = 0; w < nv; w++) { s2 += red[w]; sg += red[16 + w]; }
+        b.lin_part[2 * (size_t)b.F] = s2;
+        b.lin_part[2 * (size_t)b.F + 1] = sg;
+    }
+    __threadfence_block();
+    __syncthreads();
+    for (int e = tid; e < b.A; e += blockDim.x) {
+        if (e >= b.k_ent0) make_k_row(b.zt + 6 * (size_t)e, b.ent_out + (size_t)e * ENT_STRIDE);
+        else make_ent_row(b.zt + 6 * (size_t)e, b.ent_out + (size_t)e * ENT_STRIDE);
+    }
+}
+
+__device__ __forceinline__ void backsub_shared_row(const BacksubArgs &b, int e, double *row) {
+    double z6[6];
+#pragma unroll
+    for (int i = 0; i < 6; i++) z6[i] = b.zc[6 * (size_t)e + i] + b.delta_s[6 * (size_t)e + i];
+    make_ent_row(z6, row);
+}
+
+template <class DL, class WAIT>
+__device__ __forceinline__ void backsub_frame(const BacksubArgs &b, int f, bool live, double *row_out, DL dl, WAIT wait);
+
 __device__ __forceinline__ void backsub_body(const BacksubArgs &b, int blk, double *red, const int32_t *flag, int epoch, int32_t *err_flags) {
-    const int tid = threadIdx.x, lane = tid & 63, wave = __builtin_amdgcn_readfirstlane(tid >> 6), nwaves = blockDim.x >> 6;
+    const int tid = threadIdx.x, wave = __builtin_amdgcn_readfirstlane(tid >> 6), nwaves = blockDim.x >> 6;
     auto dl = [&](int i) -> double {
         return flag ? __hip_atomic_load(b.delta_s + i, __ATOMIC_RELAXED, __HIP_MEMORY_SCOPE_AGENT) : b.delta_s[i];
     };
@@ -38,35 +80,14 @@
         if (tid == 0 && !hop_wait(flag, epoch)) atomicOr(err_flags, 4);
         __syncthreads();
     };
-    if (blk == b.n_frame_blocks) {
-        wait();
-        double d2 = 0.0, dg = 0.0;
-        for (int i = tid; i < 6 * b.A; i += blockDim.x) {
-            const double d = dl(i);
-            b.zt[i] = b.zc[i] + d;
-            d2 += d * d;
-            dg += d * b.g0[i];
-        }
-#pragma unroll
-        for (int off = 32; off > 0; off >>= 1) { d2 += __shfl_xor(d2, off); dg += __shfl_xor(dg, off); }
-        if (lane == 0) { red[wave] = d2; red[16 + wave] = dg; }
-        __syncthreads();
-        if (tid == 0) {
-            double s2 = 0.0, sg = 0.0;
-            for (int w = 0; w < nwaves; w++) { s2 += red[w]; sg += red[16 + w]; }
-            b.lin_part[2 * (size_t)b.F] = s2;
-            b.lin_part[2 * (size_t)b.F + 1] = sg;
-        }
-        __threadfence_block();
-        __syncthreads();
-        for (int e = tid; e < b.A; e += blockDim.x) {
-            if (e >= b.k_ent0) make_k_row(b.zt + 6 * (size_t)e, b.ent_out + (size_t)e * ENT_STRIDE);
-            else make_ent_row(b.zt + 6 * (size_t)e, b.ent_out + (size_t)e * ENT_STRIDE);
-        }
-        return;
-    }
+    if (blk == b.n_frame_blocks) { backsub_shared(b, red, dl, wait); return; }
     const int f = blk * nwaves + wave;
-    const bool live = f < b.F;
+    backsub_frame(b, f, f < b.F, f < b.F ? b.ent_out + (size_t)(b.A + f) * ENT_STRIDE : nullptr, dl, wait);
+}
+
+template <class DL, class WAIT>
+__device__ __forceinline__ void backsub_frame(const BacksubArgs &b, int f, bool live, double *row_out, DL dl, WAIT wait) {
+    const int lane = threadIdx.x & 63;
     const int s0 = live ? b.fslot_start[f] : 0, s1 = live ? b.fslot_start[f + 1] : 0;
     const int sl = s0 + lane;
     const bool has = sl < s1;
@@ -146,7 +167,7 @@
         double zv[6];
 #pragma unroll
         for (int i = 0; i < 6; i++) zv[i] = __shfl(zn, i);
-        if (lane == 0) make_ent_row(zv, b.ent_out + (size_t)(b.A + f) * ENT_STRIDE);
+        if (lane == 0) make_ent_row(zv, row_out);
     }
     double d2 = (lane < 6) ? d * d : 0.0;
     double dgv = 0.0;
diff --git a/automatic-ar_amd/csrc/eval_kernels.hip b/automatic-ar_amd/csrc/eval_kernels.hip
--- a/automatic-ar_amd/csrc/eval_kernels.hip
+++ b/automatic-ar_amd/csrc/eval_kernels.hip
@@ -5,37 +5,13 @@
 #include "hostcopy.h"
 #include "wave.hpp"
 #include "track_eval.hpp"
+#include "passb.hpp"
+#include "backsub.hpp"
 
 namespace aar {
 
 volatile int g_last_kernel_id = -1;
 
-template <int NV, int CH = 32, class Sink>
-__device__ __forceinline__ void wave_sum_lds(const double (&vals)[NV], double *__restrict__ sc, int lane, Sink sink) {
-    constexpr int L = 64 / CH;
-    constexpr int SPREAD = 32 / CH > 0 ? 32 / CH : 1;
-#pragma unroll
-    for (int base = 0; base < NV; base += CH) {
-        const int cnt = (NV - base) < CH ? (NV - base) : CH;
-#pragma unroll
-        for (int i = 0; i < CH; i++)
-            if (i < cnt) sc[i * 64 + lane] = vals[base + i];
-        __builtin_amdgcn_fence(__ATOMIC_RELEASE, "wavefront");
-        __builtin_amdgcn_wave_barrier();
-        const int vi = lane / L, part = lane % L;
-        double s = 0;
-        if (vi < cnt) {
-            const double *row = sc + lane * CH;
-#pragma unroll 8
-            for (int k = 0; k < CH; k++) s += row[(k + lane / SPREAD) & (CH - 1)];
-        }
-#pragma unroll
-        for (int off = 1; off < L; off <<= 1) s += __shfl_xor(s, off);
-        if (part == 0 && vi < cnt) sink(base + vi, s);
-        __builtin_amdgcn_wave_barrier();
-        __builtin_amdgcn_fence(__ATOMIC_ACQUIRE, "wavefront");
-    }
-}
 
 __global__ void k_unpack(const double *__restrict__ z, double *__restrict__ ent, int n_ent, int k0, int k1, double *__restrict__ zero_p, int64_t zero_n,
                          double *__restrict__ zero_q, int64_t zero_qn) {
@@ -321,8 +297,9 @@
 #define PA_STAMP(n) do { } while (0)
 #endif
 
-template <int BLOCK, int CPL, bool INTR = false>
-__device__ __forceinline__ void passA_wrench_body(const PassAArgs &a, double *lds, const int f, const int n_blocks_a) {
+template <int BLOCK, int CPL, bool INTR = false, bool FUSED = false>
+__device__ __forceinline__ void passA_wrench_body(const PassAArgs &a, double *lds, const int f, const int n_blocks_a, const BacksubArgs *bsp = nullptr) {
+    static_assert(!(FUSED && INTR), "the fused step has no intrinsics variant");
     constexpr int SL = INTR ? HLS_INTR : HLS;
     double *Hl = lds;
     double *acc = lds + passA_h_doubles(a.max_kf, SL);
@@ -330,12 +307,13 @@
     double *frow = acc + 64;
     double *Yl = frow + 24;
     double *vil = Yl + 36;
+    double *entl = vil + 36;
     const int tid = threadIdx.x, lane = tid & 63, wave = tid >> 6;
     const int o0 = a.frame_obs_start[f], nobs = a.frame_obs_start[f + 1] - o0;
     const int s0 = a.fslot_start[f], kf = a.fslot_start[f + 1] - s0;
     PA_STAMP(0);
     Ent ef;
-    load_ent(a.ent, a.A + __builtin_amdgcn_readfirstlane(f), ef);
+    if (!FUSED) load_ent(a.ent, a.A + __builtin_amdgcn_readfirstlane(f), ef);
     constexpr int LPO = 4 / CPL;
     const int stride = a.frame_stride[f];
     const int part = tid % LPO;
@@ -357,18 +335,38 @@
         for (int kk = 0; kk < CPL; kk++) ouv[kk] = reinterpret_cast<const float2 *>(a.uv)[4 * (int64_t)o + part * CPL + kk];
     };
     auto fetch_rows = [&]() {
-        load_ent_rt(a.ent, id.cam, ec);
-        load_ent_rt(a.ent, id.marker, em);
+        if (FUSED) {
+            const double *rc = entl + (id.slots & ((1 << SLOT_C_BITS) - 1)) * ENT_LDS, *rm = entl + ((id.slots >> SLOT_C_BITS) & ((1 << SLOT_M_BITS) - 1)) * ENT_LDS;
+#pragma unroll
+            for (int i = 0; i < 9; i++) { ec.R[i] = rc[i]; em.R[i] = rm[i]; }
+#pragma unroll
+            for (int i = 0; i < 3; i++) { ec.t[i] = rc[9 + i]; em.t[i] = rm[9 + i]; }
+        } else {
+            load_ent_rt(a.ent, id.cam, ec);
+            load_ent_rt(a.ent, id.marker, em);
+        }
 #pragma unroll
         for (int i = 0; i < 9; i++) K[i] = a.Kmat[a.kstride * id.cam + i];
     };
     if (have) fetch_obs();
     const int e_slot = tid < kf ? a.fslot_ent[s0 + tid] : -1;
     double2 frv = make_double2(0.0, 0.0);
-    if (tid < ENT_STRIDE / 2) frv = reinterpret_cast<const double2 *>(a.ent + (size_t)(a.A + f) * ENT_STRIDE)[tid];
+    if (!FUSED && tid < ENT_STRIDE / 2) frv = reinterpret_cast<const double2 *>(a.ent + (size_t)(a.A + f) * ENT_STRIDE)[tid];
+    if (FUSED) {
+        const BacksubArgs &bs = *bsp;
+        if (e_slot >= 0) backsub_shared_row(bs, e_slot, entl + tid * ENT_LDS);
+        for (int ts = tid + BLOCK; ts < kf; ts += BLOCK) backsub_shared_row(bs, a.fslot_ent[s0 + ts], entl + ts * ENT_LDS);
+        if (wave == 0) {
+            backsub_frame(bs, __builtin_amdgcn_readfirstlane(f), true, frow, [&](int i) -> double { return bs.delta_s[i]; }, [] {});
+            __builtin_amdgcn_fence(__ATOMIC_RELEASE, "wavefront");
+            __builtin_amdgcn_wave_barrier();
+            __builtin_amdgcn_fence(__ATOMIC_ACQUIRE, "wavefront");
+            if (lane < ENT_STRIDE) bs.ent_out[(size_t)(bs.A + f) * ENT_STRIDE + lane] = lane < 21 ? frow[lane] : 0.0;
+        }
+    }
     for (int i = tid; i < kf * SL; i += BLOCK) Hl[i] = 0.0;
     for (int i = tid; i < 64; i += BLOCK) acc[i] = 0.0;
-    if (have) fetch_rows();
+    if (!FUSED && have) fetch_rows();
     {
         const int64_t gid = (int64_t)f * BLOCK + tid, gstride = (int64_t)n_blocks_a * BLOCK;
         for (int64_t i = gid; i < a.zero0_n; i += gstride) a.zero0[i] = 0.0;
@@ -377,6 +375,17 @@
     }
     __syncthreads();
     PA_STAMP(1);
+    if (FUSED) {
+        auto uni = [&](int i) -> double {
+            const double v = frow[i];
+            return __hiloint2double(__builtin_amdgcn_readfirstlane(__double2hiint(v)), __builtin_amdgcn_readfirstlane(__double2loint(v)));
+        };
+#pragma unroll
+        for (int i = 0; i < 9; i++) { ef.R[i] = uni(i); ef.Jl[i] = uni(12 + i); }
+#pragma unroll
+        for (int i = 0; i < 3; i++) ef.t[i] = uni(9 + i);
+        if (have) fetch_rows();
+    }
 
     double vals[7];
 #pragma unroll
@@ -440,15 +449,24 @@
     }
     PA_STAMP(2);
     double2 rv[7];
+    auto slot_row = [&](int ts, int e) {
+        if (FUSED) {
+            const double *rowl = entl + ts * ENT_LDS + 8;
+#pragma unroll
+            for (int i = 0; i < 7; i++) rv[i] = make_double2(rowl[2 * i], rowl[2 * i + 1]);
+        } else {
+            const double2 *rowp = reinterpret_cast<const double2 *>(a.ent + (size_t)e * ENT_STRIDE);
+#pragma unroll
+            for (int i = 0; i < 7; i++) rv[i] = rowp[4 + i];
+        }
+    };
     if (e_slot >= 0) {
-        const double2 *rowp = reinterpret_cast<const double2 *>(a.ent + (size_t)e_slot * ENT_STRIDE);
-#pragma unroll
-        for (int i = 0; i < 7; i++) rv[i] = rowp[4 + i];
+        slot_row(tid, e_slot);
         if (e_slot < a.C) atomicAdd(hacc + 30, 1.0);
     }
     for (int ts = tid + BLOCK; ts < kf; ts += BLOCK)
         if (a.fslot_ent[s0 + ts] < a.C) atomicAdd(hacc + 30, 1.0);
-    if (tid < ENT_STRIDE / 2) { frow[2 * tid] = frv.x; frow[2 * tid + 1] = frv.y; }
+    if (!FUSED && tid < ENT_STRIDE / 2) { frow[2 * tid] = frv.x; frow[2 * tid + 1] = frv.y; }
 #pragma unroll
     for (int i = 0; i < 7; i++) {
         const double sv = wave_sum_dpp(vals[i]);
@@ -522,9 +540,7 @@
         int e = e_slot;
         if (ts != tid) {
             e = a.fslot_ent[s0 + ts];
-            const double2 *rowp = reinterpret_cast<const double2 *>(a.ent + (size_t)e * ENT_STRIDE);
-#pragma unroll
-            for (int i = 0; i < 7; i++) rv[i] = rowp[4 + i];
+            slot_row(ts, e);
         }
         if (INTR && e >= a.k_ent0) {
             const double *mk = Hl + ts * SL;
@@ -636,94 +652,6 @@
     }
 }
 
-struct PassBArgs {
-    const ObsIdx *idx; const float *uv; const double *ent; const double *Kmat; const int32_t *chunk_start;
-    int kstride, k_ent0;
-    int n_chunks, A, res_f32, n_pad;
-    float huber;
-    double h;
-    double *U0, *g0;
-    double *part; int part_stride;
-};
-
-template <bool DET = false, bool LEAN = false>
-__device__ __forceinline__ void passB_body(const PassBArgs &b, double *scratch, const int first_chunk) {
-    const ObsIdx *__restrict__ idx = b.idx;
-    const float *__restrict__ uv = b.uv;
-    const double *__restrict__ ent = b.ent, *__restrict__ Kmat = b.Kmat;
-    const int32_t *__restrict__ chunk_start = b.chunk_start;
-    const int n_chunks = b.n_chunks, A = b.A, res_f32 = b.res_f32, n_pad = b.n_pad;
-    const float huber = b.huber;
-    const double h = b.h;
-    double *__restrict__ U0 = b.U0, *__restrict__ g0 = b.g0;
-    const int lane = threadIdx.x & 63, wave = __builtin_amdgcn_readfirstlane(threadIdx.x >> 6);
-    const int chunk = first_chunk + wave;
-    if (chunk >= n_chunks) return;
-    const int o0 = chunk_start[chunk], o1 = chunk_start[chunk + 1];
-    double vals[90];
-#pragma unroll
-    for (int i = 0; i < 90; i++) vals[i] = 0.0;
-    const ObsIdx head = idx[o0];
-    Ent ec, em;
-    load_ent(ent, head.cam, ec);
-    load_ent(ent, head.marker, em);
-    double K[9];
-#pragma unroll
-    for (int i = 0; i < 9; i++) K[i] = Kmat[b.kstride * head.cam + i];
-    for (int o = o0 + lane; o < o1; o += 64) {
-        const ObsIdx id = idx[o];
-        const float4 uv0 = reinterpret_cast<const float4 *>(uv)[2 * (int64_t)o];
-        const float4 uv1 = reinterpret_cast<const float4 *>(uv)[2 * (int64_t)o + 1];
-        const float ou[8] = {uv0.x, uv0.y, uv0.z, uv0.w, uv1.x, uv1.y, uv1.z, uv1.w};
-        Ent ef;
-        load_ent(ent, A + id.frame, ef);
-#pragma unroll LEAN ? 1 : 4
-        for (int k = 0; k < 4; k++) {
-            CornerGeom g;
-            project_corner(ec, em, ef, K, h, k, g);
-            double r[2];
-            float ox, oy;
-            if (LEAN) { const float2 t = reinterpret_cast<const float2 *>(uv)[4 * (int64_t)o + k]; ox = t.x; oy = t.y; }
-            else { ox = ou[2 * k]; oy = ou[2 * k + 1]; }
-            corner_residual(ox, oy, g.u, g.v, res_f32, huber, r[0], r[1]);
-            double Gc[2][6], Gm[2][6], Gf[2][6];
-            corner_jacobian<true, true, false>(ec, em, ef, K, g, Gc, Gm, Gf);
-#pragma unroll
-            for (int rr = 0; rr < 2; rr++) {
-#pragma unroll
-                for (int i = 0; i < 6; i++) {
-                    vals[78 + i] += Gc[rr][i] * r[rr];
-                    vals[84 + i] += Gm[rr][i] * r[rr];
-#pragma unroll
-                    for (int j = 0; j <= i; j++) {
-                        vals[i * (i + 1) / 2 + j] += Gc[rr][i] * Gc[rr][j];
-                        vals[21 + i * (i + 1) / 2 + j] += Gm[rr][i] * Gm[rr][j];
-                    }
-#pragma unroll
-                    for (int j = 0; j < 6; j++) vals[42 + i * 6 + j] += Gc[rr][i] * Gm[rr][j];
-                }
-            }
-        }
-    }
-    const int rc = 6 * head.cam, rm = 6 * head.marker;
-    wave_sum_lds<90>(vals, scratch + wave * 2048, lane, [&](int v, double s) {
-        if (DET) { b.part[(size_t)chunk * b.part_stride + v] = s; return; }
-        if (v < 42) {
-            const int base = v < 21 ? rc : rm, p = v < 21 ? v : v - 21;
-            int i = 0;
-            while ((i + 1) * (i + 2) / 2 <= p) i++;
-            const int j = p - i * (i + 1) / 2;
-            atomicAdd(U0 + (size_t)(base + i) * n_pad + base + j, s);
-        } else if (v < 78) {
-            const int i = (v - 42) / 6, j = (v - 42) % 6;
-            atomicAdd(U0 + (size_t)(rm + j) * n_pad + rc + i, s);
-        } else if (v < 84) {
-            atomicAdd(g0 + rc + (v - 78), s);
-        } else {
-            atomicAdd(g0 + rm + (v - 84), s);
-        }
-    });
-}
 
 template <bool DET = false>
 __device__ __forceinline__ void passB_wrench_body(const PassBArgs &b, double *scratch, const int first_chunk) {
@@ -1061,6 +989,14 @@
     else passB_body(b, lds, ((int)blockIdx.x - a.F) * (BLOCK / 64));
 }
 template <int BLOCK, int CPL>
+__global__ void __launch_bounds__(BLOCK) k_passA_fused(const PassAArgs a, const BacksubArgs bs, double *g0_clear, int n_g0) {
+    extern __shared__ double lds[];
+    if ((int)blockIdx.x < a.F) { passA_wrench_body<BLOCK, CPL, false, true>(a, lds, (int)blockIdx.x, a.F, &bs); return; }
+    backsub_shared(bs, lds, [&](int i) -> double { return bs.delta_s[i]; }, [] {}, 256);
+    __syncthreads();
+    for (int i = threadIdx.x; i < n_g0; i += BLOCK) g0_clear[i] = 0.0;
+}
+template <int BLOCK, int CPL>
 __global__ void __launch_bounds__(BLOCK, 2) k_passAB_o2(const PassAArgs a, const PassBArgs b) {
     extern __shared__ double lds[];
     if ((int)blockIdx.x < a.F) passA_wrench_body<BLOCK, CPL>(a, lds, (int)blockIdx.x, a.F);
@@ -1170,7 +1106,7 @@
     return a;
 }
 
-static PassBArgs passB_args(const DeviceProblem &P, int which) {
+PassBArgs passB_args(const DeviceProblem &P, int which) {
     PassBArgs b;
     b.idx = P.b_idx; b.uv = P.b_uv; b.ent = P.ent[which]; b.chunk_start = P.chunk_start;
     { const KTable kt = k_table(P, which); b.Kmat = kt.base; b.kstride = kt.stride; }
@@ -1226,6 +1162,23 @@
     else launch_passA_t<128, 4>(P, a, pbargs, st);
 }
 
+template <int B, int CPL>
+static void launch_passA_fused_t(const DeviceProblem &P, const PassAArgs &a, const BacksubArgs &bs, double *g0c, hipStream_t st) {
+    const size_t lds = passA_wrench_lds_bytes(P.max_kf, false) + (size_t)P.max_kf * ENT_LDS * sizeof(double);
+    HookScope _h(P, KID_PASSA);
+    launch_lds(k_passA_fused<B, CPL>, dim3(P.F + 1), dim3(B), lds, st, a, bs, g0c, P.n_pad);
+}
+void launch_passA_fused(const DeviceProblem &P, int cur, int which, double mu_pred, hipStream_t st) {
+    PassAArgs a = passA_args(P, which, mu_pred, cur);
+    a.zero2 = nullptr; a.zero2_n = 0;
+    const BacksubArgs bs = backsub_args(P, cur, which, 1);
+    double *g0c = P.blk[cur].g0;
+    const double avg = (double)P.N / (double)P.F;
+    if (avg <= 14) launch_passA_fused_t<64, 1>(P, a, bs, g0c, st);
+    else if (avg <= 30) launch_passA_fused_t<64, 2>(P, a, bs, g0c, st);
+    else if (avg <= 96) launch_passA_fused_t<64, 4>(P, a, bs, g0c, st);
+    else launch_passA_fused_t<128, 4>(P, a, bs, g0c, st);
+}
 void launch_passA(const DeviceProblem &P, int which, double mu_pred, int zero_blk, hipStream_t st) {
     if (P.F == 0) return;
     launch_passA_any(P, passA_args(P, which, mu_pred, zero_blk), nullptr, st);
diff --git a/automatic-ar_amd/csrc/kernels.h b/automatic-ar_amd/csrc/kernels.h
--- a/automatic-ar_amd/csrc/kernels.h
+++ b/automatic-ar_amd/csrc/kernels.h
@@ -122,6 +122,7 @@
         int passB_wrench_merged = 0;
         int passB_lean = 0;
         int pack_system = -1;
+        int fused_step = 0;
         int init_headstart = 1;
     } tune;
     double *z[2] = {nullptr, nullptr};
@@ -183,6 +184,7 @@
 void launch_unpack(const DeviceProblem &P, int which, hipStream_t st, int zero_blk = -1);
 void launch_residual(const DeviceProblem &P, int which, double *r_out, hipStream_t st);
 void launch_passA(const DeviceProblem &P, int which, double mu_pred, int zero_blk, hipStream_t st);
+void launch_passA_fused(const DeviceProblem &P, int cur, int which, double mu_pred, hipStream_t st);
 void launch_passB(const DeviceProblem &P, int which, hipStream_t st);
 bool launch_passAB(const DeviceProblem &P, int which, double mu_pred, int zero_blk, hipStream_t st);
 size_t passA_lds_bytes(int max_kf, int block);
@@ -190,7 +192,7 @@
 void launch_maxdiag(const DeviceProblem &P, int which, hipStream_t st);
 void launch_frame_inv(const DeviceProblem &P, int which, double mu, hipStream_t st, const double *mu_dev = nullptr, double mu_scale = 0.0);
 bool launch_schur(const DeviceProblem &P, int which, double sign, hipStream_t st, unsigned long long ride_seq = 0, int ride_n_err = 0,
-                  double *ride_scal = nullptr, bool panels_ready = false);
+                  double *ride_scal = nullptr, bool panels_ready = false, int ride_passB = 0);
 bool launch_chol(const DeviceProblem &P, int which, double mu, hipStream_t st, int trial = -1);
 void launch_backsub(const DeviceProblem &P, int cur, int trial, hipStream_t st);
 void launch_pcg(const DeviceProblem &P, int which, double mu, hipStream_t st);
diff --git a/automatic-ar_amd/csrc/passb.hpp b/automatic-ar_amd/csrc/passb.hpp
--- /dev/null
+++ b/automatic-ar_amd/csrc/passb.hpp
@@ -0,0 +1,125 @@
+#pragma once
+#include "geom.hpp"
+#include "kernels.h"
+
+namespace aar {
+
+template <int NV, int CH = 32, class Sink>
+__device__ __forceinline__ void wave_sum_lds(const double (&vals)[NV], double *__restrict__ sc, int lane, Sink sink) {
+    constexpr int L = 64 / CH;
+    constexpr int SPREAD = 32 / CH > 0 ? 32 / CH : 1;
+#pragma unroll
+    for (int base = 0; base < NV; base += CH) {
+        const int cnt = (NV - base) < CH ? (NV - base) : CH;
+#pragma unroll
+        for (int i = 0; i < CH; i++)
+            if (i < cnt) sc[i * 64 + lane] = vals[base + i];
+        __builtin_amdgcn_fence(__ATOMIC_RELEASE, "wavefront");
+        __builtin_amdgcn_wave_barrier();
+        const int vi = lane / L, part = lane % L;
+        double s = 0;
+        if (vi < cnt) {
+            const double *row = sc + lane * CH;
+#pragma unroll 8
+            for (int k = 0; k < CH; k++) s += row[(k + lane / SPREAD) & (CH - 1)];
+        }
+#pragma unroll
+        for (int off = 1; off < L; off <<= 1) s += __shfl_xor(s, off);
+        if (part == 0 && vi < cnt) sink(base + vi, s);
+        __builtin_amdgcn_wave_barrier();
+        __builtin_amdgcn_fence(__ATOMIC_ACQUIRE, "wavefront");
+    }
+}
+
+struct PassBArgs {
+    const ObsIdx *idx; const float *uv; const double *ent; const double *Kmat; const int32_t *chunk_start;
+    int kstride, k_ent0;
+    int n_chunks, A, res_f32, n_pad;
+    float huber;
+    double h;
+    double *U0, *g0;
+    double *part; int part_stride;
+};
+
+template <bool DET = false, bool LEAN = false, int CH = 32>
+__device__ __forceinline__ void passB_body(const PassBArgs &b, double *scratch, const int first_chunk) {
+    const ObsIdx *__restrict__ idx = b.idx;
+    const float *__restrict__ uv = b.uv;
+    const double *__restrict__ ent = b.ent, *__restrict__ Kmat = b.Kmat;
+    const int32_t *__restrict__ chunk_start = b.chunk_start;
+    const int n_chunks = b.n_chunks, A = b.A, res_f32 = b.res_f32, n_pad = b.n_pad;
+    const float huber = b.huber;
+    const double h = b.h;
+    double *__restrict__ U0 = b.U0, *__restrict__ g0 = b.g0;
+    const int lane = threadIdx.x & 63, wave = __builtin_amdgcn_readfirstlane(threadIdx.x >> 6);
+    const int chunk = first_chunk + wave;
+    if (chunk >= n_chunks) return;
+    const int o0 = chunk_start[chunk], o1 = chunk_start[chunk + 1];
+    double vals[90];
+#pragma unroll
+    for (int i = 0; i < 90; i++) vals[i] = 0.0;
+    const ObsIdx head = idx[o0];
+    Ent ec, em;
+    load_ent(ent, head.cam, ec);
+    load_ent(ent, head.marker, em);
+    double K[9];
+#pragma unroll
+    for (int i = 0; i < 9; i++) K[i] = Kmat[b.kstride * head.cam + i];
+    for (int o = o0 + lane; o < o1; o += 64) {
+        const ObsIdx id = idx[o];
+        const float4 uv0 = reinterpret_cast<const float4 *>(uv)[2 * (int64_t)o];
+        const float4 uv1 = reinterpret_cast<const float4 *>(uv)[2 * (int64_t)o + 1];
+        const float ou[8] = {uv0.x, uv0.y, uv0.z, uv0.w, uv1.x, uv1.y, uv1.z, uv1.w};
+        Ent ef;
+        load_ent(ent, A + id.frame, ef);
+#pragma unroll LEAN ? 1 : 4
+        for (int k = 0; k < 4; k++) {
+            CornerGeom g;
+            project_corner(ec, em, ef, K, h, k, g);
+            double r[2];
+            float ox, oy;
+            if (LEAN) { const float2 t = reinterpret_cast<const float2 *>(uv)[4 * (int64_t)o + k]; ox = t.x; oy = t.y; }
+            else { ox = ou[2 * k]; oy = ou[2 * k + 1]; }
+            corner_residual(ox, oy, g.u, g.v, res_f32, huber, r[0], r[1]);
+            double Gc[2][6], Gm[2][6], Gf[2][6];
+            corner_jacobian<true, true, false>(ec, em, ef, K, g, Gc, Gm, Gf);
+#pragma unroll
+            for (int rr = 0; rr < 2; rr++) {
+#pragma unroll
+                for (int i = 0; i < 6; i++) {
+                    vals[78 + i] += Gc[rr][i] * r[rr];
+                    vals[84 + i] += Gm[rr][i] * r[rr];
+#pragma unroll
+                    for (int j = 0; j <= i; j++) {
+                        vals[i * (i + 1) / 2 + j] += Gc[rr][i] * Gc[rr][j];
+                        vals[21 + i * (i + 1) / 2 + j] += Gm[rr][i] * Gm[rr][j];
+                    }
+#pragma unroll
+                    for (int j = 0; j < 6; j++) vals[42 + i * 6 + j] += Gc[rr][i] * Gm[rr][j];
+                }
+            }
+        }
+    }
+    const int rc = 6 * head.cam, rm = 6 * head.marker;
+    wave_sum_lds<90, CH>(vals, scratch + wave * (CH * 64), lane, [&](int v, double s) {
+        if (DET) { b.part[(size_t)chunk * b.part_stride + v] = s; return; }
+        if (v < 42) {
+            const int base = v < 21 ? rc : rm, p = v < 21 ? v : v - 21;
+            int i = 0;
+            while ((i + 1) * (i + 2) / 2 <= p) i++;
+            const int j = p - i * (i + 1) / 2;
+            atomicAdd(U0 + (size_t)(base + i) * n_pad + base + j, s);
+        } else if (v < 78) {
+            const int i = (v - 42) / 6, j = (v - 42) % 6;
+            atomicAdd(U0 + (size_t)(rm + j) * n_pad + rc + i, s);
+        } else if (v < 84) {
+            atomicAdd(g0 + rc + (v - 78), s);
+        } else {
+            atomicAdd(g0 + rm + (v - 84), s);
+        }
+    });
+}
+
+PassBArgs passB_args(const DeviceProblem &P, int which);
+
+}
diff --git a/automatic-ar_amd/csrc/solve_kernels.hip b/automatic-ar_amd/csrc/solve_kernels.hip
--- a/automatic-ar_amd/csrc/solve_kernels.hip
+++ b/automatic-ar_amd/csrc/solve_kernels.hip
@@ -1,7 +1,9 @@
+#include <algorithm>
 #include <type_traits>
 #include "geom.hpp"
 #include "kernels.h"
 #include "backsub.hpp"
+#include "passb.hpp"
 
 namespace aar {
 
@@ -118,23 +120,17 @@
 
 __global__ void __launch_bounds__(256) k_reduce_scalars(const ReduceArgs r) { reduce_scalars_body(r); }
 
-template <int PRE, int NW = 4>
-__global__ void __launch_bounds__(64 * NW) k_schur(const int32_t *__restrict__ sw_ent, const int32_t *__restrict__ sw_begin,
-                                               const int32_t *__restrict__ sw_end, const int4 *__restrict__ pair_rec,
-                                               const int32_t *__restrict__ fslot_ent, const double *__restrict__ W,
-                                               const double *__restrict__ Vinv, const double *__restrict__ hf, int A,
-                                               int n_pad, double sign, double *__restrict__ S, double *__restrict__ rhs,
-                                               int rider, const ReduceArgs red, double *__restrict__ part = nullptr,
-                                               const int64_t *__restrict__ part_off = nullptr) {
-    if (rider && blockIdx.x == 0) {
-        reduce_scalars_body(red);
-        return;
-    }
-    extern __shared__ __align__(16) double lds[];
+template <int PRE, int NW>
+__device__ __forceinline__ void schur_item(double *lds, const int w, const int32_t *__restrict__ sw_ent, const int32_t *__restrict__ sw_begin,
+                                           const int32_t *__restrict__ sw_end, const int4 *__restrict__ pair_rec,
+                                           const int32_t *__restrict__ fslot_ent, const double *__restrict__ W,
+                                           const double *__restrict__ Vinv, const double *__restrict__ hf, int A,
+                                           int n_pad, double sign, double *__restrict__ S, double *__restrict__ rhs,
+                                           double *__restrict__ part, const int64_t *__restrict__ part_off) {
     double *panel = lds;
     double *pg = lds + (size_t)A * 36;
     double *ysc = pg + 8;
-    const int w = (int)blockIdx.x - rider, tid = threadIdx.x, lane = tid & 63, wave = __builtin_amdgcn_readfirstlane(tid >> 6);
+    const int tid = threadIdx.x, lane = tid & 63, wave = __builtin_amdgcn_readfirstlane(tid >> 6);
     const int a = sw_ent[w], pb = sw_begin[w], pe = sw_end[w];
     for (int i = tid; i < (a + 1) * 36; i += 64 * NW) panel[i] = 0.0;
     if (tid < 8) pg[tid] = 0.0;
@@ -261,6 +257,38 @@
     if (tid < 6) atomicAdd(rhs + 6 * a + tid, -sign * pg[tid]);
 }
 
+template <int PRE, int NW = 4>
+__global__ void __launch_bounds__(64 * NW) k_schur(const int32_t *__restrict__ sw_ent, const int32_t *__restrict__ sw_begin,
+                                               const int32_t *__restrict__ sw_end, const int4 *__restrict__ pair_rec,
+                                               const int32_t *__restrict__ fslot_ent, const double *__restrict__ W,
+                                               const double *__restrict__ Vinv, const double *__restrict__ hf, int A,
+                                               int n_pad, double sign, double *__restrict__ S, double *__restrict__ rhs,
+                                               int rider, const ReduceArgs red, double *__restrict__ part = nullptr,
+                                               const int64_t *__restrict__ part_off = nullptr) {
+    if (rider && blockIdx.x == 0) {
+        reduce_scalars_body(red);
+        return;
+    }
+    extern __shared__ __align__(16) double lds[];
+    schur_item<PRE, NW>(lds, (int)blockIdx.x - rider, sw_ent, sw_begin, sw_end, pair_rec, fslot_ent, W, Vinv, hf, A, n_pad, sign, S, rhs, part, part_off);
+}
+
+struct SchurItemArgs {
+    const int32_t *sw_ent, *sw_begin, *sw_end; const int4 *pair_rec; const int32_t *fslot_ent; const double *W, *Vinv, *hf;
+    int A, n_pad, n_swork; double sign; double *S, *rhs;
+};
+template <int PRE, bool LEAN>
+__global__ void __launch_bounds__(256, LEAN ? 2 : 1) k_schur_pb(const SchurItemArgs s, int rider, const ReduceArgs red, const PassBArgs pb) {
+    if (rider && blockIdx.x == 0) {
+        reduce_scalars_body(red);
+        return;
+    }
+    extern __shared__ __align__(16) double lds[];
+    const int w = (int)blockIdx.x - rider;
+    if (w >= s.n_swork) { passB_body<false, LEAN, 8>(pb, lds, (w - s.n_swork) * 4); return; }
+    schur_item<PRE, 4>(lds, w, s.sw_ent, s.sw_begin, s.sw_end, s.pair_rec, s.fslot_ent, s.W, s.Vinv, s.hf, s.A, s.n_pad, s.sign, s.S, s.rhs, nullptr, nullptr);
+}
+
 __global__ void __launch_bounds__(256) k_schur_reduce(const int32_t *__restrict__ se_start, const int32_t *__restrict__ se_items,
                                                       const int64_t *__restrict__ part_off, const double *__restrict__ part, int n_pad,
                                                       double sign, double *__restrict__ S, double *__restrict__ rhs) {
@@ -1390,7 +1418,7 @@
 }
 
 bool launch_schur(const DeviceProblem &P, int which, double sign, hipStream_t st, unsigned long long ride_seq, int ride_n_err, double *ride_scal,
-                  bool panels_ready) {
+                  bool panels_ready, int ride_passB) {
     const DeviceProblem::Blocks &b = P.blk[which];
     if (P.n_smwork > 0) {
         const size_t lds = (size_t)2 * SM_ROWS * SM_PS * sizeof(double);
@@ -1418,6 +1446,15 @@
     const ReduceArgs red = reduce_args(P, ride_n_err, false, ride_scal ? 0ull : ride_seq, ride_scal);
     const int extra = (ride_seq || ride_scal) ? 1 : 0;
     HookScope _h(P, KID_SCHUR);
+    if (ride_passB) {
+        const SchurItemArgs sa{P.sw_ent, P.sw_begin, P.sw_end, P.pair_rec, P.fslot_ent, b.W, b.Vinv, b.hf, P.A, P.n_pad, P.n_swork, sign, b.S, b.rhs};
+        const PassBArgs pa = passB_args(P, which);
+        const size_t ldsb = std::max(lds, (size_t)4 * 8 * 64 * sizeof(double));
+        const dim3 grid(P.n_swork + extra + (P.n_chunks + 3) / 4);
+        if (P.max_kf > 64) { if (ride_passB == 2) launch_lds(k_schur_pb<3, true>, grid, dim3(256), ldsb, st, sa, extra, red, pa); else launch_lds(k_schur_pb<3, false>, grid, dim3(256), ldsb, st, sa, extra, red, pa); }
+        else { if (ride_passB == 2) launch_lds(k_schur_pb<0, true>, grid, dim3(256), ldsb, st, sa, extra, red, pa); else launch_lds(k_schur_pb<0, false>, grid, dim3(256), ldsb, st, sa, extra, red, pa); }
+        return extra != 0;
+    }
     launch_lds(P.max_kf > 64 ? k_schur<3> : k_schur<0>, dim3(P.n_swork + extra), dim3(256), lds, st, P.sw_ent, P.sw_begin, P.sw_end, P.pair_rec, P.fslot_ent, b.W, b.Vinv, b.hf,
                P.A, P.n_pad, sign, b.S, b.rhs, extra, red, nullptr, nullptr);
     return extra != 0;
diff --git a/include/aar.h b/include/aar.h
--- a/include/aar.h
+++ b/include/aar.h
@@ -181,9 +181,11 @@
     double pcg_eta_loose;
     double pcg_eta_switch;
     double pcg_abs_tol;
+    int64_t fused_steps;
+    int64_t fused_check_values, fused_check_mismatches;
 } aar_solver_stats;
 int aar_problem_get_solver_stats(aar_problem *, aar_solver_stats *out);
-enum { AAR_TEST_HOOK_SPCG_DROP = 1 };
+enum { AAR_TEST_HOOK_SPCG_DROP = 1, AAR_TEST_HOOK_FUSED_CHECK = 2 };
 int aar_problem_set_test_hook(aar_problem *, int32_t hook, int32_t value);
 void aar_problem_destroy(aar_problem *);
 int64_t aar_problem_full_len(const aar_problem *);
```

Measured after the change: 12780. -4.5%, worse.
